# chengl7-lab/scape

Measured on AMD Instinct MI355X. Metric: UTR regions/sec (infer_pa EM to convergence), 50k UTRs x 2k reads synthetic, higher is better.
Workload: dtype f64; 1 GPU; 50k-UTR synthetic stream x 2000 reads, K=1..10 x 10 restarts; step = one resident batch of 512 UTRs per GPU; reads_per_utr=2000, k_cap=10, n_frag_max=1469, re_run_mode=False, rng_mode=per_utr, parallelism=utr-shard x1

## Files before the change

### include/scape_hip.h

```cpp
#ifndef SCAPE_HIP_H
#define SCAPE_HIP_H

#include <stdint.h>

#ifdef __cplusplus
extern "C" {
#endif

#define SCAPE_HIP_ABI_VERSION 4
#define SCAPE_SENT (-3.4028234663852886e38)
#define SCAPE_MAX_BETA 160
#define SCAPE_MAX_S 64
#define SCAPE_MAX_K 63
#define SCAPE_MAX_JOBS_PER_UTR 1024

typedef struct scape_hip_ctx scape_hip_ctx;

typedef struct scape_hip_params {
    double mu_f;
    double sigma_f;
    double max_unif_ws;
    int32_t n_beta;
    int32_t n_s;
    int32_t nround;
    int32_t reserved;
    double betas[SCAPE_MAX_BETA];
    double s_dis[SCAPE_MAX_S];
    double pmf_s[SCAPE_MAX_S];
} scape_hip_params;

int scape_hip_abi_version(void);
const char *scape_hip_last_error(void);
int scape_hip_device_count(int *count);
int scape_hip_create(int device, scape_hip_ctx **out);
int scape_hip_destroy(scape_hip_ctx *ctx);
int scape_hip_device_name(scape_hip_ctx *ctx, char *buf, int buflen);

int scape_hip_loglik_xlr_t_pa(scape_hip_ctx *ctx, const double *x, const double *l,
                              const double *pa, int32_t n, double theta, double sigma_f,
                              double *out);
int scape_hip_loglik_xlr_t_r_known(scape_hip_ctx *ctx, const double *x, const double *l,
                                   const double *r, int32_t n, const double *s_dis,
                                   const double *pmf_s, int32_t n_s, double theta, double mu_f,
                                   double sigma_f, double *out);
int scape_hip_loglik_xlr_t_r_unknown(scape_hip_ctx *ctx, const double *x, const double *l,
                                     const double *r, int32_t n, const double *s_dis,
                                     const double *pmf_s, int32_t n_s, double theta, double mu_f,
                                     double sigma_f, double *out);
int scape_hip_get_loglik_marginal_tensor(scape_hip_ctx *ctx, const double *all_theta,
                                         int32_t n_theta, const double *betas, int32_t n_beta,
                                         const double *loglik_xlr_t_arr, int32_t n_frag,
                                         double *out);

int scape_hip_batch_load(scape_hip_ctx *ctx, const scape_hip_params *params, int32_t n_utr,
                         const int64_t *bin_off, const double *x, const double *l,
                         const double *r, const double *pa, const double *cnt,
                         const int64_t *theta_off, const double *all_theta,
                         const double *utr_L, const double *min_theta, const double *unif_ll);
int scape_hip_batch_bytes(scape_hip_ctx *ctx, int64_t *bytes_batch, int64_t *bytes_free,
                          int64_t *bytes_total);
int scape_hip_batch_build(scape_hip_ctx *ctx);
int scape_hip_batch_phase_b_form(scape_hip_ctx *ctx, int32_t *form);
int scape_hip_batch_em(scape_hip_ctx *ctx, int32_t n_jobs, int32_t kmax, const int32_t *job_utr,
                       const int32_t *job_K, const int32_t *job_fixed, const int32_t *alpha_idx,
                       const int32_t *beta_idx, const double *ws, const int8_t *k_arr,
                       int32_t *alpha_idx_out, int32_t *beta_idx_out, double *ws_out,
                       double *bic_out, int32_t *n_lb_out, double *lb_out);
int scape_hip_batch_em_fetch_lb(scape_hip_ctx *ctx, int32_t n_sel, const int32_t *job_idx, double *lb_out);
int scape_hip_batch_labels(scape_hip_ctx *ctx, int32_t n_sel, int32_t kmax, const int32_t *sel_utr,
                           const int32_t *sel_K, const int32_t *alpha_idx, const int32_t *beta_idx,
                           const double *ws, int32_t *labels_out);
int scape_hip_batch_fetch_loglik(scape_hip_ctx *ctx, int32_t utr, double *A_out);
int scape_hip_batch_fetch_tensor(scape_hip_ctx *ctx, int32_t utr, double *M_out);
int scape_hip_batch_free(scape_hip_ctx *ctx);

int scape_hip_timing_reset(scape_hip_ctx *ctx);
int scape_hip_timing_get(scape_hip_ctx *ctx, int32_t which, double *ms_total, int32_t *n_launches);
int scape_hip_em_counters(scape_hip_ctx *ctx, int64_t *rounds, int64_t *slab_elems,
                          int64_t *z_elems);

int scape_hip_em_traffic(scape_hip_ctx *ctx, int64_t *mstep_tensor_bytes, int64_t *mstep_v_bytes_requested,
                         int64_t *mstep_v_bytes_unique, int64_t *mstep_launches);

int scape_hip_report_counts(scape_hip_ctx *ctx, int32_t n_rec, const int64_t *read_off, const int32_t *K,
                            const int64_t *label, const int64_t *cb_id, int64_t id_min, int64_t id_span,
                            const int32_t *id2col, int32_t n_cols, int64_t *row_tot_out, int8_t *complete_out,
                            int64_t *bad_read_out);
int scape_hip_report_render(scape_hip_ctx *ctx, int32_t slot, int32_t n_rows, const int64_t *rows, const int8_t *is_int,
                            const int64_t *pre_off, const char *pre, int64_t *bytes_out);
int scape_hip_report_render_mtx(scape_hip_ctx *ctx, int32_t slot, int32_t n_rows, const int64_t *rows, int64_t row_no0,
                                int64_t *bytes_out, int64_t *nnz_out);
int scape_hip_report_group_sums(scape_hip_ctx *ctx, int32_t n_seg, const int32_t *seg_off, int32_t n_rows,
                                const int64_t *rows, int32_t *sum_out, int32_t *nz_out);
int scape_hip_report_perm_masks(scape_hip_ctx *ctx, int32_t n1, int32_t n2, int64_t p_first, int32_t p_count,
                                uint64_t seed);
int scape_hip_report_perm_masks_strata(scape_hip_ctx *ctx, int32_t n_strata, const int32_t *m1, const int32_t *m2,
                                       int64_t p_first, int32_t p_count, uint64_t seed);
int scape_hip_report_perm_bits_get(scape_hip_ctx *ctx, int32_t p, uint64_t *words_out);
int scape_hip_report_perm_test(scape_hip_ctx *ctx, int32_t n_rec, const int64_t *rec_row_off, const int64_t *rows,
                               int64_t *t_out, int64_t *a0_out, int64_t *site_n_ge_out, double *stat0_out,
                               int64_t *gene_n_ge_out);
int scape_hip_report_perm_len(scape_hip_ctx *ctx, int32_t n_rec, const int64_t *rec_row_off, const int64_t *rows,
                              const double *w, const double *tol, int64_t *t_out, int64_t *a0_out, double *delta0_out,
                              int64_t *n_ge_out);
int scape_hip_report_perm_labels(scape_hip_ctx *ctx, int32_t n_groups, const int32_t *sizes, int64_t p_first,
                                 int32_t p_count, uint64_t seed);
int scape_hip_report_perm_labels_get(scape_hip_ctx *ctx, int32_t p, uint8_t *labels_out);
int scape_hip_report_perm_groups(scape_hip_ctx *ctx, int32_t n_rec, const int64_t *rec_row_off, const int64_t *rows,
                                 int32_t n_groups, const int32_t *seg_off, int64_t *t_out, int64_t *a0_out,
                                 int64_t *site_n_ge_out, double *stat0_out, double *site_stat0_out,
                                 int64_t *gene_n_ge_out);
int scape_hip_report_perm_len_groups(scape_hip_ctx *ctx, int32_t n_rec, const int64_t *rec_row_off, const int64_t *rows,
                                     int32_t n_groups, const int32_t *seg_off, const int32_t *q, const double *tol_stat,
                                     const double *tol_delta, int64_t *t_out, int64_t *a0_out, double *stat0_out,
                                     double *delta0_out, int64_t *n_ge_out, int64_t *group_n_ge_out);
int scape_hip_report_perm_pair_masks(scape_hip_ctx *ctx, int32_t n_groups, const int32_t *sizes, int32_t n_pairs,
                                     const int32_t *pair_g, const int32_t *pair_h, int64_t p_first, int32_t p_count,
                                     uint64_t seed);
int scape_hip_report_perm_pair_bits_get(scape_hip_ctx *ctx, int32_t pair, int32_t p, uint64_t *words_out);
int scape_hip_report_perm_pairs(scape_hip_ctx *ctx, int32_t n_rec, const int64_t *rec_row_off, const int64_t *rows,
                                int32_t n_groups, const int32_t *seg_off, int32_t pair_first, int32_t pair_count,
                                int64_t *t_out, int64_t *a0_out, int64_t *site_n_ge_out, double *stat0_out,
                                int64_t *gene_n_ge_out);
int scape_hip_report_perm_marker_masks(scape_hip_ctx *ctx, int32_t n_markers, const int32_t *sizes, int32_t n_others,
                                       const int32_t *orig_rank, int64_t p_first, int32_t p_count, uint64_t seed);
int scape_hip_report_perm_marker_bits_get(scape_hip_ctx *ctx, int32_t marker, int32_t p, uint64_t *words_out);
int scape_hip_report_perm_markers(scape_hip_ctx *ctx, int32_t n_rec, const int64_t *rec_row_off, const int64_t *rows,
                                  int32_t n_seg, const int32_t *seg_off, int32_t marker_first, int32_t marker_count,
                                  int64_t *t_out, int64_t *a0_out, int64_t *site_n_ge_out, double *stat0_out,
                                  int64_t *gene_n_ge_out);
int scape_hip_report_perm_scores(scape_hip_ctx *ctx, int32_t n, const uint16_t *q, int64_t p_first, int32_t p_count,
                                 uint64_t seed);
int scape_hip_report_perm_scores_get(scape_hip_ctx *ctx, int32_t p, uint16_t *scores_out);
int scape_hip_report_perm_trend(scape_hip_ctx *ctx, int32_t n_rec, const int64_t *rec_row_off, const int64_t *rows,
                                int64_t *t_out, int64_t *s0_out, int64_t *sq0_out, int64_t *site_n_ge_out,
                                double *d0_out, double *stat0_out, int64_t *gene_n_ge_out);
int scape_hip_report_perm_len_trend(scape_hip_ctx *ctx, int32_t n_rec, const int64_t *rec_row_off, const int64_t *rows,
                                    const int32_t *x, int64_t *t_out, int64_t *s0_out, int64_t *sq0_out,
                                    int64_t *c0_out ,
                                    int64_t *n_ge_out );
int scape_hip_report_fetch(scape_hip_ctx *ctx, int32_t slot, void **host_ptr, int64_t *bytes_out);
int scape_hip_report_hist(scape_hip_ctx *ctx, int32_t n_rec, const int64_t *read_off, const int32_t *K,
                          const int64_t *label, const int64_t *cb_id, int64_t id_min, int64_t id_span,
                          const int32_t *id2code, int32_t n_codes, int64_t *n_groups_out, int64_t *bad_read_out);
int scape_hip_report_hist_fetch(scape_hip_ctx *ctx, int64_t n_groups, int32_t *codes_out, int64_t n_hist,
                                int32_t *hist_out);
int scape_hip_report_free(scape_hip_ctx *ctx);

#ifdef __cplusplus
}
#endif
#endif
```

### scape_amd/_lib.py

```python
from __future__ import annotations

import ctypes
import os

import numpy as np

SENT = float(np.finfo("f").min)
MAX_BETA, MAX_S, MAX_K = 160, 64, 63
_HERE = os.path.dirname(os.path.abspath(__file__))
LIB_PATH = os.environ.get("SCAPE_HIP_LIB") or os.path.join(_HERE, "libscape_hip.so")

c_d, c_i, c_i32, c_i64 = ctypes.c_double, ctypes.c_int, ctypes.c_int32, ctypes.c_int64
P_d = ctypes.POINTER(c_d)
P_i32 = ctypes.POINTER(c_i32)
P_i64 = ctypes.POINTER(c_i64)
P_i8 = ctypes.POINTER(ctypes.c_int8)
P_u16 = ctypes.POINTER(ctypes.c_uint16)
P_void = ctypes.c_void_p


class ScapeHipError(RuntimeError):
    pass


class Params(ctypes.Structure):
    _fields_ = [("mu_f", c_d), ("sigma_f", c_d), ("max_unif_ws", c_d),
                ("n_beta", c_i32), ("n_s", c_i32), ("nround", c_i32), ("reserved", c_i32),
                ("betas", c_d * MAX_BETA), ("s_dis", c_d * MAX_S), ("pmf_s", c_d * MAX_S)]


SIGNATURES = {
    "scape_hip_abi_version": (c_i, []),
    "scape_hip_last_error": (ctypes.c_char_p, []),
    "scape_hip_device_count": (c_i, [ctypes.POINTER(c_i)]),
    "scape_hip_create": (c_i, [c_i, ctypes.POINTER(P_void)]),
    "scape_hip_destroy": (c_i, [P_void]),
    "scape_hip_device_name": (c_i, [P_void, ctypes.c_char_p, c_i]),
    "scape_hip_loglik_xlr_t_pa": (c_i, [P_void, P_d, P_d, P_d, c_i32, c_d, c_d, P_d]),
    "scape_hip_loglik_xlr_t_r_known": (c_i, [P_void, P_d, P_d, P_d, c_i32, P_d, P_d, c_i32, c_d, c_d, c_d, P_d]),
    "scape_hip_loglik_xlr_t_r_unknown": (c_i, [P_void, P_d, P_d, P_d, c_i32, P_d, P_d, c_i32, c_d, c_d, c_d, P_d]),
    "scape_hip_get_loglik_marginal_tensor": (c_i, [P_void, P_d, c_i32, P_d, c_i32, P_d, c_i32, P_d]),
    "scape_hip_batch_load": (c_i, [P_void, ctypes.POINTER(Params), c_i32, P_i64, P_d, P_d, P_d, P_d, P_d,
                                   P_i64, P_d, P_d, P_d, P_d]),
    "scape_hip_batch_bytes": (c_i, [P_void, P_i64, P_i64, P_i64]),
    "scape_hip_batch_phase_b_form": (c_i, [P_void, P_i32]),
    "scape_hip_batch_build": (c_i, [P_void]),
    "scape_hip_batch_em": (c_i, [P_void, c_i32, c_i32, P_i32, P_i32, P_i32, P_i32, P_i32, P_d, P_i8,
                                 P_i32, P_i32, P_d, P_d, P_i32, P_d]),
    "scape_hip_batch_em_fetch_lb": (c_i, [P_void, c_i32, P_i32, P_d]),
    "scape_hip_batch_labels": (c_i, [P_void, c_i32, c_i32, P_i32, P_i32, P_i32, P_i32, P_d, P_i32]),
    "scape_hip_batch_fetch_loglik": (c_i, [P_void, c_i32, P_d]),
    "scape_hip_batch_fetch_tensor": (c_i, [P_void, c_i32, P_d]),
    "scape_hip_batch_free": (c_i, [P_void]),
    "scape_hip_timing_reset": (c_i, [P_void]),
    "scape_hip_timing_get": (c_i, [P_void, c_i32, P_d, P_i32]),
    "scape_hip_em_counters": (c_i, [P_void, P_i64, P_i64, P_i64]),
    "scape_hip_em_traffic": (c_i, [P_void, P_i64, P_i64, P_i64, P_i64]),
    "scape_hip_report_counts": (c_i, [P_void, c_i32, P_i64, P_i32, P_i64, P_i64, c_i64, c_i64, P_i32, c_i32,
                                      P_i64, P_i8, P_i64]),
    "scape_hip_report_render": (c_i, [P_void, c_i32, c_i32, P_i64, P_i8, P_i64, ctypes.c_char_p, P_i64]),
    "scape_hip_report_render_mtx": (c_i, [P_void, c_i32, c_i32, P_i64, c_i64, P_i64, P_i64]),
    "scape_hip_report_group_sums": (c_i, [P_void, c_i32, P_i32, c_i32, P_i64, P_i32, P_i32]),
    "scape_hip_report_perm_masks": (c_i, [P_void, c_i32, c_i32, c_i64, c_i32, ctypes.c_uint64]),
    "scape_hip_report_perm_masks_strata": (c_i, [P_void, c_i32, P_i32, P_i32, c_i64, c_i32, ctypes.c_uint64]),
    "scape_hip_report_perm_bits_get": (c_i, [P_void, c_i32, ctypes.POINTER(ctypes.c_uint64)]),
    "scape_hip_report_perm_test": (c_i, [P_void, c_i32, P_i64, P_i64, P_i64, P_i64, P_i64, P_d, P_i64]),
    "scape_hip_report_perm_len": (c_i, [P_void, c_i32, P_i64, P_i64, P_d, P_d, P_i64, P_i64, P_d, P_i64]),
    "scape_hip_report_perm_labels": (c_i, [P_void, c_i32, P_i32, c_i64, c_i32, ctypes.c_uint64]),
    "scape_hip_report_perm_labels_get": (c_i, [P_void, c_i32, ctypes.POINTER(ctypes.c_uint8)]),
    "scape_hip_report_perm_groups": (c_i, [P_void, c_i32, P_i64, P_i64, c_i32, P_i32, P_i64, P_i64, P_i64, P_d, P_d,
                                           P_i64]),
    "scape_hip_report_perm_len_groups": (c_i, [P_void, c_i32, P_i64, P_i64, c_i32, P_i32, P_i32, P_d, P_d, P_i64, P_i64,
                                               P_d, P_d, P_i64, P_i64]),
    "scape_hip_report_perm_pair_masks": (c_i, [P_void, c_i32, P_i32, c_i32, P_i32, P_i32, c_i64, c_i32, ctypes.c_uint64]),
    "scape_hip_report_perm_pair_bits_get": (c_i, [P_void, c_i32, c_i32, ctypes.POINTER(ctypes.c_uint64)]),
    "scape_hip_report_perm_pairs": (c_i, [P_void, c_i32, P_i64, P_i64, c_i32, P_i32, c_i32, c_i32, P_i64, P_i64, P_i64,
                                          P_d, P_i64]),
    "scape_hip_report_perm_marker_masks": (c_i, [P_void, c_i32, P_i32, c_i32, P_i32, c_i64, c_i32, ctypes.c_uint64]),
    "scape_hip_report_perm_marker_bits_get": (c_i, [P_void, c_i32, c_i32, ctypes.POINTER(ctypes.c_uint64)]),
    "scape_hip_report_perm_markers": (c_i, [P_void, c_i32, P_i64, P_i64, c_i32, P_i32, c_i32, c_i32, P_i64, P_i64, P_i64,
                                            P_d, P_i64]),
    "scape_hip_report_perm_scores": (c_i, [P_void, c_i32, P_u16, c_i64, c_i32, ctypes.c_uint64]),
    "scape_hip_report_perm_scores_get": (c_i, [P_void, c_i32, P_u16]),
    "scape_hip_report_perm_trend": (c_i, [P_void, c_i32, P_i64, P_i64, P_i64, P_i64, P_i64, P_i64, P_d, P_d, P_i64]),
    "scape_hip_report_perm_len_trend": (c_i, [P_void, c_i32, P_i64, P_i64, P_i32, P_i64, P_i64, P_i64, P_i64, P_i64]),
    "scape_hip_report_fetch": (c_i, [P_void, c_i32, ctypes.POINTER(P_void), P_i64]),
    "scape_hip_report_hist": (c_i, [P_void, c_i32, P_i64, P_i32, P_i64, P_i64, c_i64, c_i64, P_i32, c_i32,
                                    P_i64, P_i64]),
    "scape_hip_report_hist_fetch": (c_i, [P_void, c_i64, P_i32, c_i64, P_i32]),
    "scape_hip_report_free": (c_i, [P_void]),
}

_lib = None


def load_library():
    global _lib
    if _lib is None:
        if not os.path.exists(LIB_PATH):
            raise ScapeHipError(
                f"{LIB_PATH} is missing: build it with `python -c 'import __graft_entry__ as g; g.build()'` "
                "(hipcc --offload-arch=gfx950); scape_amd has no CPU fallback")
        lib = ctypes.CDLL(LIB_PATH)
        for name, (res, args) in SIGNATURES.items():
            fn = getattr(lib, name)
            fn.restype, fn.argtypes = res, args
        if lib.scape_hip_abi_version() != 4:
            raise ScapeHipError("libscape_hip.so ABI version mismatch")
        _lib = lib
    return _lib


def last_error():
    return load_library().scape_hip_last_error().decode("utf-8", "replace")


def check(rc, what):
    if rc != 0:
        raise ScapeHipError(f"{what}: {last_error()}")


def ptr(a, t=P_d):
    return a.ctypes.data_as(t)


def f64(a):
    return np.ascontiguousarray(a, dtype=np.float64)


def i32(a):
    return np.ascontiguousarray(a, dtype=np.int32)


def device_count():
    n = c_i(0)
    check(load_library().scape_hip_device_count(ctypes.byref(n)), "device_count")
    return n.value


class Context:

    def __init__(self, device=0):
        self.lib = load_library()
        self.h = P_void()
        check(self.lib.scape_hip_create(int(device), ctypes.byref(self.h)), f"create(device={device})")
        self.device = device

    def close(self):
        if self.h:
            self.lib.scape_hip_destroy(self.h)
            self.h = P_void()

    def __del__(self):
        try:
            self.close()
        except Exception:
            pass

    def __enter__(self):
        return self

    def __exit__(self, *exc):
        self.close()

    def name(self):
        buf = ctypes.create_string_buffer(256)
        check(self.lib.scape_hip_device_name(self.h, buf, 256), "device_name")
        return buf.value.decode()


_default_ctx = {}


def default_context(device=None):
    if device is None:
        device = int(os.environ.get("SCAPE_HIP_DEVICE", os.environ.get("LOCAL_RANK", "0")))
    if device not in _default_ctx:
        _default_ctx[device] = Context(device)
    return _default_ctx[device]
```

### scape_amd/csrc/em_lockstep.inc

```

#define MT_RB 1
#define MT_ROWS (64 * MT_RB)
#define MT_NC 32
#define MT_PITCH (MT_NC + 2)
#define MT_VPITCH (MT_NC + 2)
#define MT_MAXJ 64
#ifndef EM_DEPTH
#define EM_DEPTH 3
#endif
static_assert(EM_DEPTH >= 1 && EM_DEPTH <= 8, "column slots per job");
#ifndef MT_DV1
#define MT_DV1 1
#endif

#ifndef MT_DEEP
#define MT_DEEP 2
#endif
#define CNT_SLAB 4
#define CNT_EXEC (4 + 64)
#define CNT_MSTEP_TENSOR (4 + 2 * 64)
#define CNT_MSTEP_VREQ (4 + 3 * 64)
#define CNT_MSTEP_VUNI (4 + 4 * 64)
static_assert(MT_ROWS == TILE_ROWS, "tile height must match k_tile_extent / the host tables");
static_assert(MT_MAXJ <= 64, "the per-pass job setup gives one job to each lane of one wavefront");

struct EmState {
    int32_t *ia, *ib, *sia, *sib;
    double *ws, *slw;
    double *lb, *ell;
    int32_t *nlb, *status;
    unsigned long long *pend;
    int32_t *rd_k, *rd_lo, *rd_hi, *rd_m;
    int32_t *rd_n0, *rd_n1;
    double *rd_lw, *rd_sv;
    double *V;
    double *Vsuf;
    const int64_t *voff;
    double *pt_score;
    int32_t *pt_row;
    const int64_t *ptoff;
};

__device__ __forceinline__ double d_wave_allsum(double v) {
#pragma unroll
    for (int off = 32; off > 0; off >>= 1) v += __shfl_xor(v, off, 64);
    return v;
}

#ifndef ESTEP_EXP_GROUP
#define ESTEP_EXP_GROUP 1
#endif
struct EstepNext {
    int status;
    int nlb;
    int pub_k;
    int k_next;
};

template <int CA, int CX, int NW = 1>
__device__ __forceinline__ EstepNext estep_body(
    const UtrDesc *__restrict__ descs, const DevParams &P, const double *__restrict__ cnt,
    const double *__restrict__ M, int kmax, const int32_t *__restrict__ job_utr,
    const int32_t *__restrict__ job_K, const int32_t *__restrict__ job_fixed,
    const int32_t *__restrict__ a_in, const int32_t *__restrict__ b_in,
    const double *__restrict__ ws_in, const int8_t *__restrict__ k_arr, const EmState &S,
    int32_t *__restrict__ a_out, int32_t *__restrict__ b_out, double *__restrict__ ws_out,
    double *__restrict__ bic_out, int32_t *__restrict__ nlb_out, double *__restrict__ lb_out,
    unsigned long long *__restrict__ counters, int launch, int slot, int depth, int job, int lane, int status,
    unsigned long long *s_roff, double *s_lwc, double *s_wsum ,
    const double2 *s_exptab , int wave = 0, double *s_xz = nullptr ,
    double *s_tot = nullptr ) {
    constexpr int CMAX = CA;
#ifdef ESTEP_STAMPS
    const unsigned long long st0 = __builtin_amdgcn_s_memtime();
#define ESTEP_STAMP(v) const unsigned long long v = __builtin_amdgcn_s_memtime()
#else
#define ESTEP_STAMP(v)
#endif
    const bool lead = (NW == 1) || wave == 0;
    const int nround = P.nround, B = P.B;
    const int u_job = job_utr[job];
    const int K = (CX > 0) ? CX - 1 : job_K[job], C = K + 1;
    const bool fixed = job_fixed[job] != 0;
    int32_t *ia = S.ia + (size_t)job * kmax, *ib = S.ib + (size_t)job * kmax;
    int32_t *sia = S.sia + (size_t)job * kmax, *sib = S.sib + (size_t)job * kmax;
    double *ws = S.ws + (size_t)job * (kmax + 1), *slw = S.slw + (size_t)job * (kmax + 1);
    const bool r0 = launch == 0 && slot == 0;
    const bool resolve = slot == 0 && launch > 0;
    const size_t col0 = (size_t)job * depth, col = col0 + slot;
    int pre_m[EM_DEPTH], pre_lo[EM_DEPTH], pre_hi[EM_DEPTH], pre_k[EM_DEPTH];
    int64_t pre_ptoff[EM_DEPTH];
    bool rdm = false;
#pragma unroll
    for (int q = 0; q < EM_DEPTH; ++q) {
        const bool on = resolve && q < depth;
        pre_m[q] = on ? S.rd_m[col0 + q] : 0;
        pre_lo[q] = on ? S.rd_lo[col0 + q] : 0;
        pre_hi[q] = on ? S.rd_hi[col0 + q] : 0;
        pre_k[q] = on ? S.rd_k[col0 + q] : 0;
        pre_ptoff[q] = on ? S.ptoff[col0 + q] : 0;
        rdm = rdm || pre_m[q] != 0;
    }
    const int64_t pre_voff = S.voff[col];
    const int k_lane = (lane < nround) ? (int)k_arr[(size_t)job * nround + lane] : 0;
    const double lb_prev = r0 ? SENT : S.lb[job];
    const int nlb_prev = r0 ? 0 : S.nlb[job];
    auto k_of_round = [&](int i) {
        const int ii = min(i, nround - 1);
        return (nround <= 64) ? __shfl(k_lane, ii, 64) : (int)k_arr[(size_t)job * nround + ii];
    };
    const int k_now = k_of_round(nlb_prev);
    const int k_next = __builtin_amdgcn_readfirstlane(k_of_round(nlb_prev + 1));
    double my_ws = 0.0, my_slw = 0.0;
    int my_ia = 0, my_ib = 0, my_sia = 0, my_sib = 0;
    if (lane < C) {
        my_ws = r0 ? ws_in[(size_t)job * (kmax + 1) + lane] : ws[lane];
        if (!r0) my_slw = slw[lane];
        if (lane < K) {
            my_ia = r0 ? a_in[(size_t)job * kmax + lane] : ia[lane];
            my_ib = r0 ? b_in[(size_t)job * kmax + lane] : ib[lane];
            my_sia = r0 ? my_ia : sia[lane];
            my_sib = r0 ? my_ib : sib[lane];
        }
    }
    const UtrDesc d = descs[u_job];
    double pt_best[EM_DEPTH];
    int pt_best_r[EM_DEPTH];
#pragma unroll
    for (int q = 0; q < EM_DEPTH; ++q) {
        pt_best[q] = -INFINITY;
        pt_best_r[q] = pre_lo[q];
        if (pre_m[q]) {
            const int t0 = pre_lo[q] / MT_ROWS, t1 = (pre_hi[q] - 1) / MT_ROWS;
            for (int t = t0 + lane; t <= t1; t += 64) {
                const double sc = S.pt_score[pre_ptoff[q] + t];
                const int rr = S.pt_row[pre_ptoff[q] + t];
                if (sc > pt_best[q]) {
                    pt_best[q] = sc;
                    pt_best_r[q] = rr;
                }
            }
        }
    }
    const int N = d.N, Np = d.Np;
    const double *Mu = M + (size_t)d.m_off;
    const double *cu = cnt + d.bin_off;
    if (r0) my_slw = d_logw(my_ws);

    if (lead && r0) {
        if (lane < C) {
            ws[lane] = my_ws;
            slw[lane] = my_slw;
            if (lane < K) {
                ia[lane] = sia[lane] = my_ia;
                ib[lane] = sib[lane] = my_ib;
            }
        }
        if (lane == 0) {
            S.lb[job] = SENT;
            S.nlb[job] = 0;
            S.ell[job] = 0.0;
        }
    }
    int upd_k[EM_DEPTH], upd_a[EM_DEPTH], upd_b[EM_DEPTH];
#pragma unroll
    for (int q = 0; q < EM_DEPTH; ++q) {
        upd_k[q] = -1;
        upd_a[q] = upd_b[q] = 0;
        if (pre_m[q]) {
            double best = pt_best[q];
            int best_r = pt_best_r[q];
#pragma unroll
            for (int off = 32; off > 0; off >>= 1) {
                const double ob = __shfl_xor(best, off, 64);
                const int orr = __shfl_xor(best_r, off, 64);
                if (ob > best || (ob == best && orr < best_r)) {
                    best = ob;
                    best_r = orr;
                }
            }
            upd_k[q] = pre_k[q];
            upd_a[q] = best_r / B;
            upd_b[q] = best_r - upd_a[q] * B;
            if (lead && lane == 0) {
                ia[upd_k[q]] = upd_a[q];
                ib[upd_k[q]] = upd_b[q];
            }
            if (lane == upd_k[q]) {
                my_ia = upd_a[q];
                my_ib = upd_b[q];
            }
        }
    }
    if (slot == 0 && lead && lane == 0 && (r0 || rdm))
        for (int q = 0; q < depth; ++q) S.rd_m[col0 + q] = 0;
    auto cur_ia = [&](int i) {
        int v = ia[i];
#pragma unroll
        for (int q = 0; q < EM_DEPTH; ++q) v = (i == upd_k[q]) ? upd_a[q] : v;
        return v;
    };
    auto cur_ib = [&](int i) {
        int v = ib[i];
#pragma unroll
        for (int q = 0; q < EM_DEPTH; ++q) v = (i == upd_k[q]) ? upd_b[q] : v;
        return v;
    };

    if (status == 1 || nlb_prev >= nround) {
        if (lead && lane == 0) {
            const int n_lb = S.nlb[job];
            bic_out[job] = d_bic(S.ell[job], K, N);
            nlb_out[job] = n_lb;
            int idx[CMAX];
            for (int i = 0; i < K; ++i) idx[i] = i;
            for (int i = 1; i < K; ++i) {
                const int v = idx[i];
                int j = i - 1;
                while (j >= 0 && cur_ia(idx[j]) > cur_ia(v)) {
                    idx[j + 1] = idx[j];
                    --j;
                }
                idx[j + 1] = v;
            }
            for (int i = 0; i < K; ++i) {
                a_out[(size_t)job * kmax + i] = cur_ia(idx[i]);
                b_out[(size_t)job * kmax + i] = cur_ib(idx[i]);
                ws_out[(size_t)job * (kmax + 1) + i] = ws[idx[i]];
            }
            ws_out[(size_t)job * (kmax + 1) + K] = ws[K];
            for (int i = K; i < kmax; ++i) {
                a_out[(size_t)job * kmax + i] = -1;
                b_out[(size_t)job * kmax + i] = -1;
                ws_out[(size_t)job * (kmax + 1) + i + 1] = 0.0;
            }
            S.status[job] = 2;
            atomicAdd(&counters[0], (unsigned long long)n_lb);
            atomicAdd(&counters[2], (unsigned long long)n_lb * (unsigned long long)N * (unsigned long long)C);
        }
        return EstepNext{2, nlb_prev, -1, 0};
    }

    if (lead && lane == 0) atomicAdd(&counters[CNT_EXEC + (job & 63)], 1ull);
    const int k = k_now;
    const double wk_old = __shfl(my_ws, k, 64);
    const double slw_k = d_logw(wk_old);
    const int sia_k = (k < K) ? __shfl(my_ia, k, 64) : 0;
    const int sib_k = (k < K) ? __shfl(my_ib, k, 64) : 0;
    const int ia_km1 = __shfl(my_ia, max(k - 1, 0), 64), ia_kp1 = __shfl(my_ia, min(k + 1, 63), 64);
    if (lead && lane == 0) {
        slw[k] = slw_k;
        if (k < K) {
            sia[k] = sia_k;
            sib[k] = sib_k;
        }
    }
    if (lead && lane < CMAX) {
        const int c = lane;
        int sa = 0, sb = 0;
        double lw_c = 0.0;
        if (c < C) {
            if (c == k) {
                lw_c = slw_k;
                sa = sia_k;
                sb = sib_k;
            } else {
                lw_c = my_slw;
                sa = my_sia;
                sb = my_sib;
            }
        }
        s_roff[c] = (c < K) ? ((unsigned long long)sa * B + sb) * Np : 0ull;
        s_lwc[c] = (c < K) ? lw_c : lw_c + d.unif_ll;
    }
    __syncthreads();
    double *Vj = S.V + pre_voff;

    ESTEP_STAMP(st1);
    double tot_w[CMAX], t_sumk = 0.0, t_ell = 0.0, t_ent = 0.0;
    int nz_lo = 0x7fffffff, nz_hi = -1;
    bool mod = false;
    if constexpr (NW == 1) {
        for (int pass = 0; pass < 2; ++pass) {
    #pragma unroll
            for (int c = 0; c < CMAX; ++c) s_wsum[c * 64 + lane] = 0.0;
            double sumk = 0.0, ell = 0.0, ent = 0.0;
            nz_lo = 0x7fffffff;
            nz_hi = -1;
            double mcur[CMAX], ccur = 0.0;
            auto fetch = [&](int n, double (&m)[CMAX], double &cn) {
                const bool ok = n < N;
                cn = ok ? cu[n] : 0.0;
    #pragma unroll
                for (int c = 0; c < CMAX; ++c) m[c] = (ok && c < K) ? Mu[s_roff[c] + n] : 0.0;
            };
            fetch(lane, mcur, ccur);
    #pragma unroll
            for (int c = 0; c < CMAX; ++c) asm volatile("" : "+v"(mcur[c]));
            asm volatile("" : "+v"(ccur));
            for (int n = lane; n < Np; n += 64) {
                double mnext[CMAX], cnext;
                fetch(n + 64, mnext, cnext);
                double vkn = 0.0;
                if (n < N) {
                    const double cn = ccur;
                    auto lzv = [&](int c) { return (c < K) ? s_lwc[c] + mcur[c] : s_lwc[c]; };
                    double mx = 0.0;
    #pragma unroll
                    for (int c = 0; c < CMAX; ++c) {
                        if (c < C) {
                            const double v = lzv(c);
                            mx = (c == 0 || v > mx) ? v : mx;
                        }
                    }
                    double z[CMAX];
                    unsigned long long live = 0ull;
#if ESTEP_EXP_GROUP >= 2
    #pragma unroll
                    for (int c = 0; c < CMAX; c += ESTEP_EXP_GROUP) {
    #pragma unroll
                        for (int i = 0; i < ESTEP_EXP_GROUP; ++i)
                            if (c + i < CMAX) z[c + i] = 0.0;
                        if (c < C) {
                            double arg[ESTEP_EXP_GROUP];
                            bool any_live = false;
    #pragma unroll
                            for (int i = 0; i < ESTEP_EXP_GROUP; ++i) {
                                const bool in = (c + i < CMAX) && (c + i < C);
                                arg[i] = in ? (lzv((c + i < CMAX) ? c + i : c) - mx) * cn : -1000.0;
                                any_live |= arg[i] >= -746.0;
                            }
                            if (__ballot(any_live)) {
    #pragma unroll
                                for (int i = 0; i < ESTEP_EXP_GROUP; ++i)
                                    if (c + i < CMAX)
                                        if (c + i < C) {
                                            live |= 1ull << (c + i);
                                            z[c + i] = d_exp_nonpos(arg[i], s_exptab);
                                        }
                            }
                            __builtin_amdgcn_sched_barrier(0);
                        }
                    }
#else
    #pragma unroll
                    for (int c = 0; c < CMAX; ++c) {
                        z[c] = 0.0;
                        if (c < C) {
                            const double arg = (lzv(c) - mx) * cn;
                            if (__ballot(arg >= -746.0)) {
                                live |= 1ull << c;
                                z[c] = d_exp_nonpos(arg, s_exptab);
                            }
                            __builtin_amdgcn_sched_barrier(0);
                        }
                    }
#endif
                    const double s = d_np_sum<CMAX>(z, C);
                    const double rs = d_rcp_mid(s);
                    double zk = 0.0;
    #pragma unroll
                    for (int c = 0; c < CMAX; ++c) {
                        if (live & (1ull << c)) z[c] = z[c] * rs;
                        if (c == k) {
                            sumk += z[c];
                            if (mod) z[c] += 1e-8;
                            zk = z[c];
                        }
                    }
                    const double s2 = d_np_sum<CMAX>(z, C);
                    const double x2 = s2 - 1.0;
                    const double ls = d_log_pos(s), rs2 = d_rcp_mid(s2);
                    double ls2 = x2 - 0.5 * x2 * x2;
                    if (__ballot(fabs(x2) >= 1e-5)) ls2 = (fabs(x2) < 1e-5) ? ls2 : log(s2);
                    double lzk_mod = 0.0;
                    if (mod) lzk_mod = log(zk);
                    double en = 0.0;
    #pragma unroll
                    for (int c = 0; c < CMAX; ++c) {
                        if (c < C && ((live & (1ull << c)) || (mod && c == k))) {
                            const double lzc_full = lzv(c);
                            s_wsum[c * 64 + lane] += cn * z[c];
                            if (z[c] != 0.0) ell += (z[c] * cn) * lzc_full;
                            const double pk = z[c] * rs2;
                            const double lzc = (mod && c == k) ? lzk_mod : (lzc_full - mx) * cn - ls;
                            en += (pk > 0.0) ? -pk * (lzc - ls2) : 0.0;
                        }
                    }
                    ent += cn * en;
                    vkn = zk * cn;
                }
                Vj[n] = vkn;
                if (vkn != 0.0) {
                    nz_lo = min(nz_lo, n);
                    nz_hi = n;
                }
    #pragma unroll
                for (int c = 0; c < CMAX; ++c) mcur[c] = mnext[c];
                ccur = cnext;
            }
    #pragma unroll
            for (int c = 0; c < CMAX; ++c) tot_w[c] = d_wave_allsum(s_wsum[c * 64 + lane]);
            t_sumk = d_wave_allsum(sumk);
            t_ell = d_wave_allsum(ell);
            t_ent = d_wave_allsum(ent);
            if (pass == 0 && t_sumk < 1e-8) {
                mod = true;
                continue;
            }
            break;
        }
    } else {
        for (int pass = 0; pass < 2; ++pass) {
#pragma unroll
            for (int c = 0; c < CMAX; ++c)
                if ((c % NW) == wave) s_wsum[c * 64 + lane] = 0.0;
            double sumk = 0.0, ell = 0.0, ent = 0.0;
            nz_lo = 0x7fffffff;
            nz_hi = -1;
            double mcur[CMAX], ccur = 0.0;
            auto fetch = [&](int n, double (&m)[CMAX], double &cn) {
                const bool ok = n < N;
                cn = ok ? cu[n] : 0.0;
#pragma unroll
                for (int c = 0; c < CMAX; ++c) m[c] = (ok && c < K) ? Mu[s_roff[c] + n] : 0.0;
            };
            fetch(lane, mcur, ccur);
#pragma unroll
            for (int c = 0; c < CMAX; ++c) asm volatile("" : "+v"(mcur[c]));
            asm volatile("" : "+v"(ccur));
            int buf = 0;
            for (int n0 = 0; n0 < Np; n0 += 64, buf ^= 1) {
                const int n = n0 + lane;
                double mnext[CMAX], cnext;
                fetch(n + 64, mnext, cnext);
                double *xz = s_xz + (size_t)buf * (CMAX * 64);
                const double cn = ccur;
                auto lzv = [&](int c) { return (c < K) ? s_lwc[c] + mcur[c] : s_lwc[c]; };
                double mx = 0.0;
                if (n < N) {
#pragma unroll
                    for (int c = 0; c < CMAX; ++c) {
                        if (c < C) {
                            const double v = lzv(c);
                            mx = (c == 0 || v > mx) ? v : mx;
                        }
                    }
#pragma unroll
                    for (int c = 0; c < CMAX; ++c) {
                        if (c < C && (c % NW) == wave) {
                            const double arg = (lzv(c) - mx) * cn;
                            double zr = 0.0;
                            if (__ballot(arg >= -746.0)) zr = d_exp_nonpos(arg, s_exptab);
                            xz[c * 64 + lane] = zr;
                            __builtin_amdgcn_sched_barrier(0);
                        }
                    }
                }
                __syncthreads();
                double vkn = 0.0;
                if (n < N) {
                    double z[CMAX];
#pragma unroll
                    for (int c = 0; c < CMAX; ++c) z[c] = (c < C) ? xz[c * 64 + lane] : 0.0;
                    const double s = d_np_sum<CMAX>(z, C);
                    const double rs = d_rcp_mid(s);
                    double zk = 0.0;
#pragma unroll
                    for (int c = 0; c < CMAX; ++c) {
                        z[c] = z[c] * rs;
                        if (c == k) {
                            sumk += z[c];
                            if (mod) z[c] += 1e-8;
                            zk = z[c];
                        }
                    }
                    const double s2 = d_np_sum<CMAX>(z, C);
                    const double x2 = s2 - 1.0;
                    const double ls = d_log_pos(s), rs2 = d_rcp_mid(s2);
                    double ls2 = x2 - 0.5 * x2 * x2;
                    if (__ballot(fabs(x2) >= 1e-5)) ls2 = (fabs(x2) < 1e-5) ? ls2 : log(s2);
                    double lzk_mod = 0.0;
                    if (mod) lzk_mod = log(zk);
#pragma unroll
                    for (int c = 0; c < CMAX; ++c)
                        if (c < C && (c % NW) == wave) s_wsum[c * 64 + lane] += cn * z[c];
                    if (lead) {
                        double en = 0.0;
#pragma unroll
                        for (int c = 0; c < CMAX; ++c) {
                            if (c < C) {
                                const double lzc_full = lzv(c);
                                if (z[c] != 0.0) ell += (z[c] * cn) * lzc_full;
                                const double pk = z[c] * rs2;
                                const double lzc = (mod && c == k) ? lzk_mod : (lzc_full - mx) * cn - ls;
                                en += (pk > 0.0) ? -pk * (lzc - ls2) : 0.0;
                            }
                        }
                        ent += cn * en;
                        vkn = zk * cn;
                    }
                }
                if (lead && n < Np) {
                    Vj[n] = vkn;
                    if (vkn != 0.0) {
                        nz_lo = min(nz_lo, n);
                        nz_hi = n;
                    }
                }
#pragma unroll
                for (int c = 0; c < CMAX; ++c) mcur[c] = mnext[c];
                ccur = cnext;
            }
#pragma unroll
            for (int c = 0; c < CMAX; ++c) {
                if ((c % NW) == wave) {
                    const double t = d_wave_allsum(s_wsum[c * 64 + lane]);
                    if (lane == 0) s_tot[c] = t;
                }
            }
            if (lead) {
                t_sumk = d_wave_allsum(sumk);
                t_ell = d_wave_allsum(ell);
                t_ent = d_wave_allsum(ent);
                if (lane == 0) s_tot[CMAX] = (pass == 0 && t_sumk < 1e-8) ? 1.0 : 0.0;
            }
            __syncthreads();
#pragma unroll
            for (int c = 0; c < CMAX; ++c) tot_w[c] = s_tot[c];
            const bool redo = s_tot[CMAX] != 0.0;
            __syncthreads();
            if (redo) {
                mod = true;
                continue;
            }
            break;
        }
        if (!lead) return EstepNext{0, 0, -1, 0};
    }

    ESTEP_STAMP(st2);
    double sv = 0.0;
#pragma unroll
    for (int c = 0; c < CMAX; ++c)
        if (c == k) sv = tot_w[c];
    double wn[CMAX];
#pragma unroll
    for (int c = 0; c < CMAX; ++c) wn[c] = (c < C) ? tot_w[c] : 0.0;
    {
        const double s = d_np_sum<CMAX>(wn, C);
#pragma unroll
        for (int c = 0; c < CMAX; ++c) wn[c] = wn[c] / s;
        double wK = 0.0;
#pragma unroll
        for (int c = 0; c < CMAX; ++c)
            if (c == K) wK = wn[c];
        if (wK > P.max_unif_ws) {
            const double sk = d_np_sum<CMAX>(wn, K);
#pragma unroll
            for (int c = 0; c < CMAX; ++c) {
                if (c < K) wn[c] = (1 - P.max_unif_ws) * wn[c] / sk;
                if (c == K) wn[c] = P.max_unif_ws;
            }
        }
    }
    double wk_new = 0.0;
#pragma unroll
    for (int c = 0; c < CMAX; ++c) {
        if (c == k) wk_new = wn[c];
        if (c == lane && c < C) ws[c] = wn[c];
    }

#pragma unroll
    for (int off = 32; off > 0; off >>= 1) {
        nz_lo = min(nz_lo, __shfl_xor(nz_lo, off, 64));
        nz_hi = max(nz_hi, __shfl_xor(nz_hi, off, 64));
    }
    ESTEP_STAMP(st3);
    if (!fixed && k < K) {
        double *Sj = S.Vsuf + (pre_voff >> 4) + col;
        double carry = 0.0;
        for (int nb = ((Np - 1) >> 6) << 6; nb >= 0; nb -= 8 * 64) {
            double vv[8];
#pragma unroll
            for (int q = 0; q < 8; ++q) {
                const int n = nb - 64 * q + lane;
                vv[q] = (n >= 0 && n < Np) ? Vj[n] : 0.0;
            }
#pragma unroll
            for (int off = 1; off < 64; off <<= 1) {
#pragma unroll
                for (int q = 0; q < 8; ++q) {
                    const double t = __shfl_down(vv[q], off, 64);
                    if (lane + off < 64) vv[q] += t;
                }
            }
#pragma unroll
            for (int q = 0; q < 8; ++q) {
                const int n0 = nb - 64 * q;
                if (n0 >= 0) {
                    const int n = n0 + lane;
                    if ((lane & 15) == 0 && n < Np) Sj[n >> 4] = carry + vv[q];
                    carry += __shfl(vv[q], 0, 64);
                }
            }
        }
        if (lane == 0) Sj[Np >> 4] = 0.0;
    }
    ESTEP_STAMP(st4);
    const double lb_new = t_ell + t_ent;
    const int status_new = (fabs(lb_new - lb_prev) < fabs(1e-6 * lb_prev)) ? 1 : 0;
    const bool has_m = (!fixed && k < K);
    if (lane == 0) {
        const int n_lb = nlb_prev;
        lb_out[(size_t)job * nround + n_lb] = lb_new;
        S.nlb[job] = n_lb + 1;
        S.ell[job] = t_ell;
        S.lb[job] = lb_new;
        S.status[job] = status_new;
        S.rd_m[col] = has_m ? 1 : 0;
        if (has_m) {
            const int lo = (k == 0) ? 0 : ia_km1;
            const int hi = (k == K - 1) ? d.T - 1 : ia_kp1;
            S.rd_k[col] = k;
            S.rd_lo[col] = lo * B;
            S.rd_hi[col] = (hi + 1) * B;
            S.rd_lw[col] = d_logw(wk_new);
            S.rd_sv[col] = sv;
            S.rd_n0[col] = (nz_hi >= 0) ? nz_lo : 0;
            S.rd_n1[col] = (nz_hi >= 0) ? nz_hi + 1 : 0;
            atomicAdd(&counters[CNT_SLAB + (job & 63)], (unsigned long long)(hi + 1 - lo) * B * (unsigned long long)N);
        }
    }
#ifdef ESTEP_STAMPS
    if (NW == 1 && lane == 0) {
        const unsigned long long st5 = __builtin_amdgcn_s_memtime();
        unsigned long long *sp = counters + 4 + 5 * 64;
        atomicAdd(&sp[0], st1 - st0);
        atomicAdd(&sp[1], st2 - st1);
        atomicAdd(&sp[2], st3 - st2);
        atomicAdd(&sp[3], st4 - st3);
        atomicAdd(&sp[4], st5 - st4);
        atomicAdd(&sp[7], 1ull);
    }
#endif
#undef ESTEP_STAMP
    return EstepNext{status_new, nlb_prev + 1, has_m ? k : -1, k_next};
}

#define ESTEP_ARGS(ROUND, STATUS) descs, P, cnt, M, kmax, job_utr, job_K, job_fixed, a_in, b_in, ws_in, k_arr, S, a_out, \
                   b_out, ws_out, bic_out, nlb_out, lb_out, counters, ROUND, slot, depth, job, lane, STATUS, s_roff, s_lwc, s_wsum, s_exptab
#define ESTEP_CASE(C, ROUND, STATUS) \
    case C: nx = estep_body<C, C, ESTEP_NW>(ESTEP_ARGS(ROUND, STATUS) ESTEP_EXTRA); break;
#define ESTEP_DISPATCH(CM, ROUND, STATUS)                                                         \
    do {                                                                                          \
        if constexpr (CM <= 16) {                                                                 \
            const int c_exact = job_K[job] + 1;                                                   \
            if constexpr (CM >= 16) {                                                             \
                if (c_exact > 12) {                                                               \
                    switch (c_exact) {                                                            \
                        ESTEP_CASE(13, ROUND, STATUS) ESTEP_CASE(14, ROUND, STATUS)               \
                        ESTEP_CASE(15, ROUND, STATUS)                                             \
                        default: nx = estep_body<16, 16, ESTEP_NW>(ESTEP_ARGS(ROUND, STATUS) ESTEP_EXTRA); break;            \
                    }                                                                             \
                    break;                                                                        \
                }                                                                                 \
            }                                                                                     \
            if constexpr (CM >= 12) {                                                             \
                if (c_exact > 8) {                                                                \
                    switch (c_exact) {                                                            \
                        ESTEP_CASE(9, ROUND, STATUS) ESTEP_CASE(10, ROUND, STATUS)                \
                        ESTEP_CASE(11, ROUND, STATUS)                                             \
                        default: nx = estep_body<12, 12, ESTEP_NW>(ESTEP_ARGS(ROUND, STATUS) ESTEP_EXTRA); break;            \
                    }                                                                             \
                    break;                                                                        \
                }                                                                                 \
            }                                                                                     \
            if constexpr (CM >= 8) {                                                              \
                if (c_exact > 4) {                                                                \
                    switch (c_exact) {                                                            \
                        ESTEP_CASE(5, ROUND, STATUS) ESTEP_CASE(6, ROUND, STATUS)                 \
                        ESTEP_CASE(7, ROUND, STATUS)                                              \
                        default: nx = estep_body<8, 8, ESTEP_NW>(ESTEP_ARGS(ROUND, STATUS) ESTEP_EXTRA); break;              \
                    }                                                                             \
                    break;                                                                        \
                }                                                                                 \
            }                                                                                     \
            switch (c_exact) {                                                                    \
                ESTEP_CASE(1, ROUND, STATUS) ESTEP_CASE(2, ROUND, STATUS) ESTEP_CASE(3, ROUND, STATUS) \
                default: nx = estep_body<4, 4, ESTEP_NW>(ESTEP_ARGS(ROUND, STATUS) ESTEP_EXTRA); break;                      \
            }                                                                                     \
        } else {                                                                                  \
            nx = estep_body<CM, 0, ESTEP_NW>(ESTEP_ARGS(ROUND, STATUS) ESTEP_EXTRA);                                       \
        }                                                                                         \
    } while (0)

__host__ __device__ inline bool em_run_ahead_stops(int status, int nlb, int nround, int k_next, unsigned long long pend) {
    return status != 0 || nlb >= nround || (pend & (7ull << k_next)) != 0ull;
}
#define ESTEP_NW 1
#ifndef ESTEP_WPS
#define ESTEP_WPS 3
#endif
#define ESTEP_EXTRA
template <int CMAX>
__global__ __launch_bounds__(64, (CMAX > 12 ? 2 : ESTEP_WPS)) void k2_estep(
    const UtrDesc *__restrict__ descs, DevParams P, const double *__restrict__ cnt,
    const double *__restrict__ M, int kmax, const int32_t *__restrict__ job_utr,
    const int32_t *__restrict__ job_K, const int32_t *__restrict__ job_fixed,
    const int32_t *__restrict__ a_in, const int32_t *__restrict__ b_in,
    const double *__restrict__ ws_in, const int8_t *__restrict__ k_arr, EmState S,
    int32_t *__restrict__ a_out, int32_t *__restrict__ b_out, double *__restrict__ ws_out,
    double *__restrict__ bic_out, int32_t *__restrict__ nlb_out, double *__restrict__ lb_out,
    unsigned long long *__restrict__ counters, int launch, int slot, int depth, const int32_t *__restrict__ job_list,
    int n_jobs) {
    const int chunk = (n_jobs + 7) >> 3;
    const int jidx = (int)(blockIdx.x & 7) * chunk + (int)(blockIdx.x >> 3);
    if (jidx >= n_jobs) return;
    const int job = job_list[jidx];
    const int lane = threadIdx.x;
    const int status = (launch == 0 && slot == 0) ? 0 : S.status[job];
    if (status == 2) return;
    unsigned long long pend = 0ull;
    if (slot > 0) {
        pend = S.pend[job];
        if (!(pend & 1ull)) return;
        pend &= ~1ull;
    }
    __shared__ unsigned long long s_roff[CMAX];
    __shared__ double s_lwc[CMAX];
    __shared__ double s_wsum[CMAX * 64];
    __shared__ double2 s_exptab[128];
    d_load_exptab(s_exptab, lane, 64);
    EstepNext nx;
    ESTEP_DISPATCH(CMAX, launch, status);
    if (depth > 1 && lane == 0) {
        if (nx.pub_k >= 0) pend |= 2ull << nx.pub_k;
        const bool stop = em_run_ahead_stops(nx.status, nx.nlb, P.nround, nx.k_next, pend) || job_fixed[job] != 0;
        S.pend[job] = pend | (stop ? 0ull : 1ull);
    }
}

template <int CMAX>
__global__ __launch_bounds__(64, (CMAX > 12 ? 2 : 3)) void k2_estep_all_rounds(
    const UtrDesc *__restrict__ descs, DevParams P, const double *__restrict__ cnt,
    const double *__restrict__ M, int kmax, const int32_t *__restrict__ job_utr,
    const int32_t *__restrict__ job_K, const int32_t *__restrict__ job_fixed,
    const int32_t *__restrict__ a_in, const int32_t *__restrict__ b_in,
    const double *__restrict__ ws_in, const int8_t *__restrict__ k_arr, EmState S,
    int32_t *__restrict__ a_out, int32_t *__restrict__ b_out, double *__restrict__ ws_out,
    double *__restrict__ bic_out, int32_t *__restrict__ nlb_out, double *__restrict__ lb_out,
    unsigned long long *__restrict__ counters, const int32_t *__restrict__ job_list, int n_jobs) {
    const int chunk = (n_jobs + 7) >> 3;
    const int jidx = (int)(blockIdx.x & 7) * chunk + (int)(blockIdx.x >> 3);
    if (jidx >= n_jobs) return;
    const int job = job_list[jidx];
    const int lane = threadIdx.x;
    __shared__ unsigned long long s_roff[CMAX];
    __shared__ double s_lwc[CMAX];
    __shared__ double s_wsum[CMAX * 64];
    __shared__ double2 s_exptab[128];
    d_load_exptab(s_exptab, lane, 64);
    for (int round = 0; round <= P.nround; ++round) {
        const int status = (round == 0) ? 0 : S.status[job];
        if (status == 2) return;
        constexpr int slot = 0, depth = 1;
        EstepNext nx;
        ESTEP_DISPATCH(CMAX, round, status);
        (void)nx;
        __threadfence();
        __syncthreads();
    }
}
#undef ESTEP_NW
#undef ESTEP_EXTRA
#define ESTEP_NW 4
#define ESTEP_EXTRA , wave, s_xz, s_tot
template <int CMAX>
__global__ __launch_bounds__(256, 1) void k2_estep_cs(
    const UtrDesc *__restrict__ descs, DevParams P, const double *__restrict__ cnt,
    const double *__restrict__ M, int kmax, const int32_t *__restrict__ job_utr,
    const int32_t *__restrict__ job_K, const int32_t *__restrict__ job_fixed,
    const int32_t *__restrict__ a_in, const int32_t *__restrict__ b_in,
    const double *__restrict__ ws_in, const int8_t *__restrict__ k_arr, EmState S,
    int32_t *__restrict__ a_out, int32_t *__restrict__ b_out, double *__restrict__ ws_out,
    double *__restrict__ bic_out, int32_t *__restrict__ nlb_out, double *__restrict__ lb_out,
    unsigned long long *__restrict__ counters, int round, const int32_t *__restrict__ job_list, int n_jobs) {
    const int chunk = (n_jobs + 7) >> 3;
    const int jidx = (int)(blockIdx.x & 7) * chunk + (int)(blockIdx.x >> 3);
    if (jidx >= n_jobs) return;
    const int job = job_list[jidx];
    const int lane = threadIdx.x & 63, wave = threadIdx.x >> 6;
    const int status = (round == 0) ? 0 : S.status[job];
    if (status == 2) return;
    __shared__ unsigned long long s_roff[CMAX];
    __shared__ double s_lwc[CMAX];
    __shared__ double s_wsum[CMAX * 64];
    __shared__ double s_xz[2 * CMAX * 64];
    __shared__ double s_tot[CMAX + 4];
    __shared__ double2 s_exptab[128];
    d_load_exptab(s_exptab, threadIdx.x, 256);
    constexpr int slot = 0, depth = 1;
    EstepNext nx;
    ESTEP_DISPATCH(CMAX, round, status);
    (void)nx;
}
#undef ESTEP_NW
#undef ESTEP_EXTRA
#undef ESTEP_DISPATCH
#undef ESTEP_CASE


typedef double v4f64 __attribute__((ext_vector_type(4)));

template <int G, int D>
__device__ __forceinline__ void mstep_pass(const double *__restrict__ Mu, const double *__restrict__ V,
                                           const int64_t *__restrict__ voff, const int *s_jobs, double *mt,
                                           double *vt, int cnt, int Np, int n_lo, int n_hi, int nrows, int row0, int wave, int lane,
                                           int need, v4f64 (&acc)[MT_RB][MT_MAXJ / 16]) {
    const int quarter = lane >> 4, ns = 2 * (lane & 15);
    const int kq = lane >> 4, rc = lane & 15;
    constexpr int DV = MT_DV1 ? 1 : D;
    double2 rm_st[D][4 * MT_RB], rv_st[DV][G];
    const double *vsrc[G];
#pragma unroll
    for (int it = 0; it < G; ++it) {
        const int js = 4 * wave + quarter + 16 * it;
        vsrc[it] = (js < cnt) ? V + voff[s_jobs[js]] : nullptr;
    }
    auto fetchV = [&](int n0, double2 (&rv)[G]) {
        const int nc = (n_hi - n0 < MT_NC) ? n_hi - n0 : MT_NC;
#pragma unroll
        for (int it = 0; it < G; ++it)
            rv[it] = (ns < nc && vsrc[it]) ? *reinterpret_cast<const double2 *>(vsrc[it] + n0 + ns) : make_double2(0.0, 0.0);
    };
    auto fetchM = [&](int n0, double2 (&rm)[4 * MT_RB]) {
        const int nc = (n_hi - n0 < MT_NC) ? n_hi - n0 : MT_NC;
#pragma unroll
        for (int it = 0; it < 4 * MT_RB; ++it) {
            const int row = row0 + 4 * wave + quarter + 16 * it;
            rm[it] = (ns < nc && row < nrows && ((need >> (it / MT_RB)) & 1)) ? *reinterpret_cast<const double2 *>(Mu + (size_t)row * Np + n0 + ns)
                                               : make_double2(0.0, 0.0);
        }
    };
    auto chunk = [&](int n0, double2 (&rm)[4 * MT_RB], double2 (&rv)[G]) {
        const int nc = (n_hi - n0 < MT_NC) ? n_hi - n0 : MT_NC;
        __syncthreads();
#pragma unroll
        for (int it = 0; it < 4 * MT_RB; ++it) {
            const int rr = 4 * wave + quarter + 16 * it;
            *reinterpret_cast<double2 *>(&mt[rr * MT_PITCH + ns]) = rm[it];
        }
#pragma unroll
        for (int it = 0; it < G; ++it) {
            const int js = 4 * wave + quarter + 16 * it;
            *reinterpret_cast<double2 *>(&vt[js * MT_VPITCH + ns]) = rv[it];
        }
        __syncthreads();
        fetchM(n0 + D * MT_NC, rm);
        fetchV(n0 + DV * MT_NC, rv);
#pragma unroll 4
        for (int n4 = 0; n4 < nc; n4 += 4) {
            double a[MT_RB], b[G];
#pragma unroll
            for (int rb = 0; rb < MT_RB; ++rb) a[rb] = mt[(16 * (MT_RB * wave + rb) + rc) * MT_PITCH + n4 + kq];
#pragma unroll
            for (int g = 0; g < G; ++g) b[g] = vt[(16 * g + rc) * MT_VPITCH + n4 + kq];
#pragma unroll
            for (int rb = 0; rb < MT_RB; ++rb)
#pragma unroll
                for (int g = 0; g < G; ++g)
                    acc[rb][g] = __builtin_amdgcn_mfma_f64_16x16x4f64(a[rb], b[g], acc[rb][g], 0, 0, 0);
        }
    };
#pragma unroll
    for (int dd = 0; dd < D; ++dd) fetchM(n_lo + dd * MT_NC, rm_st[dd]);
#pragma unroll
    for (int dd = 0; dd < DV; ++dd) fetchV(n_lo + dd * MT_NC, rv_st[dd]);
    for (int n0 = n_lo; n0 < n_hi; n0 += D * MT_NC) {
#pragma unroll
        for (int dd = 0; dd < D; ++dd)
            if (n0 + dd * MT_NC < n_hi) chunk(n0 + dd * MT_NC, rm_st[dd], rv_st[dd % DV]);
    }
}

__global__ __launch_bounds__(256, 3) void k2_mstep(const UtrDesc *__restrict__ descs, DevParams P,
                                                   const double *__restrict__ M, const int32_t *__restrict__ active, int n_utr, int tiles_max,
                                                   const int64_t *__restrict__ ujob_off,
                                                   const int32_t *__restrict__ ujob_list,
                                                   const double *__restrict__ V,
                                                   const double *__restrict__ Vsuf,
                                                   const int64_t *__restrict__ voff,
                                                   const int32_t *__restrict__ rd_m,
                                                   const int32_t *__restrict__ rd_lo,
                                                   const int32_t *__restrict__ rd_hi,
                                                   const double *__restrict__ rd_lw,
                                                   const double *__restrict__ rd_sv,
                                                   const int32_t *__restrict__ rd_n0,
                                                   const int32_t *__restrict__ rd_n1,
                                                   const int64_t *__restrict__ ptoff,
                                                   double *__restrict__ pt_score,
                                                   int32_t *__restrict__ pt_row,
                                                   const int32_t *__restrict__ tile_nend,
                                                   unsigned long long *__restrict__ counters, int jobs_per_pass,
                                                   unsigned long long *__restrict__ dbg) {
    __shared__ __attribute__((aligned(16))) double mt[MT_ROWS * MT_PITCH];
    __shared__ __attribute__((aligned(16))) double vt[MT_MAXJ * MT_VPITCH];
    __shared__ int s_jobs[MT_MAXJ];
    __shared__ int s_all[1024];
    __shared__ int s_cnt, s_nlo, s_nhi, s_need, s_first;
    __shared__ double s_ps[4][MT_MAXJ];
    __shared__ int s_pr[4][MT_MAXJ];
    __shared__ double s_tail[MT_MAXJ];
    const int id = blockIdx.x;
    int ul, t;
    if (n_utr >= 8) {
        const int slot = id >> 3;
        ul = (slot / tiles_max) * 8 + (id & 7);
        t = slot % tiles_max;
    } else {
        ul = id % n_utr;
        t = id / n_utr;
    }
    if (ul >= n_utr || t >= tiles_max) return;
    const int u = active[ul];
    const UtrDesc d = descs[u];
    const int B = P.B, Np = d.Np;
    const int nrows = d.T * B, row0 = t * MT_ROWS;
    if (row0 >= nrows) return;
    const int tid = threadIdx.x, lane = tid & 63, wave = tid >> 6;
    const double *Mu = M + (size_t)d.m_off;
    const int64_t jlo = ujob_off[u], jhi = ujob_off[u + 1];
    __shared__ int s_wcnt[4];
    int found = 0;
    for (int64_t j0 = jlo; j0 < jhi; j0 += 256) {
        const int64_t jj = j0 + tid;
        int j = -1;
        bool hit = false;
        if (jj < jhi) {
            j = ujob_list[jj];
            hit = rd_m[j] && rd_lo[j] < row0 + MT_ROWS && rd_hi[j] > row0;
        }
        const unsigned long long mask = __ballot(hit);
        if (lane == 0) s_wcnt[wave] = __popcll(mask);
        __syncthreads();
        int off = found;
        for (int w = 0; w < wave; ++w) off += s_wcnt[w];
        off += __popcll(mask & ((1ull << lane) - 1ull));
        if (hit && off < 1024) s_all[off] = j;
        found += s_wcnt[0] + s_wcnt[1] + s_wcnt[2] + s_wcnt[3];
        __syncthreads();
    }
    if (tid == 0) s_cnt = found;
    __syncthreads();
    const int total = min(s_cnt, 1024);
    if (dbg && tid == 0) {
        atomicAdd(&dbg[0], 1ull);
        atomicAdd(&dbg[1], (unsigned long long)(total > 0));
        atomicAdd(&dbg[2], (unsigned long long)total);
        atomicAdd(&dbg[3], (unsigned long long)((total + MT_MAXJ - 1) / MT_MAXJ));
        atomicAdd(&dbg[4 + min((total + 15) / 16, 11)], 1ull);
    }
    if (total == 0) return;
    __shared__ unsigned long long s_by[3];
    if (tid == 0) s_by[0] = s_by[1] = s_by[2] = 0ull;

    for (int base = (int)blockIdx.y * jobs_per_pass; base < total; base += jobs_per_pass * (int)gridDim.y) {
        const int cnt = min(jobs_per_pass, total - base);
        const int G = (cnt + 15) >> 4;
        __syncthreads();
        if (wave == 0) {
            int mk = 0, nlo = 0x7fffffff, nhi = 0;
            bool fst = false;
            if (lane < cnt) {
                const int j = s_all[base + lane];
                s_jobs[lane] = j;
                fst = rd_lo[j] / MT_ROWS == t;
                const int lo = rd_lo[j] - row0, hi = rd_hi[j] - row0;
#pragma unroll
                for (int g4 = 0; g4 < 4; ++g4) mk |= (lo < 16 * (g4 + 1) && hi > 16 * g4) ? (1 << g4) : 0;
                if (rd_n1[j] > rd_n0[j]) {
                    nlo = rd_n0[j];
                    nhi = rd_n1[j];
                }
            }
#pragma unroll
            for (int off = 32; off > 0; off >>= 1) {
                mk |= __shfl_xor(mk, off, 64);
                nlo = min(nlo, __shfl_xor(nlo, off, 64));
                nhi = max(nhi, __shfl_xor(nhi, off, 64));
            }
            const unsigned long long fmask = __ballot(fst);
            if (lane == 0) {
                s_need = mk;
                s_nlo = nlo;
                s_nhi = nhi;
                s_first = __popcll(fmask);
            }
        }
        __syncthreads();
        const int n_lo = (s_nhi > 0) ? (s_nlo & ~15) : 0;
        const int n_sup = (s_nhi > 0) ? min(Np, (s_nhi + 15) & ~15) : 0;
        const int n_ext = tile_nend[d.tile_off + t];
        const int n_hi = min(n_sup, n_ext);
        const int need = s_need;
        if (tid == 0 && n_hi > n_lo) {
            int rows = 0;
#pragma unroll
            for (int g4 = 0; g4 < 4; ++g4)
                if ((need >> g4) & 1) rows += max(0, min(16, nrows - row0 - 16 * g4));
            const unsigned long long span = (unsigned long long)(n_hi - n_lo) * 8ull;
            s_by[0] += span * (unsigned long long)rows;
            s_by[1] += span * (unsigned long long)cnt;
            s_by[2] += span * (unsigned long long)s_first;
        }
        for (int sj = tid; sj < cnt; sj += 256) {
            const int j = s_jobs[sj];
            s_tail[sj] = Vsuf[(voff[j] >> 4) + j + (n_ext >> 4)];
        }
        __syncthreads();
        v4f64 acc[MT_RB][MT_MAXJ / 16];
#pragma unroll
        for (int rb = 0; rb < MT_RB; ++rb)
#pragma unroll
            for (int g = 0; g < MT_MAXJ / 16; ++g) acc[rb][g] = (v4f64){0.0, 0.0, 0.0, 0.0};
        switch (G) {
            case 1: mstep_pass<1, MT_DEEP>(Mu, V, voff, s_jobs, mt, vt, cnt, Np, n_lo, n_hi, nrows, row0, wave, lane, need, acc); break;
            case 2: mstep_pass<2, MT_DEEP>(Mu, V, voff, s_jobs, mt, vt, cnt, Np, n_lo, n_hi, nrows, row0, wave, lane, need, acc); break;
            case 3: mstep_pass<3, 2>(Mu, V, voff, s_jobs, mt, vt, cnt, Np, n_lo, n_hi, nrows, row0, wave, lane, need, acc); break;
            default: mstep_pass<4, 2>(Mu, V, voff, s_jobs, mt, vt, cnt, Np, n_lo, n_hi, nrows, row0, wave, lane, need, acc); break;
        }
        {
            const int kq = lane >> 4, rc = lane & 15;
#pragma unroll
            for (int g = 0; g < MT_MAXJ / 16; ++g) {
                if (g < G) {
                    const int slot_j = 16 * g + rc;
                    double best = -INFINITY;
                    int best_r = 0x7fffffff;
                    if (slot_j < cnt) {
                        const int j = s_jobs[slot_j];
                        const int lo = rd_lo[j], hi = rd_hi[j];
                        const double tl = s_tail[slot_j];
                        const double c0 = rd_lw[j] * rd_sv[j] + ((tl != 0.0) ? SENT * tl : 0.0);
#pragma unroll
                        for (int rb = 0; rb < MT_RB; ++rb) {
#pragma unroll
                            for (int i = 0; i < 4; ++i) {
                                const int row = row0 + 16 * (MT_RB * wave + rb) + kq + 4 * i;
                                const double sc = c0 + acc[rb][g][i];
                                if (row >= lo && row < hi && row < nrows && sc > best) {
                                    best = sc;
                                    best_r = row;
                                }
                            }
                        }
                    }
#pragma unroll
                    for (int off = 16; off <= 32; off <<= 1) {
                        const double ob = __shfl_xor(best, off, 64);
                        const int orr = __shfl_xor(best_r, off, 64);
                        if (ob > best || (ob == best && orr < best_r)) {
                            best = ob;
                            best_r = orr;
                        }
                    }
                    if (kq == 0 && slot_j < cnt) {
                        s_ps[wave][slot_j] = best;
                        s_pr[wave][slot_j] = best_r;
                    }
                }
            }
        }
        __syncthreads();
        for (int sj = tid; sj < cnt; sj += 256) {
            double best = s_ps[0][sj];
            int best_r = s_pr[0][sj];
            for (int w = 1; w < 4; ++w)
                if (s_ps[w][sj] > best) {
                    best = s_ps[w][sj];
                    best_r = s_pr[w][sj];
                }
            const int j = s_jobs[sj];
            pt_score[ptoff[j] + t] = best;
            pt_row[ptoff[j] + t] = (best_r == 0x7fffffff) ? max(rd_lo[j], row0) : best_r;
        }
    }
    if (tid == 0 && s_by[0]) {
        const int sh = (int)(blockIdx.x & 63);
        atomicAdd(&counters[CNT_MSTEP_TENSOR + sh], s_by[0]);
        atomicAdd(&counters[CNT_MSTEP_VREQ + sh], s_by[1]);
        atomicAdd(&counters[CNT_MSTEP_VUNI + sh], s_by[2]);
    }
}
```

### scape_amd/csrc/mstep_multi.inc

```

#ifndef M4_TPW
#define M4_TPW 2
#endif
static_assert(M4_TPW >= 1 && M4_TPW <= 4, "one wavefront per tile table");
#define M4_NW 4
#define M4_WPC M3_WPC
static_assert(M4_TPW * M4_NW <= 16, "per-wavefront hit counts of the set-up");
__device__ __forceinline__ bool m4_is_tile_issuer(int wave) { return wave < 2; }
__device__ __forceinline__ bool m4_is_vec_issuer(int wave) { return wave >= 2; }
__device__ __forceinline__ int m4_role_index(int wave) { return wave & 1; }
#define M4_REC_BYTES (64 * 24)
#define M4_TAIL_BYTES (4 * 64 * 12 + M4_TPW * (M4_REC_BYTES + 12 * 4) + 16 * 4 + 4 * 8)
#define M4_AREA_BYTES (((M4_WPC >= 3 ? 53760 : 81920) - M4_TAIL_BYTES) / 1024 * 1024)
#define M4_LDS_BYTES (M4_AREA_BYTES + M4_TAIL_BYTES)
static_assert((M4_LDS_BYTES + 1279) / 1280 * M4_WPC <= 128, "LDS granules: the rings do not fit at this occupancy");
__host__ __device__ constexpr int m4_rv(int G) { return M4_AREA_BYTES / (G * 2048 + 8192) < 2 ? 2 : M4_AREA_BYTES / (G * 2048 + 8192); }
__host__ __device__ constexpr int m4_rt(int G) {
    return (M4_AREA_BYTES - m4_rv(G) * G * 2048) / 8192 > 10 ? 10 : (M4_AREA_BYTES - m4_rv(G) * G * 2048) / 8192;
}
static_assert(m4_rt(4) >= 2 && m4_rt(3) >= 2 && m4_rt(2) >= 2 && m4_rt(1) >= 2, "a ring needs the slot being multiplied and one in flight");

struct M4Tile {
    const double *tb0, *vb0;
    int nh, G, np_w;
    int he1, he2, he3;
    unsigned pieces;
    bool needed;
    unsigned offs[4];
#ifdef M4_STAMPS
    unsigned long long *stamps;
#endif
};

template <int G>
__device__ __forceinline__ int m4_gact(const M4Tile &T, int h) {
    int g = 1;
    if (G > 1 && h < T.he1) g = 2;
    if (G > 2 && h < T.he2) g = 3;
    if (G > 3 && h < T.he3) g = 4;
    return g;
}
template <int G>
__device__ __forceinline__ void m4_issue(const M4Tile &T, unsigned lds_area, int wave, int h) {
    constexpr int RT = m4_rt(G), RV = m4_rv(G), VSLOT = G * 16 * M3_CH;
    if (m4_is_vec_issuer(wave)) {
        const double *b = T.vb0 + (size_t)h * M3_CH;
        const unsigned dst = lds_area + (unsigned)(h % RV) * (VSLOT * 8) + (unsigned)m4_role_index(wave) * 1024u;
        const int np = m4_gact<G>(T, h);
#pragma unroll
        for (int q = 0; q < G; ++q)
            if (q < np) m3_dma<false>(T.offs[q], b, dst + (unsigned)q * 2048u);
    } else if (m4_is_tile_issuer(wave)) {
        const double *b = T.tb0 + (size_t)h * M3_CH;
        const unsigned dst = lds_area + RV * VSLOT * 8 + (unsigned)(h % RT) * (M3_TSLOT * 8);
#pragma unroll
        for (int i = 0; i < 4; ++i)
            if (i < T.np_w) m3_dma<M3_TILE_NT>(T.offs[i], b, dst + ((T.pieces >> (4 * i)) & 15u) * 1024u);
    }
}
template <int G>
__device__ __forceinline__ void m4_prologue(const M4Tile &T, unsigned lds_area, int wave) {
    const int ahead = m4_is_vec_issuer(wave) ? m4_rv(G) - 1 : m4_rt(G) - 1;
    for (int j = 0; j < ahead; ++j)
        if (j < T.nh) m4_issue<G>(T, lds_area, wave, j);
}
template <int G, int GA>
__device__ __forceinline__ void m4_seg(const M4Tile &T, unsigned lds_area, const double *area, int wave, int lane, int h0, int h1,
                                       v4f64 (&acc)[MT_MAXJ / 16]) {
    constexpr int RT = m4_rt(G), RV = m4_rv(G), VSLOT = G * 16 * M3_CH;
    const double *ringV = area, *ringT = area + RV * VSLOT;
    const int kq = lane >> 4, rc = lane & 15, f = (rc >> 1) & 7;
    int offd[4];
#pragma unroll
    for (int s = 0; s < 4; ++s) offd[s] = ((((2 * s + (kq >> 1)) ^ f) << 1) | (kq & 1));
    const bool vwave = m4_is_vec_issuer(wave);
    const int ahead = vwave ? RV - 1 : RT - 1;
    const int nh = T.nh;
#ifdef M4_STAMPS
    unsigned long long st_wait = 0, st_bar = 0, st_issue = 0, st_mfma = 0;
#define M4_T(v) const unsigned long long v = __builtin_amdgcn_s_memtime()
#else
#define M4_T(v)
#endif
    for (int h = h0; h < h1; ++h) {
        M4_T(t0);
        const int keep = min(ahead - 1, nh - 1 - h);
        int younger = T.np_w * keep;
        if (vwave) {
            younger = 0;
            for (int y = 1; y <= keep; ++y) younger += m4_gact<G>(T, h + y);
        }
        m3_wait_vm(younger);
        asm volatile("s_waitcnt lgkmcnt(0)" ::: "memory");
        M4_T(t1);
        __builtin_amdgcn_s_barrier();
        asm volatile("" ::: "memory");
        M4_T(t2);
        if (h + ahead < nh) m4_issue<G>(T, lds_area, wave, h + ahead);
        M4_T(t3);
        if (T.needed) {
            const double *ts = ringT + (h % RT) * M3_TSLOT + (16 * wave + rc) * M3_CH;
            const double *vs = ringV + (h % RV) * VSLOT + rc * M3_CH;
#pragma unroll
            for (int s = 0; s < 4; ++s) {
                const double a = ts[offd[s]];
                double b[GA];
#pragma unroll
                for (int g = 0; g < GA; ++g) b[g] = vs[g * 16 * M3_CH + offd[s]];
#pragma unroll
                for (int g = 0; g < GA; ++g) acc[g] = __builtin_amdgcn_mfma_f64_16x16x4f64(a, b[g], acc[g], 0, 0, 0);
            }
        }
#ifdef M4_STAMPS
        asm volatile("" : "+v"(acc[0]));
        M4_T(t4);
        st_wait += t1 - t0;
        st_bar += t2 - t1;
        st_issue += t3 - t2;
        st_mfma += t4 - t3;
#endif
    }
#ifdef M4_STAMPS
    if (lane == 0 && h1 > h0) {
        unsigned long long *sp = T.stamps + 4 * ((GA - 1) * 2 + (vwave ? 1 : 0));
        atomicAdd(&sp[0], st_wait);
        atomicAdd(&sp[1], st_bar);
        atomicAdd(&sp[2], st_issue);
        atomicAdd(&sp[3], st_mfma);
        atomicAdd(T.stamps + 32 + (GA - 1) * 2 + (vwave ? 1 : 0), (unsigned long long)(h1 - h0));
    }
#endif
#undef M4_T
}
template <int G>
__device__ __forceinline__ void m4_loop(const M4Tile &T, unsigned lds_area, const double *area, int wave, int lane,
                                        v4f64 (&acc)[MT_MAXJ / 16]) {
    const int nh = T.nh;
    int h = 0;
    if constexpr (G >= 4) {
        m4_seg<G, 4>(T, lds_area, area, wave, lane, h, min(T.he3, nh), acc);
        h = max(h, min(T.he3, nh));
    }
    if constexpr (G >= 3) {
        m4_seg<G, 3>(T, lds_area, area, wave, lane, h, min(T.he2, nh), acc);
        h = max(h, min(T.he2, nh));
    }
    if constexpr (G >= 2) {
        m4_seg<G, 2>(T, lds_area, area, wave, lane, h, min(T.he1, nh), acc);
        h = max(h, min(T.he1, nh));
    }
    m4_seg<G, 1>(T, lds_area, area, wave, lane, h, nh, acc);
}

__global__ __launch_bounds__(64 * M4_NW, (M4_NW * M4_WPC + 3) / 4) void k4_mstep(const UtrDesc *__restrict__ descs, DevParams P,
                                                        const double *__restrict__ M, const int32_t *__restrict__ active, int n_utr, int groups_max,
                                                        const int64_t *__restrict__ ujob_off,
                                                        const int32_t *__restrict__ ujob_list,
                                                        const double *__restrict__ V,
                                                        const double *__restrict__ Vsuf,
                                                        const int64_t *__restrict__ voff,
                                                        const int32_t *__restrict__ rd_m,
                                                        const int32_t *__restrict__ rd_lo,
                                                        const int32_t *__restrict__ rd_hi,
                                                        const double *__restrict__ rd_lw,
                                                        const double *__restrict__ rd_sv,
                                                        const int32_t *__restrict__ rd_n0,
                                                        const int32_t *__restrict__ rd_n1,
                                                        const int64_t *__restrict__ ptoff,
                                                        double *__restrict__ pt_score,
                                                        int32_t *__restrict__ pt_row,
                                                        const int32_t *__restrict__ tile_nend,
                                                        unsigned long long *__restrict__ counters) {
    extern __shared__ __attribute__((aligned(16))) double m4_lds[];
    double *area = m4_lds;
    double *x_ps = m4_lds + M4_AREA_BYTES / 8;
    int *x_pr = reinterpret_cast<int *>(x_ps + 4 * 64);
    int *rec_i = x_pr + 4 * 64;
    int *t_sc = rec_i + M4_TPW * 64 * 6;
    int *t_he = t_sc + M4_TPW * 8;
    int *s_misc = t_he + M4_TPW * 4;
    unsigned long long *s_by = reinterpret_cast<unsigned long long *>(s_misc + 16);
    const unsigned lds_area = (unsigned)(size_t)(__attribute__((address_space(3))) double *)area;

    const int id = blockIdx.x;
    int ul, tg;
    if (n_utr >= 8) {
        const int slot = id >> 3;
        ul = (slot / groups_max) * 8 + (id & 7);
        tg = slot % groups_max;
    } else {
        ul = id % n_utr;
        tg = id / n_utr;
    }
    if (ul >= n_utr || tg >= groups_max) return;
    const int u = active[ul];
    const UtrDesc d = descs[u];
    const int B = P.B, Np = d.Np;
    const int nrows = d.T * B;
    const int t_first = tg * M4_TPW;
    if (t_first * MT_ROWS >= nrows) return;
    const int n_tiles = min(M4_TPW, (nrows - t_first * MT_ROWS + MT_ROWS - 1) / MT_ROWS);
    const int tid = threadIdx.x, lane = tid & 63, wave = __builtin_amdgcn_readfirstlane(tid >> 6);
    const double *Mu = M + (size_t)d.m_off;
    const int64_t jlo = ujob_off[u], jhi = ujob_off[u + 1];

    int found[M4_TPW];
    auto collect = [&](int i_lo, int i_hi, int base) {
#pragma unroll
        for (int i = 0; i < M4_TPW; ++i) found[i] = 0;
        for (int64_t j0 = jlo; j0 < jhi; j0 += 64 * M4_NW) {
            const int64_t jj = j0 + tid;
            int j = -1, lo = 0, hi = 0;
            if (jj < jhi) {
                j = ujob_list[jj];
                if (rd_m[j]) {
                    lo = rd_lo[j];
                    hi = rd_hi[j];
                }
            }
#pragma unroll
            for (int i = 0; i < M4_TPW; ++i) {
                const int row0 = (t_first + i) * MT_ROWS;
                const bool hit = i >= i_lo && i < i_hi && lo < row0 + MT_ROWS && hi > row0;
                const unsigned long long mask = __ballot(hit);
                if (lane == 0) s_misc[M4_NW * i + wave] = __popcll(mask);
            }
            __syncthreads();
#pragma unroll
            for (int i = 0; i < M4_TPW; ++i) {
                const int row0 = (t_first + i) * MT_ROWS;
                const bool hit = i >= i_lo && i < i_hi && lo < row0 + MT_ROWS && hi > row0;
                const unsigned long long mask = __ballot(hit);
                int off = found[i];
                for (int w = 0; w < wave; ++w) off += s_misc[M4_NW * i + w];
                off += __popcll(mask & ((1ull << lane) - 1ull));
                if (hit && off >= base && off < base + 64) rec_i[(i * 64 + off - base) * 6 + 2] = j;
#pragma unroll
                for (int w = 0; w < M4_NW; ++w) found[i] += s_misc[M4_NW * i + w];
            }
            __syncthreads();
        }
    };
    auto finish_table = [&](int i, int total, int base) {
        const int t = t_first + i, row0 = t * MT_ROWS;
        const int cnt = max(0, min(total - base, 64));
        const int n_ext = tile_nend[d.tile_off + t];
        int mk = 0, nlo = 0x7fffffff, nhi = 0;
        bool fst = false;
        int j = 0, lo = 0, hi = 0, n0 = 0, n1 = 0, po32 = 0, vo16 = 0;
        double c0 = 0.0;
        if (lane < cnt) {
            j = rec_i[(i * 64 + lane) * 6 + 2];
            lo = rd_lo[j];
            hi = rd_hi[j];
            n0 = rd_n0[j];
            n1 = rd_n1[j];
            const int64_t vo = voff[j];
            const double lw = rd_lw[j], sv = rd_sv[j];
            const int64_t po = ptoff[j];
            const double tl = Vsuf[(vo >> 4) + j + (n_ext >> 4)];
            c0 = lw * sv + ((tl != 0.0) ? SENT * tl : 0.0);
            fst = lo / MT_ROWS == t;
#pragma unroll
            for (int g4 = 0; g4 < 4; ++g4) mk |= (lo - row0 < 16 * (g4 + 1) && hi - row0 > 16 * g4) ? (1 << g4) : 0;
            if (n1 > n0) {
                nlo = n0;
                nhi = n1;
            }
            po32 = (int)(po + t);
            vo16 = (int)(vo >> 4);
        }
#pragma unroll
        for (int off = 32; off > 0; off >>= 1) {
            mk |= __shfl_xor(mk, off, 64);
            nlo = min(nlo, __shfl_xor(nlo, off, 64));
            nhi = max(nhi, __shfl_xor(nhi, off, 64));
        }
        const unsigned long long fmask = __ballot(fst);
        const int n_lo = (nhi > 0) ? (nlo & ~15) : 0;
        const int n_sup = (nhi > 0) ? min(Np, (nhi + 15) & ~15) : 0;
        const int n_hi = min(n_sup, n_ext);
        const int nh = (n_hi > n_lo) ? (n_hi - n_lo) >> 4 : 0;
        if (lane < 4) t_he[i * 4 + lane] = 0;
        int hc = 0;
        if (lane < cnt && n1 > n0) hc = max(0, min((min(n1, n_hi) - n_lo + 15) >> 4, nh));
        int rank = 0;
        for (int o = 0; o < 64; ++o) {
            const int other = __shfl(hc, o, 64);
            rank += (o < cnt) && (other > hc || (other == hc && o < lane));
        }
        if (lane < cnt) {
            int *rc_ = rec_i + (i * 64 + rank) * 6;
            rc_[0] = lo;
            rc_[1] = hi;
            rc_[2] = po32;
            rc_[3] = vo16;
            *reinterpret_cast<double *>(rc_ + 4) = c0;
            if ((rank & 15) == 0) t_he[i * 4 + (rank >> 4)] = hc;
        }
        if (lane == 0) {
            int *sc = t_sc + i * 8;
            sc[0] = cnt;
            sc[1] = n_lo;
            sc[2] = nh;
            sc[3] = mk;
            sc[4] = __popcll(fmask);
            sc[5] = n_ext;
            sc[6] = total;
        }
    };
    collect(0, n_tiles, 0);
    if (wave < n_tiles) {
        int total = 0;
#pragma unroll
        for (int i = 0; i < M4_TPW; ++i)
            if (i == wave) total = found[i];
        finish_table(wave, total, 0);
    }
    if (tid == 0) s_by[0] = s_by[1] = s_by[2] = 0ull;
    __syncthreads();

    const int l8 = lane >> 3, u8 = lane & 7;
    auto make_tile = [&](int i, M4Tile &T) {
        const int t = t_first + i, row0 = t * MT_ROWS;
        const int *sc = t_sc + i * 8;
        const int cnt = __builtin_amdgcn_readfirstlane(sc[0]), n_lo = __builtin_amdgcn_readfirstlane(sc[1]);
        const int need = __builtin_amdgcn_readfirstlane(sc[3]);
        T.nh = __builtin_amdgcn_readfirstlane(sc[2]);
        T.G = (cnt + 15) >> 4;
        T.he1 = __builtin_amdgcn_readfirstlane(t_he[i * 4 + 1]);
        T.he2 = __builtin_amdgcn_readfirstlane(t_he[i * 4 + 2]);
        T.he3 = __builtin_amdgcn_readfirstlane(t_he[i * 4 + 3]);
        T.needed = (need >> wave) & 1;
        T.np_w = 0;
        T.pieces = 0;
        if (cnt == 0) T.nh = 0;
        if (m4_is_tile_issuer(wave)) {
#pragma unroll
            for (int q = 0; q < 4; ++q) {
                const int pc = 4 * m4_role_index(wave) + q;
                if ((need >> (pc >> 1)) & 1) {
                    const int r = 8 * pc + l8;
                    const int rr = min(row0 + r, nrows - 1) - row0;
                    const unsigned o = (unsigned)(((size_t)rr * Np + 2 * (u8 ^ ((r >> 1) & 7))) * 8);
                    if (T.np_w == 0) T.offs[0] = o; else if (T.np_w == 1) T.offs[1] = o; else if (T.np_w == 2) T.offs[2] = o; else T.offs[3] = o;
                    T.pieces |= (unsigned)pc << (4 * T.np_w);
                    ++T.np_w;
                }
            }
        } else if (m4_is_vec_issuer(wave)) {
#pragma unroll
            for (int q = 0; q < 4; ++q) {
                const int js = 8 * (2 * q + m4_role_index(wave)) + l8;
                const unsigned vo16 = (unsigned)rec_i[(i * 64 + min(js, max(cnt, 1) - 1)) * 6 + 3];
                T.offs[q] = (unsigned)((((size_t)vo16 << 4) + 2 * (u8 ^ ((js >> 1) & 7))) * 8);
            }
        }
#ifdef M4_STAMPS
        T.stamps = counters + (4 + 5 * 64 + 16);
#endif
        T.tb0 = m3_uniform_ptr(Mu + (size_t)row0 * Np + n_lo);
        T.vb0 = m3_uniform_ptr(V + n_lo);
        if (tid == 0 && T.nh > 0) {
            int rows = 0;
#pragma unroll
            for (int g4 = 0; g4 < 4; ++g4)
                if ((need >> g4) & 1) rows += max(0, min(16, nrows - row0 - 16 * g4));
            const unsigned long long span = (unsigned long long)T.nh * 128ull;
            s_by[0] += span * (unsigned long long)rows;
            s_by[1] += span * (unsigned long long)cnt;
            s_by[2] += span * (unsigned long long)sc[4];
        }
    };
#define M4_BY_G(G_, CALL)                 \
    switch (G_) {                          \
        case 0: break;                     \
        case 1: { constexpr int GG = 1; CALL; } break; \
        case 2: { constexpr int GG = 2; CALL; } break; \
        case 3: { constexpr int GG = 3; CALL; } break; \
        default: { constexpr int GG = 4; CALL; } break; \
    }
    auto process = [&](int i, M4Tile &cur, bool have_next, int i_next, M4Tile &nxt) {
        const int t = t_first + i, row0 = t * MT_ROWS;
        v4f64 acc[MT_MAXJ / 16];
#pragma unroll
        for (int g = 0; g < MT_MAXJ / 16; ++g) acc[g] = (v4f64){0.0, 0.0, 0.0, 0.0};
        M4_BY_G(cur.G, m4_loop<GG>(cur, lds_area, area, wave, lane, acc));
        asm volatile("s_waitcnt lgkmcnt(0)" ::: "memory");
        __builtin_amdgcn_s_barrier();
        asm volatile("" ::: "memory");
        if (have_next) {
            make_tile(i_next, nxt);
            M4_BY_G(nxt.G, m4_prologue<GG>(nxt, lds_area, wave));
        }
        const int cnt = __builtin_amdgcn_readfirstlane(t_sc[i * 8]);
        const int G = (cnt + 15) >> 4;
        {
            const int kq = lane >> 4, rc = lane & 15;
#pragma unroll
            for (int g = 0; g < MT_MAXJ / 16; ++g) {
                if (g < G) {
                    const int slot_j = 16 * g + rc;
                    double best = -INFINITY;
                    int best_r = 0x7fffffff;
                    if (slot_j < cnt) {
                        const int *rc_ = rec_i + (i * 64 + slot_j) * 6;
                        const int lo = rc_[0], hi = rc_[1];
                        const double c0 = *reinterpret_cast<const double *>(rc_ + 4);
#pragma unroll
                        for (int q = 0; q < 4; ++q) {
                            const int row = row0 + 16 * wave + kq + 4 * q;
                            const double sc = c0 + acc[g][q];
                            if (row >= lo && row < hi && row < nrows && sc > best) {
                                best = sc;
                                best_r = row;
                            }
                        }
                    }
#pragma unroll
                    for (int off = 16; off <= 32; off <<= 1) {
                        const double ob = __shfl_xor(best, off, 64);
                        const int orr = __shfl_xor(best_r, off, 64);
                        if (ob > best || (ob == best && orr < best_r)) {
                            best = ob;
                            best_r = orr;
                        }
                    }
                    if (kq == 0 && slot_j < cnt) {
                        x_ps[wave * 64 + slot_j] = best;
                        x_pr[wave * 64 + slot_j] = best_r;
                    }
                }
            }
        }
        asm volatile("s_waitcnt lgkmcnt(0)" ::: "memory");
        __builtin_amdgcn_s_barrier();
        asm volatile("" ::: "memory");
        if (tid < cnt) {
            double best = x_ps[tid];
            int best_r = x_pr[tid];
            for (int w = 1; w < 4; ++w)
                if (x_ps[w * 64 + tid] > best) {
                    best = x_ps[w * 64 + tid];
                    best_r = x_pr[w * 64 + tid];
                }
            const int *rc_ = rec_i + (i * 64 + tid) * 6;
            pt_score[(unsigned)rc_[2]] = best;
            pt_row[(unsigned)rc_[2]] = (best_r == 0x7fffffff) ? max(rc_[0], row0) : best_r;
        }
    };
    M4Tile cur, nxt;
    make_tile(0, cur);
    M4_BY_G(cur.G, m4_prologue<GG>(cur, lds_area, wave));
    bool overflow = false;
    for (int i = 0; i < n_tiles; ++i) {
        process(i, cur, i + 1 < n_tiles, i + 1, nxt);
        overflow |= t_sc[i * 8 + 6] > 64;
        cur = nxt;
    }
    if (overflow) {
        asm volatile("s_waitcnt vmcnt(0) lgkmcnt(0)" ::: "memory");
        __syncthreads();
        for (int i = 0; i < n_tiles; ++i) {
            const int total = __builtin_amdgcn_readfirstlane(t_sc[i * 8 + 6]);
            for (int base = 64; base < total; base += 64) {
                collect(i, i + 1, base);
                if (wave == 0) finish_table(i, total, base);
                __syncthreads();
                make_tile(i, cur);
                M4_BY_G(cur.G, m4_prologue<GG>(cur, lds_area, wave));
                process(i, cur, false, 0, nxt);
                asm volatile("s_waitcnt vmcnt(0) lgkmcnt(0)" ::: "memory");
                __syncthreads();
                if (tid == 0) t_sc[i * 8 + 6] = total;
                __syncthreads();
            }
        }
    }
#undef M4_BY_G
    if (tid == 0 && s_by[0]) {
        const int sh = (int)(blockIdx.x & 63);
        atomicAdd(&counters[CNT_MSTEP_TENSOR + sh], s_by[0]);
        atomicAdd(&counters[CNT_MSTEP_VREQ + sh], s_by[1]);
        atomicAdd(&counters[CNT_MSTEP_VUNI + sh], s_by[2]);
    }
}
```

### scape_amd/csrc/scape_hip.hip

```cpp
#include <hip/hip_runtime.h>

#include <algorithm>
#include <atomic>
#include <cmath>
#include <cstdint>
#include <cstdio>
#include <cstdlib>
#include <cstring>
#include <string>
#include <type_traits>
#include <chrono>
#include <utility>
#include <vector>

#include "scape_hip.h"

#define SENT SCAPE_SENT
#define PI_REF 3.141592653589793
#define PITCH 16
#define TILE_ROWS 64

static thread_local std::string g_err;
static int fail(const std::string &msg) {
    g_err = msg;
// ... 325 lines not shown
    }
    const int Wall = hi_all - lo_all + 1;
    for (int e = tid; e < B * Wmax; e += blockDim.x) {
        const int j = e / Wmax, w = e - j * Wmax;
        const int tw = lo_all + w;
        double val = 0.0;
        if (w < Wall && tw >= lo[j] && tw <= hi[j]) val = exp(g[(size_t)j * Wmax + (tw - lo[j])] - G[j]);
        p[e] = val;
    }
    __syncthreads();
    if (Wall > Wmax) {
        if (tid == 0) atomicExch(err_flag, 2);
        return;
    }

    double *Mi = M + (size_t)d.m_off + (size_t)i * B * d.Np;
    const int tile0 = (i * B) / TILE_ROWS, j_split = (tile0 + 1) * TILE_ROWS - i * B;
    int fin0 = 0, fin1 = 0;
    auto note = [&](int j, int n, double val) {
        if (val != SENT) {
            if (j < j_split) fin0 = max(fin0, n + 1);
            else fin1 = max(fin1, n + 1);
        }
    };
    if (probe & 2) {
    } else if (!all_log && BMAX == 16) {
        typedef double v4d __attribute__((ext_vector_type(4)));
        const int WP = ((Wmax + 3) & ~3) + 1;
        double *pm = reinterpret_cast<double *>(hi + B + (B & 1));
        for (int e = tid; e < 16 * WP; e += blockDim.x) {
            const int j = e / WP, w = e - j * WP;
            pm[e] = (j < B && w < Wmax) ? p[(size_t)j * Wmax + w] : 0.0;
        }
        __syncthreads();
        const double *Vu = V + (size_t)d.at_off;
        const int lane = tid & 63, wave = tid >> 6, kq = lane >> 4, rc = lane & 15;
        const int nblocks = d.Np >> 4;
        const int steps = (Wall + 3) >> 2;
        const int full = max(0, min(steps, (d.T - lo_all) >> 2));
        const size_t rstep = (size_t)4 * d.Np;
        const double *pw = pm + rc * WP + kq;
        const double *vbase = Vu + (size_t)(lo_all + kq) * d.Np + rc;
        auto finish = [&](int n, const v4d &acc) {
            const bool pad = n >= d.N;
            const int nn = pad ? d.N - 1 : n;
            const bool lin = !pad && isnan(pa[d.bin_off + nn]) && isnan(r[d.bin_off + nn]);
            const bool wr = pad || lin;
            bool f0 = false, f1 = false;
#pragma unroll
            for (int q = 0; q < 4; ++q) {
                const int j = kq + 4 * q;
                const double a = acc[q];
                const bool pos = a > 0.0;
                const double lg = d_log_pos(pos ? a : 1.0);
                const double val = pad ? 0.0 : (pos ? lg : SENT);
                if (wr && j < B) Mi[(size_t)j * d.Np + n] = val;
                const bool fin = lin && pos && j < B;
                f0 |= fin && j < j_split;
                f1 |= fin && j >= j_split;
            }
            fin0 = max(fin0, f0 ? n + 1 : 0);
            fin1 = max(fin1, f1 ? n + 1 : 0);
        };
        int nb = wave;
        for (; nb + 4 < nblocks; nb += 8) {
            const double *v0 = vbase + nb * 16, *v1 = v0 + 64;
            v4d acc0 = {0.0, 0.0, 0.0, 0.0}, acc1 = {0.0, 0.0, 0.0, 0.0};
            int st = 0;
            auto batch = [&](auto nbc) {
                constexpr int NB = decltype(nbc)::value;
                double b0[NB], b1[NB], av[NB];
#pragma unroll
                for (int k = 0; k < NB; ++k) {
                    b0[k] = v0[k * rstep];
                    b1[k] = v1[k * rstep];
                }
#pragma unroll
                for (int k = 0; k < NB; ++k) av[k] = pw[4 * (st + k)];
#pragma unroll
                for (int k = 0; k < NB; ++k) {
                    acc0 = __builtin_amdgcn_mfma_f64_16x16x4f64(av[k], b0[k], acc0, 0, 0, 0);
                    acc1 = __builtin_amdgcn_mfma_f64_16x16x4f64(av[k], b1[k], acc1, 0, 0, 0);
                }
                v0 += NB * rstep;
                v1 += NB * rstep;
                st += NB;
            };
            while (st + 4 <= full) batch(std::integral_constant<int, 4>());
            switch (full - st) {
                case 3: batch(std::integral_constant<int, 3>()); break;
                case 2: batch(std::integral_constant<int, 2>()); break;
                case 1: batch(std::integral_constant<int, 1>()); break;
                default: break;
            }
            for (; st < steps; ++st) {
                const int wr = min(lo_all + 4 * st + kq, d.T - 1);
                const double av = pw[4 * st];
                const double *vr = Vu + (size_t)wr * d.Np + nb * 16 + rc;
                acc0 = __builtin_amdgcn_mfma_f64_16x16x4f64(av, vr[0], acc0, 0, 0, 0);
                acc1 = __builtin_amdgcn_mfma_f64_16x16x4f64(av, vr[64], acc1, 0, 0, 0);
            }
            finish(nb * 16 + rc, acc0);
            finish(nb * 16 + 64 + rc, acc1);
        }
        for (; nb < nblocks; nb += 4) {
            const double *v0 = vbase + nb * 16;
            v4d acc0 = {0.0, 0.0, 0.0, 0.0};
            int st = 0;
#pragma unroll 4
            for (; st < full; ++st) {
                acc0 = __builtin_amdgcn_mfma_f64_16x16x4f64(pw[4 * st], *v0, acc0, 0, 0, 0);
                v0 += rstep;
            }
            for (; st < steps; ++st) {
                const int wr = min(lo_all + 4 * st + kq, d.T - 1);
                acc0 = __builtin_amdgcn_mfma_f64_16x16x4f64(pw[4 * st], Vu[(size_t)wr * d.Np + nb * 16 + rc], acc0, 0, 0, 0);
            }
            finish(nb * 16 + rc, acc0);
        }
    } else if (!all_log) {
        const double *Vu = V + (size_t)d.at_off;
        for (int n = tid; n < d.Np; n += blockDim.x) {
            if (n >= d.N) {
                for (int j = 0; j < B; ++j) Mi[(size_t)j * d.Np + n] = 0.0;
                continue;
            }
            if (!isnan(pa[d.bin_off + n]) || !isnan(r[d.bin_off + n])) continue;
            if (B <= BMAX) {
                double acc[BMAX];
#pragma unroll
                for (int j = 0; j < BMAX; ++j) acc[j] = 0.0;
                for (int w = 0; w < Wall; ++w) {
                    const double v = Vu[(size_t)(lo_all + w) * d.Np + n];
#pragma unroll
                    for (int j = 0; j < BMAX; ++j)
                        if (j < B) acc[j] += v * p[(size_t)j * Wmax + w];
                }
#pragma unroll
                for (int j = 0; j < BMAX; ++j)
                    if (j < B) {
                        const double val = (acc[j] > 0.0) ? d_log_pos(acc[j]) : SENT;
                        Mi[(size_t)j * d.Np + n] = val;
                        note(j, n, val);
                    }
            } else {
                for (int j = 0; j < B; ++j) {
                    double acc = 0.0;
                    for (int w = 0; w < Wall; ++w)
                        acc += Vu[(size_t)(lo_all + w) * d.Np + n] * p[(size_t)j * Wmax + w];
                    const double val = (acc > 0.0) ? d_log_pos(acc) : SENT;
                    Mi[(size_t)j * d.Np + n] = val;
                    note(j, n, val);
                }
            }
        }
    } else if (all_log) {
        for (int n = d.N + tid; n < d.Np; n += blockDim.x)
            for (int j = 0; j < B; ++j) Mi[(size_t)j * d.Np + n] = 0.0;
    }
    const int n_log = (probe & 1) ? 0 : (all_log ? d.N : d.n_log);
    const double *Au = AT + (size_t)d.at_off;
    for (int item = tid; item < n_log * B; item += blockDim.x) {
        const int j = item / n_log, q = item - j * n_log;
        const int n = all_log ? q : loglist[d.log_off + q];
        const int a = lo[j], W = hi[j] - lo[j] + 1;
        const double Gj = G[j];
        const double *gj = g + (size_t)j * Wmax;
        double mx = Au[(size_t)a * d.Np + n] + gj[0] - Gj;
        for (int w = 1; w < W; ++w) {
            const double t = Au[(size_t)(a + w) * d.Np + n] + gj[w] - Gj;
            if (t > mx) mx = t;
        }
        double sum = 0.0;
        for (int w = 0; w < W; ++w) sum += d_exp_nonpos(Au[(size_t)(a + w) * d.Np + n] + gj[w] - Gj - mx, s_exptab);
        const double val = d_log_pos(sum) + mx;
        Mi[(size_t)j * d.Np + n] = val;
        note(j, n, val);
    }
    if (tile_nend) {
        __shared__ int s_fin[2];
        if (tid < 2) s_fin[tid] = 0;
        __syncthreads();
#pragma unroll
        for (int off = 32; off > 0; off >>= 1) {
            fin0 = max(fin0, __shfl_xor(fin0, off, 64));
            fin1 = max(fin1, __shfl_xor(fin1, off, 64));
        }
        if ((tid & 63) == 0) {
            atomicMax(&s_fin[0], fin0);
            atomicMax(&s_fin[1], fin1);
        }
        __syncthreads();
        if (tid < 2 && s_fin[tid] > 0)
            atomicMax(&tile_nend[d.tile_off + tile0 + tid], min(d.Np, (s_fin[tid] + 15) & ~15));
    }
}

#include "phase_b_split.inc"
#include "em_lockstep.inc"
#include "mstep_ring.inc"
#include "mstep_multi.inc"

template <int CMAX>
__global__ __launch_bounds__(256) void k_labels(const UtrDesc *__restrict__ descs, DevParams P,
                                                const double *__restrict__ cnt,
                                                const double *__restrict__ M, int kmax,
                                                const int32_t *__restrict__ sel_utr,
                                                const int32_t *__restrict__ sel_K,
                                                const int32_t *__restrict__ a_in,
                                                const int32_t *__restrict__ b_in,
                                                const double *__restrict__ ws_in,
                                                int32_t *__restrict__ labels) {
    __shared__ double2 s_exptab[128];
    d_load_exptab(s_exptab, threadIdx.x, blockDim.x);
    __syncthreads();
    const int sel = blockIdx.x;
    const UtrDesc d = descs[sel_utr[sel]];
    const int K = sel_K[sel], C = K + 1, B = P.B;
    const double *Mu = M + (size_t)d.m_off;
    size_t roff[CMAX];
    double slw[CMAX];
#pragma unroll
    for (int c = 0; c < CMAX; ++c) {
        roff[c] = (c < K) ? ((size_t)a_in[(size_t)sel * kmax + c] * B + b_in[(size_t)sel * kmax + c]) * d.Np : 0;
        slw[c] = (c < C) ? d_logw(ws_in[(size_t)sel * (kmax + 1) + c]) : 0.0;
    }
    for (int n = threadIdx.x; n < d.N; n += blockDim.x) {
        const double cn = cnt[d.bin_off + n];
        double lz[CMAX], z[CMAX], mx = 0.0;
#pragma unroll
        for (int c = 0; c < CMAX; ++c) {
            if (c < C) {
                lz[c] = (c < K) ? slw[c] + Mu[roff[c] + n] : slw[c] + d.unif_ll;
                mx = (c == 0 || lz[c] > mx) ? lz[c] : mx;
            } else {
                lz[c] = 0.0;
            }
        }
#pragma unroll
        for (int c = 0; c < CMAX; ++c) z[c] = (c < C) ? d_exp_nonpos((lz[c] - mx) * cn, s_exptab) : 0.0;
        const double s = d_np_sum<CMAX>(z, C);
        int best = 0;
        double bz = 0.0;
#pragma unroll
        for (int c = 0; c < CMAX; ++c) {
            const double zc = z[c] / s;
            if (c < C && (c == 0 || zc > bz)) {
                bz = zc;
                best = c;
            }
        }
        labels[d.bin_off + n] = best;
    }
}

struct DevBuf {
    void *p = nullptr;
    size_t cap = 0;
    DevBuf() = default;
    DevBuf(const DevBuf &) = delete;
    DevBuf &operator=(const DevBuf &) = delete;
    ~DevBuf() { release(); }
    int ensure(size_t bytes) {
        if (bytes <= cap && p) return 0;
        const bool regrow = p != nullptr || (bytes > ((size_t)1 << 30) && bytes <= ((size_t)48 << 30));
        if (p) {
            (void)hipFree(p);
            p = nullptr;
            cap = 0;
        }
        if (bytes == 0) bytes = 16;
        size_t want = regrow ? bytes + bytes / 8 : bytes;
        if (hipMalloc(&p, want) != hipSuccess) {
            (void)hipGetLastError();
            p = nullptr;
            want = bytes;
            HIPCHK(hipMalloc(&p, want));
        }
        cap = want;
        return 0;
    }
    void release() {
        if (p) (void)hipFree(p);
        p = nullptr;
        cap = 0;
    }
    template <typename T>
    T *as() const {
        return reinterpret_cast<T *>(p);
    }
};
static_assert(!std::is_copy_constructible<DevBuf>::value && !std::is_copy_assignable<DevBuf>::value,
              "a copy of a DevBuf would free its memory twice");

struct EventPair {
    hipEvent_t a, b;
};

struct ReportState;

struct EmBufs {
    DevBuf ia, ib, sia, sib, ws, slw, lb, ell, nlb, status, pend, rd_k, rd_lo, rd_hi, rd_m, rd_n0, rd_n1, rd_lw, rd_sv, V, Vsuf,
        voff, pt_score, pt_row, ptoff;
    DevBuf ujoff, ujlist, active, elist, dbg;
    int ensure(size_t nj, size_t nc, size_t kmax, size_t n_utr, size_t vtot, size_t pttot) {
        return ia.ensure(nj * kmax * 4) || ib.ensure(nj * kmax * 4) || sia.ensure(nj * kmax * 4) || sib.ensure(nj * kmax * 4) ||
               ws.ensure(nj * (kmax + 1) * 8) || slw.ensure(nj * (kmax + 1) * 8) || lb.ensure(nj * 8) || ell.ensure(nj * 8) ||
               nlb.ensure(nj * 4) || status.ensure(nj * 4) || pend.ensure(nj * 8) || rd_k.ensure(nc * 4) || rd_lo.ensure(nc * 4) ||
               rd_hi.ensure(nc * 4) || rd_m.ensure(nc * 4) || rd_n0.ensure(nc * 4) || rd_n1.ensure(nc * 4) ||
               rd_lw.ensure(nc * 8) || rd_sv.ensure(nc * 8) || V.ensure(vtot * 8) || Vsuf.ensure((vtot / 16 + nc + 1) * 8) ||
               voff.ensure(nc * 8) || pt_score.ensure(pttot * 8) || pt_row.ensure(pttot * 4) || ptoff.ensure(nc * 8) ||
               ujoff.ensure((n_utr + 1) * 8) || ujlist.ensure(nc * 4) || active.ensure(n_utr * 4) || elist.ensure(nj * 4);
    }
    EmState state() const {
        return EmState{ia.as<int32_t>(), ib.as<int32_t>(), sia.as<int32_t>(), sib.as<int32_t>(), ws.as<double>(), slw.as<double>(),
                       lb.as<double>(), ell.as<double>(), nlb.as<int32_t>(), status.as<int32_t>(), pend.as<unsigned long long>(),
                       rd_k.as<int32_t>(),
                       rd_lo.as<int32_t>(), rd_hi.as<int32_t>(), rd_m.as<int32_t>(), rd_n0.as<int32_t>(), rd_n1.as<int32_t>(),
                       rd_lw.as<double>(), rd_sv.as<double>(), V.as<double>(), Vsuf.as<double>(), voff.as<int64_t>(),
                       pt_score.as<double>(), pt_row.as<int32_t>(), ptoff.as<int64_t>()};
    }
    void release() {
        for (DevBuf *b : {&ia, &ib, &sia, &sib, &ws, &slw, &lb, &ell, &nlb, &status, &pend, &rd_k, &rd_lo, &rd_hi, &rd_m, &rd_n0, &rd_n1, &rd_lw,
                          &rd_sv, &V, &Vsuf, &voff, &pt_score, &pt_row, &ptoff, &ujoff, &ujlist, &active, &elist, &dbg})
            b->release();
    }
};

#define N_COUNTERS (4 + 5 * 64 + 16 + 48)
struct scape_hip_ctx {
    int device = 0;
    std::atomic<bool> busy{false};
    hipStream_t stream = nullptr;
    char name[256] = {0};
    DevParams prm;
    bool loaded = false, built = false;
    bool build_unchecked = false;
    int n_utr = 0, T_max = 0, Np_max = 0, W_max = 1;
    int64_t n_bins = 0;
    std::vector<UtrDesc> h_desc;
    size_t at_total = 0, m_total = 0;
    DevBuf d_x, d_l, d_r, d_pa, d_cnt, d_theta, d_desc, d_loglist, d_AT, d_V, d_M, d_err, d_counters, d_tile_nend;
    DevBuf d_tbi, d_tbG, d_tbpm, d_mlog, d_logbin;
    size_t n_theta_total = 0, mlog_total = 0, n_logbins = 0;
    int pb_form = 0;
    bool pb_slide = false;
    int tiles_max_all = 1;
    size_t tiles_total = 0;
    DevBuf j_utr, j_K, j_fixed, j_a, j_b, j_ws, j_karr, j_ao, j_bo, j_wso, j_bic, j_nlb, j_lb, j_sel, j_lbsel;
    int last_em_jobs = 0;
    DevBuf l_utr, l_K, l_a, l_b, l_ws, l_labels;
    EmBufs em;
    std::vector<EventPair> ev[6];
    double ms_acc[6] = {0, 0, 0, 0, 0, 0};
    int n_acc[6] = {0, 0, 0, 0, 0, 0};
    unsigned long long h_counters[3] = {0, 0, 0};
    unsigned long long h_traffic[4] = {0, 0, 0, 0};
    ReportState *rep = nullptr;
};

static int ev_begin(scape_hip_ctx *c, int which) {
    EventPair e;
    HIPCHK(hipEventCreate(&e.a));
    HIPCHK(hipEventCreate(&e.b));
    HIPCHK(hipEventRecord(e.a, c->stream));
    c->ev[which].push_back(e);
    return 0;
}
static int ev_end(scape_hip_ctx *c, int which) {
    HIPCHK(hipEventRecord(c->ev[which].back().b, c->stream));
    return 0;
}
static int ev_collect(scape_hip_ctx *c) {
    HIPCHK(hipStreamSynchronize(c->stream));
    const bool trace = getenv("SCAPE_HIP_ROUND_TRACE") != nullptr;
    for (int w = 0; w < 6; ++w) {
        int i = 0;
        for (auto &e : c->ev[w]) {
            float ms = 0;
            HIPCHK(hipEventElapsedTime(&ms, e.a, e.b));
            if (trace && w >= 4) fprintf(stderr, "[trace] kind %d launch %d %.4f ms\n", w, i, ms);
            ++i;
            c->ms_acc[w] += ms;
            c->n_acc[w] += 1;
            (void)hipEventDestroy(e.a);
            (void)hipEventDestroy(e.b);
        }
        c->ev[w].clear();
    }
    return 0;
}

static int round_up(int v, int g) { return (v + g - 1) / g * g; }

static int set_device(scape_hip_ctx *c) {
    HIPCHK(hipSetDevice(c->device));
    return 0;
}

struct BusyGuard {
    scape_hip_ctx *c;
    bool ok;
    explicit BusyGuard(scape_hip_ctx *ctx) : c(ctx), ok(ctx && !ctx->busy.exchange(true)) {}
    ~BusyGuard() { if (ok) c->busy.store(false); }
};
#define CTX_GUARD(c)                                                                                      \
    if (!(c)) return fail("ctx is NULL");                                                                 \
    BusyGuard busy_guard_(c);                                                                             \
    if (!busy_guard_.ok) return fail("handle is in use by another host thread (calls on a handle are not re-entrant)")
#define CTX_ENTER(c)                                                                                      \
    CTX_GUARD(c);                                                                                         \
    if (set_device(c)) return 1

static void fill_params(DevParams &d, double mu_f, double sigma_f, double max_unif_ws, int B,
                        const double *betas, int S, const double *s, const double *pmf, int nround) {
    memset(&d, 0, sizeof(d));
    d.mu_f = mu_f;
    d.sigma_f = sigma_f;
    d.max_unif_ws = max_unif_ws;
    d.B = B;
    d.S = S;
    d.nround = nround;
    for (int i = 0; i < B; ++i) d.betas[i] = betas[i];
    for (int i = 0; i < S; ++i) {
        d.s_dis[i] = s[i];
        d.pmf_s[i] = pmf[i];
        d.inv_s[i] = 1 / s[i];
    }
}

static int max_window(const double *th, int T, double beta) {
    int best = 1, a = 0, b = 0;
    for (int i = 0; i < T; ++i) {
        const double lo = th[i] - 3 * beta, hi = th[i] + 3 * beta;
        while (a < i && th[a] < lo) ++a;
        if (b < i) b = i;
        while (b + 1 < T && th[b + 1] <= hi) ++b;
        best = std::max(best, b - a + 1);
    }
    return best;
}

static int launch_phase_b(scape_hip_ctx *c, const DevParams &prm, int n_utr, int T_max, int Wmax,
                          const UtrDesc *d_desc, const double *d_r, const double *d_pa,
                          const double *d_theta, const int32_t *d_loglist, const double *d_AT,
                          const double *d_V, double *d_M, int all_log, int32_t *d_tile_nend) {
    if (c->d_err.ensure(sizeof(int))) return 1;
    HIPCHK(hipMemsetAsync(c->d_err.p, 0, sizeof(int), c->stream));
    const size_t lds = ((size_t)2 * prm.B * Wmax + prm.B) * sizeof(double) + (size_t)2 * (prm.B + 1) * sizeof(int) +
                       (size_t)16 * (((Wmax + 3) & ~3) + 1) * sizeof(double);
    if (lds > 150 * 1024) return fail("Phase B: window table does not fit LDS (n_beta x window too large)");
    dim3 grid((unsigned)(((n_utr + 7) / 8) * 8 * T_max));
#ifdef SCAPE_HIP_TOOLS
    const char *pe = getenv("SCAPE_HIP_PB_PROBE");
    const int probe = pe ? atoi(pe) : 0;
#else
    const int probe = 0;
#endif
    if (prm.B <= 16)
        hipLaunchKernelGGL(k_phase_b<16>, grid, dim3(256), lds, c->stream, d_desc, prm, d_r, d_pa, d_theta,
                           d_loglist, d_AT, d_V, d_M, Wmax, all_log, c->d_err.as<int>(), n_utr, T_max, d_tile_nend, probe);
    else
        hipLaunchKernelGGL(k_phase_b<1>, grid, dim3(256), lds, c->stream, d_desc, prm, d_r, d_pa, d_theta,
                           d_loglist, d_AT, d_V, d_M, Wmax, all_log, c->d_err.as<int>(), n_utr, T_max, d_tile_nend, probe);
    HIPCHK(hipGetLastError());
    return 0;
}

static int check_err_flag(scape_hip_ctx *c, const char *what);
static int finish_build(scape_hip_ctx *c) {
    if (!c->build_unchecked) return 0;
    c->build_unchecked = false;
    if (check_err_flag(c, "batch_build")) {
        c->built = false;
        return 1;
    }
    return 0;
}

static int check_err_flag(scape_hip_ctx *c, const char *what) {
    int flag = 0;
    HIPCHK(hipMemcpyAsync(&flag, c->d_err.p, sizeof(int), hipMemcpyDeviceToHost, c->stream));
    HIPCHK(hipStreamSynchronize(c->stream));
    if (flag) return fail(std::string(what) + ": device-side consistency check failed (flag " + std::to_string(flag) + ")");
    return 0;
}

using EstepClasses = std::integer_sequence<int, 4, 8, 12, 16, 24, 32, 64>;
using WideClasses = std::integer_sequence<int, 4, 8, 12, 16>;
using LabelClasses = std::integer_sequence<int, 8, 16, 32, 64>;

template <int... Cs>
constexpr int last_class(std::integer_sequence<int, Cs...>) {
    int last = 0;
    ((last = Cs), ...);
    return last;
}
static_assert(last_class(EstepClasses{}) == SCAPE_MAX_K + 1 && last_class(LabelClasses{}) == SCAPE_MAX_K + 1,
              "the largest class holds the largest kmax a call may have");
constexpr int WIDE_MAX_COLUMNS = last_class(WideClasses{});

template <int... Cs, typename F>
static bool with_column_class(std::integer_sequence<int, Cs...>, int columns, F &&f) {
    return ((columns <= Cs && (f(std::integral_constant<int, Cs>()), true)) || ...);
}

struct EmPlan {
    std::vector<int64_t> ujoff, voff, ptoff;
    std::vector<int32_t> ujlist, active, elist;
    size_t vtot = 0, pttot = 0;
    int depth = 1;
    int tiles_max = 1, max_cols_utr = 1;
    bool any_m = false;
};

static EmPlan em_plan(const std::vector<UtrDesc> &h_desc, int B, size_t nj, const int32_t *job_utr, const int32_t *job_fixed,
                      bool size_order, int depth) {
    EmPlan p;
    const int n_utr = (int)h_desc.size();
    p.depth = depth;
    p.ujoff.assign(n_utr + 1, 0);
    p.ujlist.resize(nj * depth);
    for (size_t j = 0; j < nj; ++j) p.ujoff[job_utr[j] + 1] += depth;
    for (int u = 0; u < n_utr; ++u) p.ujoff[u + 1] += p.ujoff[u];
    {
        std::vector<int64_t> fill(p.ujoff.begin(), p.ujoff.end() - 1);
        for (size_t j = 0; j < nj; ++j)
            for (int q = 0; q < depth; ++q) p.ujlist[fill[job_utr[j]]++] = (int32_t)(j * depth + q);
    }
    for (int u = 0; u < n_utr; ++u)
        if (p.ujoff[u + 1] > p.ujoff[u]) p.active.push_back(u);
    if (size_order)
        std::stable_sort(p.active.begin(), p.active.end(), [&](int32_t a, int32_t b) {
            const UtrDesc &da = h_desc[a], &db = h_desc[b];
            return (int64_t)da.T * da.Np > (int64_t)db.T * db.Np;
        });
    const int n_active = (int)p.active.size();
    for (int u : p.active) {
        p.max_cols_utr = std::max<int>(p.max_cols_utr, (int)(p.ujoff[u + 1] - p.ujoff[u]));
        p.tiles_max = std::max(p.tiles_max, (h_desc[u].T * B + MT_ROWS - 1) / MT_ROWS);
    }
    p.voff.resize(nj * depth);
    p.ptoff.resize(nj * depth);
    for (size_t j = 0; j < nj; ++j) {
        const UtrDesc &d = h_desc[job_utr[j]];
        for (int q = 0; q < depth; ++q) {
            p.voff[j * depth + q] = (int64_t)p.vtot;
            p.ptoff[j * depth + q] = (int64_t)p.pttot;
            p.vtot += (size_t)d.Np;
            p.pttot += (size_t)((d.T * B + MT_ROWS - 1) / MT_ROWS);
        }
        p.any_m = p.any_m || job_fixed[j] == 0;
    }
    p.elist.reserve(nj);
    auto jobs_of = [&](int u) {
        for (int64_t q = p.ujoff[u]; q < p.ujoff[u + 1]; q += depth) p.elist.push_back(p.ujlist[q] / depth);
    };
    if (size_order && n_active >= 8) {
        for (int x = 0; x < 8; ++x)
            for (int k = x; k < n_active; k += 8) jobs_of(p.active[k]);
    } else {
        for (int u = 0; u < n_utr; ++u) jobs_of(u);
    }
    return p;
}

struct EmSwitches {
    bool size_order, debug, fine, mstep_v2, mstep_v3;
    int split_maxtiles, wide_maxjobs;
    int depth;
};
static EmSwitches em_switches() {
    const char *env_m = getenv("SCAPE_HIP_MSTEP"), *env_r = getenv("SCAPE_HIP_SPLIT_MAXTILES"), *env_w = getenv("SCAPE_HIP_WIDE_MAXJOBS");
    EmSwitches s;
    s.size_order = !getenv("SCAPE_HIP_NO_SIZE_ORDER");
    s.debug = getenv("SCAPE_HIP_DEBUG") != nullptr;
    s.fine = getenv("SCAPE_HIP_ROUND_TIMING") != nullptr;
    s.mstep_v2 = env_m && strcmp(env_m, "v2") == 0;
    s.mstep_v3 = env_m && strcmp(env_m, "v3") == 0;
    s.split_maxtiles = env_r ? atoi(env_r) : 1024;
    s.wide_maxjobs = env_w ? atoi(env_w) : 1024;
    const char *env_d = getenv("SCAPE_HIP_EM_DEPTH");
    s.depth = std::min(EM_DEPTH, std::max(1, env_d ? atoi(env_d) : EM_DEPTH));
    return s;
}

struct EmKernels {
    bool wide;
    bool job_split;
    bool ring_mstep;
    bool multi_mstep;
};
static bool em_wide(const EmSwitches &sw, int n_jobs, int kmax) {
    const bool wide = n_jobs <= sw.wide_maxjobs && kmax + 1 <= WIDE_MAX_COLUMNS;
    return wide;
}

static int em_depth(const std::vector<UtrDesc> &h_desc, int B, const EmSwitches &sw, int n_jobs, int kmax, const int32_t *job_utr,
                    const int32_t *job_fixed) {
    bool any_m = false;
    size_t v1 = 0, pt1 = 0;
    std::vector<int> per_utr(h_desc.size(), 0);
    int max_jobs_utr = 1;
    for (int j = 0; j < n_jobs; ++j) {
        const UtrDesc &d = h_desc[job_utr[j]];
        any_m = any_m || job_fixed[j] == 0;
        v1 += (size_t)d.Np;
        pt1 += (size_t)((d.T * B + MT_ROWS - 1) / MT_ROWS);
        max_jobs_utr = std::max(max_jobs_utr, ++per_utr[job_utr[j]]);
    }
    if (!any_m || em_wide(sw, n_jobs, kmax)) return 1;
    int depth = sw.depth;
    while (depth > 1 && ((size_t)max_jobs_utr * depth > 1024 || v1 * depth * 8 >= ((size_t)1 << 31) || pt1 * depth >= ((size_t)1 << 31)))
        --depth;
    return depth;
}

static int em_choose(const EmPlan &p, const EmSwitches &sw, int n_jobs, int kmax, EmKernels &k) {
    k.wide = em_wide(sw, n_jobs, kmax);
    k.job_split = (long long)p.active.size() * p.tiles_max <= sw.split_maxtiles;
    k.ring_mstep = !sw.mstep_v2 && p.vtot * 8 < ((size_t)1 << 31);
    k.multi_mstep = k.ring_mstep && !k.job_split && !sw.debug && p.pttot < ((size_t)1 << 31) && !sw.mstep_v3;
    if (k.multi_mstep && M4_LDS_BYTES > 64 * 1024)
        HIPCHK(hipFuncSetAttribute(reinterpret_cast<const void *>(k4_mstep), hipFuncAttributeMaxDynamicSharedMemorySize, M4_LDS_BYTES));
    if (k.ring_mstep && M3_LDS_BYTES > 64 * 1024)
        HIPCHK(hipFuncSetAttribute(reinterpret_cast<const void *>(k3_mstep), hipFuncAttributeMaxDynamicSharedMemorySize, M3_LDS_BYTES));
    return 0;
}

static int em_upload(scape_hip_ctx *c, const EmPlan &p, size_t nj, int kmax) {
    EmBufs &e = c->em;
    const size_t nc = nj * p.depth;
    if (e.ensure(nj, nc, kmax, c->n_utr, p.vtot, p.pttot)) return 1;
    HIPCHK(hipMemcpyAsync(e.elist.p, p.elist.data(), nj * 4, hipMemcpyHostToDevice, c->stream));
    if (!p.active.empty())
        HIPCHK(hipMemcpyAsync(e.active.p, p.active.data(), p.active.size() * 4, hipMemcpyHostToDevice, c->stream));
    HIPCHK(hipMemcpyAsync(e.voff.p, p.voff.data(), nc * 8, hipMemcpyHostToDevice, c->stream));
    HIPCHK(hipMemcpyAsync(e.ptoff.p, p.ptoff.data(), nc * 8, hipMemcpyHostToDevice, c->stream));
    HIPCHK(hipMemcpyAsync(e.ujoff.p, p.ujoff.data(), p.ujoff.size() * 8, hipMemcpyHostToDevice, c->stream));
    HIPCHK(hipMemcpyAsync(e.ujlist.p, p.ujlist.data(), nc * 4, hipMemcpyHostToDevice, c->stream));
    HIPCHK(hipStreamSynchronize(c->stream));
    return 0;
}

template <typename Kernel, typename... Round>
static void launch_estep(scape_hip_ctx *c, Kernel kernel, unsigned threads, const EmState &S, int kmax, const int32_t *job_list,
                         int n_jobs, Round... round) {
    hipLaunchKernelGGL(kernel, dim3((unsigned)(((n_jobs + 7) / 8) * 8)), dim3(threads), 0, c->stream, c->d_desc.as<UtrDesc>(),
                       c->prm, c->d_cnt.as<double>(), c->d_M.as<double>(), kmax, c->j_utr.as<int32_t>(), c->j_K.as<int32_t>(),
                       c->j_fixed.as<int32_t>(), c->j_a.as<int32_t>(), c->j_b.as<int32_t>(), c->j_ws.as<double>(),
                       c->j_karr.as<int8_t>(), S, c->j_ao.as<int32_t>(), c->j_bo.as<int32_t>(), c->j_wso.as<double>(),
                       c->j_bic.as<double>(), c->j_nlb.as<int32_t>(), c->j_lb.as<double>(),
                       c->d_counters.as<unsigned long long>(), round..., job_list, n_jobs);
}

template <typename Kernel>
static void launch_estep_slots(scape_hip_ctx *c, Kernel kernel, const EmState &S, int kmax, const int32_t *job_list, int n_jobs,
                               int r, int slots, int depth) {
    for (int slot = 0; slot < slots; ++slot) launch_estep(c, kernel, 64, S, kmax, job_list, n_jobs, r, slot, depth);
}

template <typename Kernel, typename... Tail>
static void launch_mstep(scape_hip_ctx *c, Kernel kernel, unsigned grid_y, unsigned threads, size_t lds, const EmState &S,
                         int n_active, int extent, Tail... tail) {
    hipLaunchKernelGGL(kernel, dim3((unsigned)(((n_active + 7) / 8) * 8 * extent), grid_y), dim3(threads), lds, c->stream,
                       c->d_desc.as<UtrDesc>(), c->prm, c->d_M.as<double>(), c->em.active.as<int32_t>(), n_active, extent,
                       c->em.ujoff.as<int64_t>(), c->em.ujlist.as<int32_t>(), S.V, S.Vsuf, S.voff, S.rd_m, S.rd_lo, S.rd_hi,
                       S.rd_lw, S.rd_sv, S.rd_n0, S.rd_n1, S.ptoff, S.pt_score, S.pt_row, c->d_tile_nend.as<int32_t>(),
                       c->d_counters.as<unsigned long long>(), tail...);
}

static int em_debug_round(scape_hip_ctx *c, int r, int nround) {
    unsigned long long *dbg = c->em.dbg.as<unsigned long long>();
    if (r < nround) {
        unsigned long long shard[64], tb = 0;
        HIPCHK(hipMemcpy(shard, c->d_counters.as<unsigned long long>() + CNT_MSTEP_TENSOR, sizeof(shard), hipMemcpyDeviceToHost));
        for (int i = 0; i < 64; ++i) tb += shard[i];
        fprintf(stderr, "[em bytes %d] %llu\n", r, tb);
    }
    if (r == 0 || r == 10 || r == 25 || r == nround - 1) {
        unsigned long long h[24];
        HIPCHK(hipMemcpy(h, dbg, sizeof(h), hipMemcpyDeviceToHost));
        fprintf(stderr, "[em round %d] job-halfchunks own-support %llu, union %llu, padded to groups %llu; sorted-by-n1 groups %llu\n", r, h[16], h[17], h[18], h[19]);
        fprintf(stderr, "[em round %d] tiles %llu active %llu sum_cnt %llu passes %llu | G-hist:", r, h[0], h[1], h[2], h[3]);
        for (int i = 4; i < 16; ++i) fprintf(stderr, " %llu", h[i]);
        fprintf(stderr, "\n");
        HIPCHK(hipMemsetAsync(dbg, 0, 24 * sizeof(unsigned long long), c->stream));
    }
    return 0;
}

static int em_rounds(scape_hip_ctx *c, const EmPlan &p, const EmSwitches &sw, const EmKernels &k, int n_jobs, int kmax) {
    const EmState S = c->em.state();
    const int nround = c->prm.nround, n_active = (int)p.active.size();
    const int32_t *jl = c->em.elist.as<int32_t>();
    unsigned long long *dbg = nullptr;
    if (sw.debug) {
        if (c->em.dbg.ensure(24 * sizeof(unsigned long long))) return 1;
        dbg = c->em.dbg.as<unsigned long long>();
        HIPCHK(hipMemsetAsync(dbg, 0, 24 * sizeof(unsigned long long), c->stream));
    }
    if (!p.any_m) {
        if (sw.fine && ev_begin(c, 4)) return 1;
        if (!with_column_class(EstepClasses{}, kmax + 1, [&](auto cm) {
                launch_estep(c, k2_estep_all_rounds<decltype(cm)::value>, 64, S, kmax, c->em.ujlist.as<int32_t>(), n_jobs);
            }))
            return fail("no E-step kernel for kmax " + std::to_string(kmax));
        HIPCHK(hipGetLastError());
        if (sw.fine && ev_end(c, 4)) return 1;
        return 0;
    }
    const int jobs_per_pass = k.job_split ? 16 : MT_MAXJ;
    const unsigned psplit = k.job_split ? (unsigned)std::min(64, (p.max_cols_utr + 15) / 16) : 1u;
    unsigned long long executed_prev = 0;
    const int probe_mask = (n_jobs >= 8192 && p.depth == 1) ? 7 : 3;
    for (int r = 0; r <= nround; ++r) {
        if (sw.fine && ev_begin(c, 4)) return 1;
        const bool launched =
            k.wide ? with_column_class(WideClasses{}, kmax + 1, [&](auto cm) {
                         launch_estep(c, k2_estep_cs<decltype(cm)::value>, 256, S, kmax, jl, n_jobs, r);
                     })
                   : with_column_class(EstepClasses{}, kmax + 1, [&](auto cm) {
                         launch_estep_slots(c, k2_estep<decltype(cm)::value>, S, kmax, jl, n_jobs, r, r < nround ? p.depth : 1, p.depth);
                     });
        if (!launched) return fail("no E-step kernel for kmax " + std::to_string(kmax));
        HIPCHK(hipGetLastError());
        if (sw.fine && ev_end(c, 4)) return 1;
        if (r < nround) {
            if (sw.fine && ev_begin(c, 5)) return 1;
            if (k.multi_mstep)
                launch_mstep(c, k4_mstep, 1u, 64 * M4_NW, M4_LDS_BYTES, S, n_active, (p.tiles_max + M4_TPW - 1) / M4_TPW);
            else if (k.ring_mstep)
                launch_mstep(c, k3_mstep, psplit, 256, M3_LDS_BYTES, S, n_active, p.tiles_max, jobs_per_pass, dbg);
            else
                launch_mstep(c, k2_mstep, psplit, 256, 0, S, n_active, p.tiles_max, jobs_per_pass, dbg);
            c->h_traffic[3] += 1;
            HIPCHK(hipGetLastError());
            if (sw.fine && ev_end(c, 5)) return 1;
        }
        if (r < nround && (r & probe_mask) == probe_mask) {
            unsigned long long executed = 0, shard[64];
            HIPCHK(hipMemcpyAsync(shard, c->d_counters.as<unsigned long long>() + CNT_EXEC, sizeof(shard),
                                  hipMemcpyDeviceToHost, c->stream));
            HIPCHK(hipStreamSynchronize(c->stream));
            for (int i = 0; i < 64; ++i) executed += shard[i];
            if (executed == executed_prev) break;
            executed_prev = executed;
        }
        if (sw.debug && em_debug_round(c, r, nround)) return 1;
    }
    return 0;
}

static int em_lockstep(scape_hip_ctx *c, int n_jobs, int kmax, const int32_t *job_utr, const int32_t *job_fixed) {
    const EmSwitches sw = em_switches();
    const int depth = em_depth(c->h_desc, c->prm.B, sw, n_jobs, kmax, job_utr, job_fixed);
    const EmPlan plan = em_plan(c->h_desc, c->prm.B, (size_t)n_jobs, job_utr, job_fixed, sw.size_order, depth);
    EmKernels kernels;
    if (em_choose(plan, sw, n_jobs, kmax, kernels) || em_upload(c, plan, (size_t)n_jobs, kmax)) return 1;
    return em_rounds(c, plan, sw, kernels, n_jobs, kmax);
}

static void report_release(scape_hip_ctx *c);

extern "C" {

int scape_hip_abi_version(void) { return SCAPE_HIP_ABI_VERSION; }
const char *scape_hip_last_error(void) { return g_err.c_str(); }

int scape_hip_device_count(int *count) {
    if (!count) return fail("count is NULL");
    HIPCHK(hipGetDeviceCount(count));
    return 0;
}

int scape_hip_create(int device, scape_hip_ctx **out) {
    if (!out) return fail("out is NULL");
    int n = 0;
    HIPCHK(hipGetDeviceCount(&n));
    if (device < 0 || device >= n) return fail("no such HIP device: " + std::to_string(device));
    HIPCHK(hipSetDevice(device));
    scape_hip_ctx *c = new scape_hip_ctx();
    c->device = device;
    hipDeviceProp_t prop;
    HIPCHK(hipGetDeviceProperties(&prop, device));
    snprintf(c->name, sizeof(c->name), "%s (%s, %d CUs)", prop.name, prop.gcnArchName, prop.multiProcessorCount);
    HIPCHK(hipStreamCreate(&c->stream));
    if (c->d_counters.ensure(N_COUNTERS * sizeof(unsigned long long))) return 1;
    *out = c;
    return 0;
}

int scape_hip_device_name(scape_hip_ctx *c, char *buf, int buflen) {
    if (!c || !buf || buflen <= 0) return fail("bad argument");
    snprintf(buf, buflen, "%s", c->name);
    return 0;
}

int scape_hip_batch_free(scape_hip_ctx *c) {
    if (!c) return fail("ctx is NULL");
    CTX_ENTER(c);
    DevBuf *all[] = {&c->d_tbi, &c->d_tbG, &c->d_tbpm, &c->d_mlog, &c->d_logbin, &c->d_tile_nend, &c->d_x, &c->d_l, &c->d_r, &c->d_pa, &c->d_cnt, &c->d_theta, &c->d_desc, &c->d_loglist,
                     &c->d_AT, &c->d_V, &c->d_M, &c->j_utr, &c->j_K, &c->j_fixed, &c->j_a, &c->j_b, &c->j_ws,
                     &c->j_karr, &c->j_ao, &c->j_bo, &c->j_wso, &c->j_bic, &c->j_nlb, &c->j_lb, &c->l_utr,
                     &c->l_K, &c->l_a, &c->l_b, &c->l_ws, &c->l_labels, &c->j_sel, &c->j_lbsel};
    for (DevBuf *b : all) b->release();
    c->em.release();
    c->last_em_jobs = 0;
    c->loaded = c->built = c->build_unchecked = false;
    c->n_utr = 0;
    return 0;
}

int scape_hip_destroy(scape_hip_ctx *c) {
    if (!c) return 0;
    (void)hipSetDevice(c->device);
    (void)hipStreamSynchronize(c->stream);
    scape_hip_batch_free(c);
    report_release(c);
    c->d_err.release();
    c->d_counters.release();
    for (int w = 0; w < 6; ++w)
        for (auto &e : c->ev[w]) {
            (void)hipEventDestroy(e.a);
            (void)hipEventDestroy(e.b);
        }
    (void)hipStreamDestroy(c->stream);
    delete c;
    return 0;
}

static int op_common(scape_hip_ctx *c, int n, const double *const *in, int n_in, double **dev, double **dout) {
    if (!c) return fail("ctx is NULL");
    if (n < 0) return fail("negative length");
    if (set_device(c)) return 1;
    for (int i = 0; i < n_in; ++i) {
        if (!in[i] && n > 0) return fail("NULL input array");
        HIPCHK(hipMalloc((void **)&dev[i], std::max<size_t>(16, (size_t)n * sizeof(double))));
        if (n) HIPCHK(hipMemcpyAsync(dev[i], in[i], (size_t)n * sizeof(double), hipMemcpyHostToDevice, c->stream));
    }
    HIPCHK(hipMalloc((void **)dout, std::max<size_t>(16, (size_t)n * sizeof(double))));
    return 0;
}
static int op_finish(scape_hip_ctx *c, int n, double **dev, int n_in, double *dout, double *out) {
    int rc = 0;
    hipError_t e = hipGetLastError();
    if (e != hipSuccess) rc = fail(std::string("kernel launch: ") + hipGetErrorString(e));
    if (!rc && n) {
        e = hipMemcpyAsync(out, dout, (size_t)n * sizeof(double), hipMemcpyDeviceToHost, c->stream);
        if (e != hipSuccess) rc = fail(std::string("copy back: ") + hipGetErrorString(e));
    }
    e = hipStreamSynchronize(c->stream);
    if (!rc && e != hipSuccess) rc = fail(std::string("sync: ") + hipGetErrorString(e));
    for (int i = 0; i < n_in; ++i) (void)hipFree(dev[i]);
    (void)hipFree(dout);
    return rc;
}

int scape_hip_loglik_xlr_t_pa(scape_hip_ctx *c, const double *x, const double *l, const double *pa,
                              int32_t n, double theta, double sigma_f, double *out) {
    CTX_GUARD(c);
    const double *in[3] = {x, l, pa};
    double *dev[3] = {nullptr, nullptr, nullptr}, *dout = nullptr;
    if (op_common(c, n, in, 3, dev, &dout)) return 1;
    if (n) hipLaunchKernelGGL(k_op_pa, dim3((n + 255) / 256), dim3(256), 0, c->stream, dev[0], dev[1], dev[2], n, theta, sigma_f, dout);
    return op_finish(c, n, dev, 3, dout, out);
}

int scape_hip_loglik_xlr_t_r_known(scape_hip_ctx *c, const double *x, const double *l, const double *r,
                                   int32_t n, const double *s_dis, const double *pmf_s, int32_t n_s,
                                   double theta, double mu_f, double sigma_f, double *out) {
    CTX_GUARD(c);
    if (n_s < 1 || n_s > SCAPE_MAX_S) return fail("n_s out of range");
    DevParams P;
    fill_params(P, mu_f, sigma_f, 0, 0, nullptr, n_s, s_dis, pmf_s, 0);
    const double *in[3] = {x, l, r};
    double *dev[3] = {nullptr, nullptr, nullptr}, *dout = nullptr;
    if (op_common(c, n, in, 3, dev, &dout)) return 1;
    if (n) hipLaunchKernelGGL(k_op_r_known, dim3((n + 255) / 256), dim3(256), 0, c->stream, dev[0], dev[1], dev[2], n, P, theta, dout);
    return op_finish(c, n, dev, 3, dout, out);
}

int scape_hip_loglik_xlr_t_r_unknown(scape_hip_ctx *c, const double *x, const double *l, const double *r,
                                     int32_t n, const double *s_dis, const double *pmf_s, int32_t n_s,
                                     double theta, double mu_f, double sigma_f, double *out) {
    CTX_GUARD(c);
    (void)r;
    if (n_s < 1 || n_s > SCAPE_MAX_S) return fail("n_s out of range");
    DevParams P;
    fill_params(P, mu_f, sigma_f, 0, 0, nullptr, n_s, s_dis, pmf_s, 0);
    const double *in[2] = {x, l};
    double *dev[2] = {nullptr, nullptr}, *dout = nullptr;
    if (op_common(c, n, in, 2, dev, &dout)) return 1;
    if (n) hipLaunchKernelGGL(k_op_r_unknown, dim3((n + 255) / 256), dim3(256), 0, c->stream, dev[0], dev[1], n, P, theta, dout);
    return op_finish(c, n, dev, 2, dout, out);
}

int scape_hip_get_loglik_marginal_tensor(scape_hip_ctx *c, const double *all_theta, int32_t T,
                                         const double *betas, int32_t B, const double *A, int32_t N,
                                         double *out) {
    if (!c) return fail("ctx is NULL");
    if (T < 1 || N < 1) return fail("empty theta grid or no fragments");
    if (B < 1 || B > SCAPE_MAX_BETA) return fail("n_beta out of range");
    if (!all_theta || !betas || !A || !out) return fail("NULL argument");
    CTX_ENTER(c);
    if (finish_build(c)) return 1;
    for (int i = 1; i < T; ++i)
        if (!(all_theta[i] >= all_theta[i - 1])) return fail("all_theta must be ascending");
    DevParams P;
    fill_params(P, 0, 1, 0, B, betas, 0, nullptr, nullptr, 0);
    const int Np = round_up(N, PITCH);
    double bmax = betas[0];
    for (int j = 1; j < B; ++j) bmax = std::max(bmax, betas[j]);
    const int Wmax = max_window(all_theta, T, bmax);
    std::vector<double> at((size_t)T * Np, 0.0);
    for (int n = 0; n < N; ++n)
        for (int t = 0; t < T; ++t) at[(size_t)t * Np + n] = A[(size_t)n * T + t];
    UtrDesc d;
    memset(&d, 0, sizeof(d));
    d.N = N;
    d.Np = Np;
    d.T = T;
    DevBuf dAT, dM, dth, ddesc;
    int rc = 0;
    if (dAT.ensure(at.size() * sizeof(double)) || dM.ensure((size_t)T * B * Np * sizeof(double)) ||
        dth.ensure((size_t)T * sizeof(double)) || ddesc.ensure(sizeof(UtrDesc)))
        return 1;
    hipError_t e;
    e = hipMemcpyAsync(dAT.p, at.data(), at.size() * sizeof(double), hipMemcpyHostToDevice, c->stream);
    if (e == hipSuccess) e = hipMemcpyAsync(dth.p, all_theta, (size_t)T * sizeof(double), hipMemcpyHostToDevice, c->stream);
    if (e == hipSuccess) e = hipMemcpyAsync(ddesc.p, &d, sizeof(d), hipMemcpyHostToDevice, c->stream);
    if (e != hipSuccess) return fail(std::string("upload: ") + hipGetErrorString(e));
    rc = launch_phase_b(c, P, 1, T, Wmax, ddesc.as<UtrDesc>(), nullptr, nullptr, dth.as<double>(), nullptr,
                        dAT.as<double>(), nullptr, dM.as<double>(), 1, nullptr);
    if (!rc) rc = check_err_flag(c, "get_loglik_marginal_tensor");
    if (!rc) {
        e = hipMemcpy2DAsync(out, (size_t)N * sizeof(double), dM.p, (size_t)Np * sizeof(double),
                             (size_t)N * sizeof(double), (size_t)T * B, hipMemcpyDeviceToHost, c->stream);
        if (e == hipSuccess) e = hipStreamSynchronize(c->stream);
        if (e != hipSuccess) rc = fail(std::string("copy back: ") + hipGetErrorString(e));
    }
    return rc;
}

int scape_hip_batch_load(scape_hip_ctx *c, const scape_hip_params *p, int32_t n_utr, const int64_t *bin_off,
                         const double *x, const double *l, const double *r, const double *pa,
                         const double *cnt, const int64_t *theta_off, const double *all_theta,
                         const double *utr_L, const double *min_theta, const double *unif_ll) {
    if (!c || !p) return fail("NULL ctx/params");
    if (n_utr < 1 || n_utr > 65535) return fail("n_utr must be in [1, 65535] per batch");
    if (p->n_beta < 1 || p->n_beta > SCAPE_MAX_BETA) return fail("n_beta out of range");
    if (p->n_s < 1 || p->n_s > SCAPE_MAX_S) return fail("n_s out of range");
    if (p->nround < 1 || p->nround > 127) return fail("nround out of range");
    if (!bin_off || !x || !l || !r || !pa || !cnt || !theta_off || !all_theta || !utr_L || !min_theta || !unif_ll)
        return fail("NULL array argument");
    CTX_ENTER(c);
    HIPCHK(hipStreamSynchronize(c->stream));
    c->loaded = c->built = c->build_unchecked = false;
    fill_params(c->prm, p->mu_f, p->sigma_f, p->max_unif_ws, p->n_beta, p->betas, p->n_s, p->s_dis, p->pmf_s, p->nround);
    double bmax = p->betas[0];
    for (int j = 1; j < p->n_beta; ++j) bmax = std::max(bmax, p->betas[j]);

    c->h_desc.assign(n_utr, UtrDesc());
    std::vector<int32_t> loglist;
    size_t at_total = 0, m_total = 0, tiles_total = 0, mlog_total = 0;
    std::vector<int32_t> logbin_utr;
    bool pb_slide = p->n_beta <= 16;
    int T_max = 0, Np_max = 0, W_max = 1, tiles_max_all = 1;
    for (int u = 0; u < n_utr; ++u) {
        UtrDesc &d = c->h_desc[u];
        const int64_t N = bin_off[u + 1] - bin_off[u], T = theta_off[u + 1] - theta_off[u];
        if (N < 1 || T < 1 || N > (1 << 26) || T > 65535) return fail("UTR " + std::to_string(u) + ": bad n_frag / n_theta");
        const double *th = all_theta + theta_off[u];
        for (int64_t i = 1; i < T; ++i)
            if (!(th[i] >= th[i - 1])) return fail("UTR " + std::to_string(u) + ": all_theta must be ascending");
        d.bin_off = bin_off[u];
        d.theta_off = theta_off[u];
        d.N = (int)N;
        d.Np = round_up((int)N, PITCH);
        d.T = (int)T;
        d.at_off = (int64_t)at_total;
        d.m_off = (int64_t)m_total;
        d.log_off = (int64_t)loglist.size();
        d.tile_off = (int64_t)tiles_total;
        {
            const int nt = (int)((T * p->n_beta + TILE_ROWS - 1) / TILE_ROWS);
            tiles_total += (size_t)nt;
            tiles_max_all = std::max(tiles_max_all, nt);
        }
        for (int64_t n = 0; n < N; ++n)
            if (!std::isnan(pa[bin_off[u] + n]) || !std::isnan(r[bin_off[u] + n])) loglist.push_back((int32_t)n);
        d.n_log = (int)(loglist.size() - (size_t)d.log_off);
        d.mlog_off = (int64_t)mlog_total;
        if (d.n_log > 0 && d.n_log <= PB_LOGCAP) mlog_total += (size_t)T * p->n_beta * d.n_log;
        logbin_utr.insert(logbin_utr.end(), (size_t)d.n_log, (int32_t)u);
        {
            d.c_lo = 1;
            d.c_hi = 0;
            const double step0 = (T > 1) ? th[1] - th[0] : 0.0;
            bool uni = step0 > 0.0;
            for (int64_t i = 0; i < T && uni; ++i) uni = std::floor(th[i]) == th[i] && (i == 0 || th[i] - th[i - 1] == step0);
            if (uni) {
                const int rmax = (int)std::floor(3 * bmax / step0) + 1;
                d.c_lo = rmax + 1;
                d.c_hi = (int)T - 2 - rmax;
            }
            if (d.c_lo > d.c_hi) pb_slide = false;
        }
        d.unif_ll = unif_ll[u];
        d.L = utr_L[u];
        d.min_theta = min_theta[u];
        at_total += (size_t)T * d.Np;
        m_total += (size_t)T * p->n_beta * d.Np;
        T_max = std::max(T_max, d.T);
        Np_max = std::max(Np_max, d.Np);
        W_max = std::max(W_max, max_window(th, d.T, bmax));
    }
    const int64_t nb = bin_off[n_utr], nt = theta_off[n_utr];
    c->n_utr = n_utr;
    c->n_bins = nb;
    c->T_max = T_max;
    c->Np_max = Np_max;
    c->W_max = W_max;
    c->at_total = at_total;
    c->m_total = m_total;
    c->tiles_total = tiles_total;
    c->tiles_max_all = tiles_max_all;
    c->n_theta_total = (size_t)nt;
    c->mlog_total = mlog_total;
    c->n_logbins = logbin_utr.size();
    c->pb_slide = pb_slide && W_max <= 4 * PB_STEPS && T_max <= 4096;
    const bool trace_load = getenv("SCAPE_HIP_DEBUG") != nullptr;
    const auto t_alloc0 = std::chrono::steady_clock::now();
    if (c->d_x.ensure(nb * 8) || c->d_l.ensure(nb * 8) || c->d_r.ensure(nb * 8) || c->d_pa.ensure(nb * 8) ||
        c->d_cnt.ensure(nb * 8) || c->d_theta.ensure(nt * 8) || c->d_desc.ensure(n_utr * sizeof(UtrDesc)) ||
        c->d_loglist.ensure(loglist.size() * 4) || c->d_AT.ensure(at_total * 8) || c->d_V.ensure(at_total * 8) ||
        c->d_M.ensure(m_total * 8) || c->d_tile_nend.ensure(tiles_total * 4))
        return 1;
    if (p->n_beta <= 16) {
        const size_t WP = (size_t)(((W_max + 3) & ~3) + 1);
        if (c->d_tbi.ensure((size_t)nt * 40 * 4) || c->d_tbG.ensure((size_t)nt * 16 * 8) || c->d_tbpm.ensure((size_t)nt * 16 * WP * 8) ||
            c->d_mlog.ensure(mlog_total * 8) || c->d_logbin.ensure(logbin_utr.size() * 4))
            return 1;
        if (!logbin_utr.empty())
            HIPCHK(hipMemcpyAsync(c->d_logbin.p, logbin_utr.data(), logbin_utr.size() * 4, hipMemcpyHostToDevice, c->stream));
    }
    const auto t_up0 = std::chrono::steady_clock::now();
    HIPCHK(hipMemcpyAsync(c->d_x.p, x, nb * 8, hipMemcpyHostToDevice, c->stream));
    HIPCHK(hipMemcpyAsync(c->d_l.p, l, nb * 8, hipMemcpyHostToDevice, c->stream));
    HIPCHK(hipMemcpyAsync(c->d_r.p, r, nb * 8, hipMemcpyHostToDevice, c->stream));
    HIPCHK(hipMemcpyAsync(c->d_pa.p, pa, nb * 8, hipMemcpyHostToDevice, c->stream));
    HIPCHK(hipMemcpyAsync(c->d_cnt.p, cnt, nb * 8, hipMemcpyHostToDevice, c->stream));
    HIPCHK(hipMemcpyAsync(c->d_theta.p, all_theta, nt * 8, hipMemcpyHostToDevice, c->stream));
    HIPCHK(hipMemcpyAsync(c->d_desc.p, c->h_desc.data(), n_utr * sizeof(UtrDesc), hipMemcpyHostToDevice, c->stream));
    if (!loglist.empty())
        HIPCHK(hipMemcpyAsync(c->d_loglist.p, loglist.data(), loglist.size() * 4, hipMemcpyHostToDevice, c->stream));
    HIPCHK(hipStreamSynchronize(c->stream));
    if (trace_load) {
        const auto t1 = std::chrono::steady_clock::now();
        fprintf(stderr, "scape_hip_batch_load: %d UTRs, tensors %.2f GB, device buffers (re)allocated in %.1f ms, uploads %.1f ms\n", n_utr,
                (double)(m_total + 2 * at_total) * 8e-9, std::chrono::duration<double, std::milli>(t_up0 - t_alloc0).count(),
                std::chrono::duration<double, std::milli>(t1 - t_up0).count());
    }
    c->loaded = true;
    return 0;
}

int scape_hip_batch_bytes(scape_hip_ctx *c, int64_t *bytes_batch, int64_t *bytes_free, int64_t *bytes_total) {
    if (!c) return fail("ctx is NULL");
    CTX_ENTER(c);
    size_t f = 0, t = 0;
    HIPCHK(hipMemGetInfo(&f, &t));
    if (bytes_batch)
        *bytes_batch = c->loaded ? (int64_t)((2 * c->at_total + c->m_total) * 8 + c->n_bins * 40 + c->em.V.cap + c->em.Vsuf.cap +
                                             c->em.pt_score.cap + c->em.pt_row.cap)
                                 : 0;
    if (bytes_free) *bytes_free = (int64_t)f;
    if (bytes_total) *bytes_total = (int64_t)t;
    return 0;
}

int scape_hip_batch_phase_b_form(scape_hip_ctx *c, int32_t *form) {
    if (!c || !form) return fail("ctx / form is NULL");
    *form = c->pb_form;
    return 0;
}

int scape_hip_batch_build(scape_hip_ctx *c) {
    if (!c) return fail("ctx is NULL");
    if (!c->loaded) return fail("no batch loaded");
    CTX_ENTER(c);
    if (finish_build(c)) return 1;
    dim3 grid((c->Np_max + 255) / 256, (c->T_max + PA_TT - 1) / PA_TT, c->n_utr);
    if (ev_begin(c, 0)) return 1;
    hipLaunchKernelGGL(k_phase_a, grid, dim3(256), 0, c->stream, c->d_desc.as<UtrDesc>(), c->prm, c->d_x.as<double>(),
                       c->d_l.as<double>(), c->d_r.as<double>(), c->d_pa.as<double>(), c->d_theta.as<double>(),
                       c->d_AT.as<double>(), c->d_V.as<double>());
    HIPCHK(hipGetLastError());
    if (ev_end(c, 0)) return 1;
    if (ev_begin(c, 1)) return 1;
    HIPCHK(hipMemsetAsync(c->d_tile_nend.p, 0, c->tiles_total * 4, c->stream));
    const char *pbm = getenv("SCAPE_HIP_PHASE_B");
    const bool pb_v2 = pbm && strcmp(pbm, "v2") == 0, pb_split = pbm && strcmp(pbm, "split") == 0;
    if (c->prm.B <= 16 && !pb_v2 && (pb_split || c->pb_slide)) {
        const bool slide = c->pb_slide && !pb_split;
        c->pb_form = slide ? 2 : 1;
        if (c->d_err.ensure(sizeof(int))) return 1;
        HIPCHK(hipMemsetAsync(c->d_err.p, 0, sizeof(int), c->stream));
        const int Wmax = c->W_max, WP = ((Wmax + 3) & ~3) + 1, B = c->prm.B;
        const size_t lds_t = ((size_t)B * Wmax + 16) * sizeof(double) + 32 * sizeof(int);
        const size_t lds_l = ((size_t)16 * WP + 16 * PB_LOGCAP) * sizeof(double) + PB_LOGCAP * sizeof(int);
        if (lds_t > 60 * 1024 || lds_l > 60 * 1024) return fail("Phase B: window table does not fit LDS (n_beta x window too large)");
        hipLaunchKernelGGL(k_pb_tables<16>, dim3((unsigned)c->T_max, (unsigned)c->n_utr), dim3(PB_TAB_THREADS), lds_t, c->stream,
                           c->d_desc.as<UtrDesc>(), c->prm, c->d_theta.as<double>(), Wmax, WP, c->d_tbi.as<int32_t>(), c->d_tbG.as<double>(),
                           c->d_tbpm.as<double>(), c->d_err.as<int>(), c->T_max, slide ? nullptr : c->d_loglist.as<int32_t>(), c->d_AT.as<double>(),
                           c->d_M.as<double>(), c->d_mlog.as<double>(), c->d_tile_nend.as<int32_t>());
        HIPCHK(hipGetLastError());
        if (slide) {
            if (c->n_logbins) {
                const size_t lds_c = ((size_t)((c->T_max + 1) & ~1) + (size_t)B * Wmax) * sizeof(double) + 16 * sizeof(int);
                hipLaunchKernelGGL(k_pb_logcol, dim3((unsigned)c->n_logbins), dim3(256), lds_c, c->stream, c->d_desc.as<UtrDesc>(), c->prm,
                                   c->d_theta.as<double>(), c->d_loglist.as<int32_t>(), c->d_logbin.as<int32_t>(), c->d_AT.as<double>(),
                                   c->d_tbi.as<int32_t>(), c->d_tbG.as<double>(), c->d_M.as<double>(), c->d_mlog.as<double>(),
                                   c->d_tile_nend.as<int32_t>(), Wmax);
                HIPCHK(hipGetLastError());
            }
            const int blocks_max = (c->Np_max + 63) / 64;
            const size_t lds_s = ((size_t)16 * WP + 4 * PB_RING * 16) * sizeof(double);
            hipLaunchKernelGGL(k_pb_slide, dim3((unsigned)(((c->n_utr + 7) / 8) * 8 * blocks_max)), dim3(256), lds_s, c->stream,
                               c->d_desc.as<UtrDesc>(), c->prm, c->d_r.as<double>(), c->d_pa.as<double>(), c->d_loglist.as<int32_t>(),
                               c->d_V.as<double>(), c->d_M.as<double>(), c->d_mlog.as<double>(), WP, c->d_tbi.as<int32_t>(),
                               c->d_tbpm.as<double>(), c->n_utr, blocks_max, c->d_tile_nend.as<int32_t>());
        } else {
            hipLaunchKernelGGL(k_phase_b_lin, dim3((unsigned)(((c->n_utr + 7) / 8) * 8 * c->T_max)), dim3(256), lds_l, c->stream,
                               c->d_desc.as<UtrDesc>(), c->prm, c->d_r.as<double>(), c->d_pa.as<double>(), c->d_loglist.as<int32_t>(),
                               c->d_V.as<double>(), c->d_M.as<double>(), c->d_mlog.as<double>(), WP, c->d_tbi.as<int32_t>(),
                               c->d_tbpm.as<double>(), c->n_utr, c->T_max, c->d_tile_nend.as<int32_t>());
        }
        HIPCHK(hipGetLastError());
    } else if ((c->pb_form = 0), launch_phase_b(c, c->prm, c->n_utr, c->T_max, c->W_max, c->d_desc.as<UtrDesc>(), c->d_r.as<double>(),
                       c->d_pa.as<double>(), c->d_theta.as<double>(), c->d_loglist.as<int32_t>(),
                       c->d_AT.as<double>(), c->d_V.as<double>(), c->d_M.as<double>(), 0, c->d_tile_nend.as<int32_t>()))
        return 1;
    if (ev_end(c, 1)) return 1;
    c->build_unchecked = true;
    c->built = true;
    if (getenv("SCAPE_HIP_SYNC_BUILD") && finish_build(c)) return 1;
    return 0;
}

int scape_hip_batch_em(scape_hip_ctx *c, int32_t n_jobs, int32_t kmax, const int32_t *job_utr,
                       const int32_t *job_K, const int32_t *job_fixed, const int32_t *alpha_idx,
                       const int32_t *beta_idx, const double *ws, const int8_t *k_arr,
                       int32_t *alpha_idx_out, int32_t *beta_idx_out, double *ws_out, double *bic_out,
                       int32_t *n_lb_out, double *lb_out) {
    if (!c) return fail("ctx is NULL");
    if (!c->built) return fail("batch_build has not run");
    if (n_jobs < 1) return fail("n_jobs < 1");
    if (kmax < 1 || kmax > SCAPE_MAX_K) return fail("kmax out of range");
    if (!job_utr || !job_K || !job_fixed || !alpha_idx || !beta_idx || !ws || !k_arr || !alpha_idx_out ||
        !beta_idx_out || !ws_out || !bic_out || !n_lb_out)
        return fail("NULL array argument");
    CTX_ENTER(c);
    c->last_em_jobs = 0;
    const int nround = c->prm.nround, B = c->prm.B;
    for (int j = 0; j < n_jobs; ++j) {
        const int u = job_utr[j], K = job_K[j];
        if (u < 0 || u >= c->n_utr) return fail("job " + std::to_string(j) + ": bad UTR index");
        if (K < 0 || K > kmax) return fail("job " + std::to_string(j) + ": K out of range");
        const int T = c->h_desc[u].T;
        for (int k = 0; k < K; ++k) {
            const int a = alpha_idx[(size_t)j * kmax + k], b = beta_idx[(size_t)j * kmax + k];
            if (a < 0 || a >= T || b < 0 || b >= B) return fail("job " + std::to_string(j) + ": alpha/beta index out of range");
            if (k > 0 && a < alpha_idx[(size_t)j * kmax + k - 1]) return fail("job " + std::to_string(j) + ": alpha indices must be non-decreasing");
        }
        for (int t = 0; t < nround; ++t) {
            const int k = k_arr[(size_t)j * nround + t];
            if (k < 0 || k > K || (K > 0 && k >= K)) return fail("job " + std::to_string(j) + ": k_arr entry out of range");
        }
    }
    {
        std::vector<int32_t> per_utr(c->n_utr, 0);
        for (int j = 0; j < n_jobs; ++j)
            if (!job_fixed[j] && ++per_utr[job_utr[j]] > SCAPE_MAX_JOBS_PER_UTR)
                return fail("UTR " + std::to_string(job_utr[j]) + ": more than " + std::to_string(SCAPE_MAX_JOBS_PER_UTR) +
                            " non-fixed jobs in one call (split the call)");
    }
    const size_t nj = n_jobs;
    if (c->j_utr.ensure(nj * 4) || c->j_K.ensure(nj * 4) || c->j_fixed.ensure(nj * 4) || c->j_a.ensure(nj * kmax * 4) ||
        c->j_b.ensure(nj * kmax * 4) || c->j_ws.ensure(nj * (kmax + 1) * 8) || c->j_karr.ensure(nj * nround) ||
        c->j_ao.ensure(nj * kmax * 4) || c->j_bo.ensure(nj * kmax * 4) || c->j_wso.ensure(nj * (kmax + 1) * 8) ||
        c->j_bic.ensure(nj * 8) || c->j_nlb.ensure(nj * 4) || c->j_lb.ensure(nj * nround * 8))
        return 1;
    HIPCHK(hipMemcpyAsync(c->j_utr.p, job_utr, nj * 4, hipMemcpyHostToDevice, c->stream));
    HIPCHK(hipMemcpyAsync(c->j_K.p, job_K, nj * 4, hipMemcpyHostToDevice, c->stream));
    HIPCHK(hipMemcpyAsync(c->j_fixed.p, job_fixed, nj * 4, hipMemcpyHostToDevice, c->stream));
    HIPCHK(hipMemcpyAsync(c->j_a.p, alpha_idx, nj * kmax * 4, hipMemcpyHostToDevice, c->stream));
    HIPCHK(hipMemcpyAsync(c->j_b.p, beta_idx, nj * kmax * 4, hipMemcpyHostToDevice, c->stream));
    HIPCHK(hipMemcpyAsync(c->j_ws.p, ws, nj * (kmax + 1) * 8, hipMemcpyHostToDevice, c->stream));
    HIPCHK(hipMemcpyAsync(c->j_karr.p, k_arr, nj * nround, hipMemcpyHostToDevice, c->stream));
    HIPCHK(hipMemsetAsync(c->d_counters.p, 0, N_COUNTERS * sizeof(unsigned long long), c->stream));
    HIPCHK(hipMemsetAsync(c->j_lb.p, 0, nj * nround * 8, c->stream));
    c->h_traffic[3] = 0;
    if (ev_begin(c, 2)) return 1;
    if (em_lockstep(c, n_jobs, kmax, job_utr, job_fixed)) return 1;
    if (ev_end(c, 2)) return 1;
    HIPCHK(hipMemcpyAsync(alpha_idx_out, c->j_ao.p, nj * kmax * 4, hipMemcpyDeviceToHost, c->stream));
    HIPCHK(hipMemcpyAsync(beta_idx_out, c->j_bo.p, nj * kmax * 4, hipMemcpyDeviceToHost, c->stream));
    HIPCHK(hipMemcpyAsync(ws_out, c->j_wso.p, nj * (kmax + 1) * 8, hipMemcpyDeviceToHost, c->stream));
    HIPCHK(hipMemcpyAsync(bic_out, c->j_bic.p, nj * 8, hipMemcpyDeviceToHost, c->stream));
    HIPCHK(hipMemcpyAsync(n_lb_out, c->j_nlb.p, nj * 4, hipMemcpyDeviceToHost, c->stream));
    if (lb_out) HIPCHK(hipMemcpyAsync(lb_out, c->j_lb.p, nj * nround * 8, hipMemcpyDeviceToHost, c->stream));
    unsigned long long hc[N_COUNTERS];
    HIPCHK(hipMemcpyAsync(hc, c->d_counters.p, sizeof(hc), hipMemcpyDeviceToHost, c->stream));
    HIPCHK(hipStreamSynchronize(c->stream));
    if (finish_build(c)) return 1;
    c->last_em_jobs = n_jobs;
#ifdef M4_STAMPS
    {
        const unsigned long long *st = hc + 4 + 5 * 64 + 16;
        for (int ga = 0; ga < 4; ++ga)
            for (int role = 0; role < 2; ++role) {
                const double n = (double)st[32 + ga * 2 + role];
                const unsigned long long *v = st + 4 * (ga * 2 + role);
                if (n > 0)
                    fprintf(stderr, "[mstep stamps] %d running groups, %s wavefronts: %.3g iterations; mean cycles: dma wait %.0f, barrier %.0f, issue %.0f, reads+mfma %.0f (total %.0f)\n",
                            ga + 1, role ? "vector" : "tile", n, v[0] / n, v[1] / n, v[2] / n, v[3] / n, (v[0] + v[1] + v[2] + v[3]) / n);
            }
    }
#endif
#ifdef ESTEP_STAMPS
    {
        const unsigned long long *st = hc + 4 + 5 * 64;
        const double n = (double)st[7];
        if (n > 0)
            fprintf(stderr, "[estep stamps] job-rounds %.0f; mean cycles: set-up %.0f, bin loop %.0f, reductions+weights %.0f, suffix sums %.0f, tail %.0f (total %.0f)\n",
                    n, st[0] / n, st[1] / n, st[2] / n, st[3] / n, st[4] / n, (st[0] + st[1] + st[2] + st[3] + st[4]) / n);
    }
#endif
    for (int i = 0; i < 3; ++i) c->h_counters[i] = hc[i];
    c->h_traffic[0] = c->h_traffic[1] = c->h_traffic[2] = 0;
    for (int i = 0; i < 64; ++i) {
        c->h_counters[1] += hc[CNT_SLAB + i];
        c->h_traffic[0] += hc[CNT_MSTEP_TENSOR + i];
        c->h_traffic[1] += hc[CNT_MSTEP_VREQ + i];
        c->h_traffic[2] += hc[CNT_MSTEP_VUNI + i];
    }
    return 0;
}

__global__ void k_gather_rows(const double *__restrict__ src, const int32_t *__restrict__ idx, double *__restrict__ dst,
                              int rowlen, int n_sel) {
    const int i = blockIdx.x * blockDim.x + threadIdx.x;
    if (i < n_sel * rowlen) dst[i] = src[(size_t)idx[i / rowlen] * rowlen + i % rowlen];
}

int scape_hip_batch_em_fetch_lb(scape_hip_ctx *c, int32_t n_sel, const int32_t *job_idx, double *lb_out) {
    if (!c) return fail("ctx is NULL");
    if (n_sel < 1 || !job_idx || !lb_out) return fail("fetch_lb: bad arguments");
    CTX_ENTER(c);
    if (finish_build(c)) return 1;
    if (c->last_em_jobs < 1) return fail("fetch_lb: no completed scape_hip_batch_em call on this handle");
    for (int i = 0; i < n_sel; ++i)
        if (job_idx[i] < 0 || job_idx[i] >= c->last_em_jobs) return fail("fetch_lb: job index out of range");
    const int nround = c->prm.nround;
    if (c->j_sel.ensure((size_t)n_sel * 4) || c->j_lbsel.ensure((size_t)n_sel * nround * 8)) return 1;
    HIPCHK(hipMemcpyAsync(c->j_sel.p, job_idx, (size_t)n_sel * 4, hipMemcpyHostToDevice, c->stream));
    hipLaunchKernelGGL(k_gather_rows, dim3((unsigned)((n_sel * nround + 255) / 256)), dim3(256), 0, c->stream,
                       c->j_lb.as<double>(), c->j_sel.as<int32_t>(), c->j_lbsel.as<double>(), nround, n_sel);
    HIPCHK(hipGetLastError());
    HIPCHK(hipMemcpyAsync(lb_out, c->j_lbsel.p, (size_t)n_sel * nround * 8, hipMemcpyDeviceToHost, c->stream));
    HIPCHK(hipStreamSynchronize(c->stream));
    return 0;
}

int scape_hip_batch_labels(scape_hip_ctx *c, int32_t n_sel, int32_t kmax, const int32_t *sel_utr,
                           const int32_t *sel_K, const int32_t *alpha_idx, const int32_t *beta_idx,
                           const double *ws, int32_t *labels_out) {
    if (!c) return fail("ctx is NULL");
    if (!c->built) return fail("batch_build has not run");
    if (n_sel < 1) return fail("n_sel < 1");
    if (kmax < 1 || kmax > SCAPE_MAX_K) return fail("kmax out of range");
    if (!sel_utr || !sel_K || !alpha_idx || !beta_idx || !ws || !labels_out) return fail("NULL array argument");
    CTX_ENTER(c);
    const int B = c->prm.B;
    for (int j = 0; j < n_sel; ++j) {
        const int u = sel_utr[j], K = sel_K[j];
        if (u < 0 || u >= c->n_utr) return fail("labels: bad UTR index");
        if (K < 0 || K > kmax) return fail("labels: K out of range");
        for (int k = 0; k < K; ++k) {
            const int a = alpha_idx[(size_t)j * kmax + k], b = beta_idx[(size_t)j * kmax + k];
            if (a < 0 || a >= c->h_desc[u].T || b < 0 || b >= B) return fail("labels: alpha/beta index out of range");
        }
    }
    const size_t ns = n_sel;
    if (c->l_utr.ensure(ns * 4) || c->l_K.ensure(ns * 4) || c->l_a.ensure(ns * kmax * 4) || c->l_b.ensure(ns * kmax * 4) ||
        c->l_ws.ensure(ns * (kmax + 1) * 8) || c->l_labels.ensure((size_t)c->n_bins * 4))
        return 1;
    HIPCHK(hipMemcpyAsync(c->l_utr.p, sel_utr, ns * 4, hipMemcpyHostToDevice, c->stream));
    HIPCHK(hipMemcpyAsync(c->l_K.p, sel_K, ns * 4, hipMemcpyHostToDevice, c->stream));
    HIPCHK(hipMemcpyAsync(c->l_a.p, alpha_idx, ns * kmax * 4, hipMemcpyHostToDevice, c->stream));
    HIPCHK(hipMemcpyAsync(c->l_b.p, beta_idx, ns * kmax * 4, hipMemcpyHostToDevice, c->stream));
    HIPCHK(hipMemcpyAsync(c->l_ws.p, ws, ns * (kmax + 1) * 8, hipMemcpyHostToDevice, c->stream));
    if (ev_begin(c, 3)) return 1;
    if (!with_column_class(LabelClasses{}, kmax + 1, [&](auto cm) {
            hipLaunchKernelGGL(k_labels<decltype(cm)::value>, dim3(n_sel), dim3(256), 0, c->stream, c->d_desc.as<UtrDesc>(), c->prm,
                               c->d_cnt.as<double>(), c->d_M.as<double>(), kmax, c->l_utr.as<int32_t>(), c->l_K.as<int32_t>(),
                               c->l_a.as<int32_t>(), c->l_b.as<int32_t>(), c->l_ws.as<double>(), c->l_labels.as<int32_t>());
        }))
        return fail("no label kernel for kmax " + std::to_string(kmax));
    HIPCHK(hipGetLastError());
    if (ev_end(c, 3)) return 1;
    {
        std::vector<char> sel(c->n_utr, 0);
        for (int j = 0; j < n_sel; ++j) sel[sel_utr[j]] = 1;
        int u = 0;
        while (u < c->n_utr) {
            if (!sel[u]) {
                ++u;
                continue;
            }
            int v = u;
            while (v + 1 < c->n_utr && sel[v + 1]) ++v;
            const int64_t b0 = c->h_desc[u].bin_off, b1 = c->h_desc[v].bin_off + c->h_desc[v].N;
            HIPCHK(hipMemcpyAsync(labels_out + b0, c->l_labels.as<int32_t>() + b0, (size_t)(b1 - b0) * 4,
                                  hipMemcpyDeviceToHost, c->stream));
            u = v + 1;
        }
    }
    HIPCHK(hipStreamSynchronize(c->stream));
    if (finish_build(c)) return 1;
    return 0;
}

int scape_hip_batch_fetch_loglik(scape_hip_ctx *c, int32_t utr, double *A_out) {
    if (!c || !A_out) return fail("NULL argument");
    if (!c->built) return fail("batch_build has not run");
    if (utr < 0 || utr >= c->n_utr) return fail("bad UTR index");
    CTX_ENTER(c);
    if (finish_build(c)) return 1;
    const UtrDesc &d = c->h_desc[utr];
    std::vector<double> at((size_t)d.T * d.Np);
    HIPCHK(hipMemcpy(at.data(), c->d_AT.as<double>() + d.at_off, at.size() * 8, hipMemcpyDeviceToHost));
    for (int n = 0; n < d.N; ++n)
        for (int t = 0; t < d.T; ++t) A_out[(size_t)n * d.T + t] = at[(size_t)t * d.Np + n];
    return 0;
}

int scape_hip_batch_fetch_tensor(scape_hip_ctx *c, int32_t utr, double *M_out) {
    if (!c || !M_out) return fail("NULL argument");
    if (!c->built) return fail("batch_build has not run");
    if (utr < 0 || utr >= c->n_utr) return fail("bad UTR index");
    CTX_ENTER(c);
    if (finish_build(c)) return 1;
    const UtrDesc &d = c->h_desc[utr];
    HIPCHK(hipMemcpy2D(M_out, (size_t)d.N * 8, c->d_M.as<double>() + d.m_off, (size_t)d.Np * 8, (size_t)d.N * 8,
                       (size_t)d.T * c->prm.B, hipMemcpyDeviceToHost));
    return 0;
}

int scape_hip_timing_reset(scape_hip_ctx *c) {
    if (!c) return fail("ctx is NULL");
    CTX_ENTER(c);
    if (ev_collect(c)) return 1;
    for (int w = 0; w < 6; ++w) {
        c->ms_acc[w] = 0;
        c->n_acc[w] = 0;
    }
    return 0;
}

int scape_hip_timing_get(scape_hip_ctx *c, int32_t which, double *ms_total, int32_t *n_launches) {
    if (!c) return fail("ctx is NULL");
    if (which < 0 || which > 5) return fail("which out of range");
    CTX_ENTER(c);
    if (ev_collect(c)) return 1;
    if (ms_total) *ms_total = c->ms_acc[which];
    if (n_launches) *n_launches = c->n_acc[which];
    return 0;
}

int scape_hip_em_counters(scape_hip_ctx *c, int64_t *rounds, int64_t *slab_elems, int64_t *z_elems) {
    if (!c) return fail("ctx is NULL");
    if (rounds) *rounds = (int64_t)c->h_counters[0];
    if (slab_elems) *slab_elems = (int64_t)c->h_counters[1];
    if (z_elems) *z_elems = (int64_t)c->h_counters[2];
    return 0;
}

int scape_hip_em_traffic(scape_hip_ctx *c, int64_t *mstep_tensor_bytes, int64_t *mstep_v_bytes_requested,
                         int64_t *mstep_v_bytes_unique, int64_t *mstep_launches) {
    if (!c) return fail("ctx is NULL");
    if (mstep_tensor_bytes) *mstep_tensor_bytes = (int64_t)c->h_traffic[0];
    if (mstep_v_bytes_requested) *mstep_v_bytes_requested = (int64_t)c->h_traffic[1];
    if (mstep_v_bytes_unique) *mstep_v_bytes_unique = (int64_t)c->h_traffic[2];
    if (mstep_launches) *mstep_launches = (int64_t)c->h_traffic[3];
    return 0;
}

}

#include "report.inc"
#include "perm.inc"
```

### scape_amd/engine.py

```python
from __future__ import annotations

import contextlib
import ctypes
from dataclasses import dataclass, field

import numpy as np

from . import _lib
from ._lib import Params, check, f64, i32, ptr, P_i32, P_i64, P_i8
from . import _hostlib
from .host import MODEL_DEFAULTS, N_ROUND, N_TRIAL, FastSampler, Sampler, UtrPrep


@dataclass
class Fit:
    K: int
    a_idx: np.ndarray
    b_idx: np.ndarray
    ws: np.ndarray
    bic: float
    lb: np.ndarray


@dataclass
class UtrResult:
    prep: UtrPrep
    fit: Fit = None
    labels_bin: np.ndarray = None
    n_jobs: int = 0


@dataclass
class _Job:
    u: int
    K: int
    fixed: bool
    a_idx: np.ndarray
    b_idx: np.ndarray
    ws: np.ndarray
    k_arr: np.ndarray


@dataclass
class PackedJobs:
    ju: np.ndarray
    jk: np.ndarray
    jf: np.ndarray
    a: np.ndarray
    b: np.ndarray
    w: np.ndarray
    ka: np.ndarray

    def __len__(self):
        return len(self.ju)

    @property
    def kmax(self):
        return self.a.shape[1]


def pack_jobs(jobs):
    n = len(jobs)
    kmax = max(1, max(j.K for j in jobs))
    a = np.zeros((n, kmax), dtype=np.int32)
    b = np.zeros((n, kmax), dtype=np.int32)
    w = np.zeros((n, kmax + 1), dtype=np.float64)
    ka = np.zeros((n, N_ROUND), dtype=np.int8)
    for i, j in enumerate(jobs):
        a[i, :j.K], b[i, :j.K], w[i, :j.K + 1], ka[i] = j.a_idx, j.b_idx, j.ws, j.k_arr
    return PackedJobs(i32([j.u for j in jobs]), i32([j.K for j in jobs]), i32([int(j.fixed) for j in jobs]), a, b, w, ka)


def concat_packed(packs):
    if len(packs) == 1:
        return packs[0]
    n, kmax = sum(len(p) for p in packs), max(p.kmax for p in packs)
    a, b = np.zeros((n, kmax), np.int32), np.zeros((n, kmax), np.int32)
    w = np.zeros((n, kmax + 1), np.float64)
    lo = 0
    for p in packs:
        hi, k = lo + len(p), p.kmax
        a[lo:hi, :k], b[lo:hi, :k], w[lo:hi, :k + 1] = p.a, p.b, p.w
        lo = hi
    cat = lambda name: np.concatenate([getattr(p, name) for p in packs])
    return PackedJobs(cat("ju"), cat("jk"), cat("jf"), a, b, w, cat("ka"))


class HipBatch:

    def __init__(self, ctx, preps):
        self.ctx, self.lib, self.preps = ctx, ctx.lib, preps
        p0 = preps[0]
        for q in preps[1:]:
            if not (np.array_equal(q.betas, p0.betas) and np.array_equal(q.s_dis, p0.s_dis)
                    and q.p["mu_f"] == p0.p["mu_f"] and q.p["sigma_f"] == p0.p["sigma_f"]
                    and q.p["max_unif_ws"] == p0.p["max_unif_ws"]):
                raise ValueError("all UTRs of a batch must share the model constants")
        if len(p0.betas) > _lib.MAX_BETA or len(p0.s_dis) > _lib.MAX_S:
            raise ValueError("beta / polyA-length grid too long for the HIP kernels")
        prm = Params()
        prm.mu_f, prm.sigma_f, prm.max_unif_ws = float(p0.p["mu_f"]), float(p0.p["sigma_f"]), float(p0.p["max_unif_ws"])
        prm.n_beta, prm.n_s, prm.nround = len(p0.betas), len(p0.s_dis), N_ROUND
        for i, v in enumerate(p0.betas):
            prm.betas[i] = v
        for i, (s, q) in enumerate(zip(p0.s_dis, p0.pmf_s)):
            prm.s_dis[i], prm.pmf_s[i] = s, q
        self.params = prm
        self.bin_off = np.zeros(len(preps) + 1, dtype=np.int64)
        self.theta_off = np.zeros(len(preps) + 1, dtype=np.int64)
        np.cumsum([q.N for q in preps], out=self.bin_off[1:])
        np.cumsum([q.T for q in preps], out=self.theta_off[1:])
        cat = lambda name: f64(np.concatenate([getattr(q, name) for q in preps]))
        x, l, r, pa, cnt, th = cat("x"), cat("l"), cat("r"), cat("pa"), cat("cnt"), cat("theta")
        Ls = f64([q.L for q in preps])
        mt = f64([q.min_theta for q in preps])
        ul = f64([q.unif_ll for q in preps])
        check(self.lib.scape_hip_batch_load(self.ctx.h, ctypes.byref(prm), len(preps), ptr(self.bin_off, P_i64),
                                            ptr(x), ptr(l), ptr(r), ptr(pa), ptr(cnt), ptr(self.theta_off, P_i64),
                                            ptr(th), ptr(Ls), ptr(mt), ptr(ul)), "batch_load")
        self.n_bins = int(self.bin_off[-1])

    def build(self):
        check(self.lib.scape_hip_batch_build(self.ctx.h), "batch_build")

    def phase_b_form(self):
        form = ctypes.c_int32(-1)
        check(self.lib.scape_hip_batch_phase_b_form(self.ctx.h, ctypes.byref(form)), "batch_phase_b_form")
        return int(form.value)

    def em_packed(self, pj, reuse_buffers=False, want_lb=True):
        n, kmax = len(pj), pj.kmax
        key = (n, kmax, want_lb)
        if reuse_buffers and getattr(self, "_em_buf_key", None) == key:
            ao, bo, wo, bic, nlb, lb = self._em_buf
        else:
            ao, bo = np.empty_like(pj.a), np.empty_like(pj.b)
            wo = np.empty_like(pj.w)
            bic = np.empty(n)
            nlb = np.empty(n, dtype=np.int32)
            lb = np.empty((n, N_ROUND)) if want_lb else None
            if reuse_buffers:
                self._em_buf_key, self._em_buf = key, (ao, bo, wo, bic, nlb, lb)
        check(self.lib.scape_hip_batch_em(self.ctx.h, n, kmax, ptr(pj.ju, P_i32), ptr(pj.jk, P_i32),
                                          ptr(pj.jf, P_i32), ptr(pj.a, P_i32), ptr(pj.b, P_i32), ptr(pj.w),
                                          ptr(pj.ka, P_i8), ptr(ao, P_i32), ptr(bo, P_i32), ptr(wo), ptr(bic),
                                          ptr(nlb, P_i32), ptr(lb) if want_lb else None), "batch_em")
        return ao, bo, wo, bic, nlb, lb

    def em_fetch_lb(self, job_idx):
        idx = i32(job_idx)
        out = np.empty((len(idx), N_ROUND))
        if len(idx):
            check(self.lib.scape_hip_batch_em_fetch_lb(self.ctx.h, len(idx), ptr(idx, P_i32), ptr(out)), "em_fetch_lb")
        return out

    @staticmethod
    def fit_at(pj, out, i, lb_row=None):
        ao, bo, wo, bic, nlb, lb = out
        K = int(pj.jk[i])
        row = lb[i] if lb_row is None else lb_row
        return Fit(K=K, a_idx=ao[i, :K].copy(), b_idx=bo[i, :K].copy(), ws=wo[i, :K + 1].copy(),
                   bic=float(bic[i]), lb=row[:nlb[i]].copy())

    def em(self, jobs):
        if not jobs:
            return []
        pj = pack_jobs(jobs)
        out = self.em_packed(pj)
        return [self.fit_at(pj, out, i) for i in range(len(jobs))]

    def timing(self, which):
        ms, n = ctypes.c_double(), ctypes.c_int32()
        check(self.lib.scape_hip_timing_get(self.ctx.h, which, ctypes.byref(ms), ctypes.byref(n)), "timing_get")
        return ms.value, n.value

    def em_counters(self):
        r, s, z = ctypes.c_int64(), ctypes.c_int64(), ctypes.c_int64()
        check(self.lib.scape_hip_em_counters(self.ctx.h, ctypes.byref(r), ctypes.byref(s), ctypes.byref(z)),
              "em_counters")
        return r.value, s.value, z.value

    def em_traffic(self):
        t, vr, vu, n = ctypes.c_int64(), ctypes.c_int64(), ctypes.c_int64(), ctypes.c_int64()
        check(self.lib.scape_hip_em_traffic(self.ctx.h, ctypes.byref(t), ctypes.byref(vr), ctypes.byref(vu),
                                            ctypes.byref(n)), "em_traffic")
        return dict(tensor_bytes=t.value, v_bytes_requested=vr.value, v_bytes_unique=vu.value, launches=n.value)

    def labels(self, sel):
        if not sel:
            return {}
        n = len(sel)
        kmax = max(1, max(f.K for _, f in sel))
        su = i32([u for u, _ in sel])
        sk = i32([f.K for _, f in sel])
        a = np.zeros((n, kmax), dtype=np.int32)
        b = np.zeros((n, kmax), dtype=np.int32)
        w = np.zeros((n, kmax + 1), dtype=np.float64)
        for i, (_, f) in enumerate(sel):
            a[i, :f.K], b[i, :f.K], w[i, :f.K + 1] = f.a_idx, f.b_idx, f.ws
        out = np.full(self.n_bins, -1, dtype=np.int32)
        check(self.lib.scape_hip_batch_labels(self.ctx.h, n, kmax, ptr(su, P_i32), ptr(sk, P_i32), ptr(a, P_i32),
                                              ptr(b, P_i32), ptr(w), ptr(out, P_i32)), "batch_labels")
        return {u: out[self.bin_off[u]:self.bin_off[u + 1]].copy() for u, _ in sel}

    def labels_packed(self, su, sk, a, b, w):
        su, sk, a, b = i32(su), i32(sk), i32(a), i32(b)
        w = f64(w)
        out = np.full(self.n_bins, -1, dtype=np.int32)
        check(self.lib.scape_hip_batch_labels(self.ctx.h, len(su), a.shape[1], ptr(su, P_i32), ptr(sk, P_i32),
                                              ptr(a, P_i32), ptr(b, P_i32), ptr(w), ptr(out, P_i32)), "batch_labels")
        return out

    def fetch_loglik(self, u):
        q = self.preps[u]
        A = np.zeros((q.N, q.T))
        check(self.lib.scape_hip_batch_fetch_loglik(self.ctx.h, u, ptr(A)), "fetch_loglik")
        return A

    def fetch_tensor(self, u):
        q = self.preps[u]
        M = np.zeros((q.T, len(q.betas), q.N))
        check(self.lib.scape_hip_batch_fetch_tensor(self.ctx.h, u, ptr(M)), "fetch_tensor")
        return M

    def free(self):
        check(self.lib.scape_hip_batch_free(self.ctx.h), "batch_free")


def _no_component_left(q):
    raise IndexError(f"{q.gene_info_str}: every pA component has weight < min_ws={q.p['min_ws']} "
                     "(the reference's rm_component fails here too: arrays used as indices must be of integer "
                     "(or boolean) type, apa_core.py:838-839)")


class _Sweep:

    def __init__(self, u, prep, sampler, re_run_mode, trace=None):
        self.u, self.prep, self.sampler, self.re_run = u, prep, sampler, re_run_mode
        self.n_max, self.n_min = prep.p["n_max_apa"], prep.p["n_min_apa"]
        self.stage = "sweep"
        self.best = None
        self.done = False
        self.n_jobs = 0
        self.trace = trace
        self.pred = None

    def prune_K(self):
        f = self.best
        return int(np.count_nonzero(~(f.ws[:f.K] < self.prep.p["min_ws"])))

    def make_jobs(self, predrawn=None):
        q = self.prep
        jobs = []
        if self.stage == "sweep":
            for K in range(self.n_max, self.n_min - 1, -1):
                for _ in range(N_TRIAL):
                    a, b, w, ka = self.sampler.init_job(q, K)
                    jobs.append(_Job(self.u, K, False, a, b, w, ka))
        elif self.stage == "prune":
            f = self.best
            keep = np.array([i for i in range(f.K) if not f.ws[i] < q.p["min_ws"]], dtype=int)
            Kp = len(keep)
            if Kp == 0:
                _no_component_left(q)
            if predrawn is not None:
                w, ka = predrawn
            else:
                w = self.sampler.init_ws(Kp, q.p["max_unif_ws"])
                ka = self.sampler.k_arr(Kp)
            jobs.append(_Job(self.u, Kp, True, f.a_idx[keep].astype(np.int32), f.b_idx[keep].astype(np.int32), w, ka))
        self.n_jobs += len(jobs)
        return jobs

    def make_packed(self, tables=None, predrawn=None):
        q = self.prep
        if predrawn is not None:
            return pack_jobs(self.make_jobs(predrawn))
        if self.stage == "sweep" and hasattr(self.sampler, "sweep"):
            jk, a, b, w, ka = tables if tables is not None else self.sampler.sweep(q, self.n_max, self.n_min)
            n = len(jk)
            self.n_jobs += n
            return PackedJobs(np.full(n, self.u, np.int32), jk, np.zeros(n, np.int32), a, b, w, ka)
        return pack_jobs(self.make_jobs())

    @staticmethod
    def make_packed_many(sweeps):
        idx = [i for i, sw in enumerate(sweeps) if sw.stage == "sweep" and isinstance(sw.sampler, FastSampler)]
        if len(idx) < 2 or len({id(sweeps[i].sampler) for i in idx}) != len(idx):
            return [sw.make_packed() for sw in sweeps]
        tabs = FastSampler.sweep_many([(sweeps[i].sampler, sweeps[i].prep, sweeps[i].n_max, sweeps[i].n_min) for i in idx])
        by = dict(zip(idx, tabs))
        return [sw.make_packed(by.get(i)) for i, sw in enumerate(sweeps)]

    def absorb_packed(self, pj, out, lo, hi):
        if self.stage == "sweep":
            with np.errstate(over="ignore"):
                grid = out[3][lo:hi].astype(np.float32).reshape(-1, N_TRIAL)
            tb = np.argmin(grid, axis=1)
            kb = int(np.argmin(grid[np.arange(len(tb)), tb]))
            self.best = HipBatch.fit_at(pj, out, lo + kb * N_TRIAL + int(tb[kb]))
            if not self.prep.fixed_run and np.any(self.best.ws[:self.best.K] < self.prep.p["min_ws"]):
                self.stage = "prune"
                return
        elif self.stage == "prune":
            self.best = HipBatch.fit_at(pj, out, lo)
        self._after_fit()

    def absorb(self, fits):
        q = self.prep
        if self.trace is not None:
            self.trace.extend(fits)
        if self.stage == "sweep":
            per_k = []
            for i in range(0, len(fits), N_TRIAL):
                grp = fits[i:i + N_TRIAL]
                per_k.append(grp[int(np.argmin(np.array([f.bic for f in grp], dtype=np.float32)))])
            self.best = per_k[int(np.argmin(np.array([f.bic for f in per_k], dtype=np.float32)))]
            if not q.fixed_run and any(self.best.ws[i] < q.p["min_ws"] for i in range(self.best.K)):
                self.stage = "prune"
                return
        elif self.stage == "prune":
            self.best = fits[0]
        self._after_fit()

    def set_sweep_winner(self, best, n_jobs):
        self.best = best
        self.n_jobs += n_jobs
        if not self.prep.fixed_run and any(best.ws[i] < self.prep.p["min_ws"] for i in range(best.K)):
            self.stage = "prune"
            return
        self._after_fit()

    def _after_fit(self):
        if self.re_run and not self.prep.fixed_run and self.best.K == self.n_max:
            if self.n_max + 2 > _lib.MAX_K:
                import sys
                sys.stderr.write(f"scape_amd: {self.prep.gene_info_str}: K reached n_max_apa={self.n_max} and the "
                                 f"next sweep would exceed the library's K <= {_lib.MAX_K}; keeping K={self.best.K} "
                                 "(the reference would re-run with n_max_apa + 2)\n")
                self.done = True
                return
            self.n_min = self.n_max
            self.n_max = self.n_max + 2
            self.stage = "sweep"
            return
        self.done = True


class Engine:
    defer_prunes = True

    def __init__(self, device=None, mem_fraction=0.7, own_context=False):
        if own_context:
            if device is None:
                device = _lib.default_context(None).device
            self.ctx = _lib.Context(device)
        else:
            self.ctx = _lib.default_context(device)
        self.mem_fraction = mem_fraction
        self.own_context = own_context
        self.sweep_lock = None

    def _budget(self):
        fb, tb, bb = ctypes.c_int64(), ctypes.c_int64(), ctypes.c_int64()
        check(self.ctx.lib.scape_hip_batch_bytes(self.ctx.h, ctypes.byref(bb), ctypes.byref(fb), ctypes.byref(tb)),
              "batch_bytes")
        return int(fb.value * self.mem_fraction)

    EM_DEPTH = 3

    @staticmethod
    def utr_bytes(q):
        npad = (q.N + 15) // 16 * 16
        p = getattr(q, "p", None) or MODEL_DEFAULTS
        jobs = N_TRIAL * max(1, p["n_max_apa"] - p["n_min_apa"] + 1)
        return 8 * npad * q.T * (len(q.betas) + 2) + 48 * q.N + (Engine.EM_DEPTH - 1) * jobs * npad * 17 // 2

    def close(self):
        if self.own_context:
            self.ctx.close()

    def load(self, preps):
        return HipBatch(self.ctx, preps)

    def waves(self, preps):
        budget = self._budget()
        out, cur, used = [], [], 0
        for i, q in enumerate(preps):
            b = self.utr_bytes(q)
            if b > budget:
                raise _lib.ScapeHipError(f"UTR {q.gene_info_str}: marginal tensor ({b >> 20} MiB) exceeds device memory")
            if cur and (used + b > budget or len(cur) >= 65535):
                out.append(cur)
                cur, used = [], 0
            cur.append(i)
            used += b
        if cur:
            out.append(cur)
        return out

    def run(self, preps, rng_mode="reference", seed=1, re_run_mode=True, rs=None, keep_trace=False, seeds=None):
        if rng_mode not in ("reference", "per_utr"):
            raise ValueError("rng_mode must be 'reference' or 'per_utr'")
        results = [UtrResult(prep=q) for q in preps]
        if seeds is None:
            seeds = [(seed + i) % (2 ** 32) for i in range(len(preps))]
        shared = FastSampler(rs if rs is not None else np.random.RandomState(seed)) if rng_mode == "reference" else None
        self.traces = [[] for _ in preps] if keep_trace else None
        for wave in self.waves(preps):
            wp = [preps[i] for i in wave]
            batch = HipBatch(self.ctx, wp)
            if rng_mode == "reference" or keep_trace or any(q.fixed_run for q in wp):
                batch.build()
                sweeps = []
                for u, gi in enumerate(wave):
                    smp = shared if shared is not None else FastSampler(np.random.RandomState(seeds[gi]))
                    sweeps.append(_Sweep(u, preps[gi], smp, re_run_mode, self.traces[gi] if keep_trace else None))
                if rng_mode == "reference":
                    deferred = []
                    if keep_trace:
                        for sw in sweeps:
                            self._drive(batch, [sw], deferred)
                    else:
                        depth = self._stream_depth(1)
                        if depth > 1:
                            self._predict_outcomes(batch, wp, sweeps, re_run_mode)
                        self._drive_streams(batch, [(shared, sweeps)], deferred, depth=depth)
                    self._finish_deferred(batch, deferred)
                else:
                    self._drive(batch, sweeps)
                labs = batch.labels([(sw.u, sw.best) for sw in sweeps])
                out = [(sw.best, labs[sw.u], sw.n_jobs) for sw in sweeps]
            else:
                plan = self.plan(wp, [seeds[gi] for gi in wave])
                out = self.process(batch, wp, plan, re_run_mode)
            for (fit, lab, nj), gi in zip(out, wave):
                results[gi].fit, results[gi].labels_bin, results[gi].n_jobs = fit, lab, nj
        if shared is not None:
            shared.rs
        return results

    def run_streams(self, streams, re_run_mode=True):
        out = [None] * len(streams)
        ready = [(si, preps, seed) for si, (preps, seed) in enumerate(streams)]

        def take(block, room):
            got = ready[:room]
            del ready[:room]
            return got
        self.run_streams_rolling(take, lambda: bool(ready), lambda si, res: out.__setitem__(si, res), re_run_mode,
                                 streams_in_flight=max(1, len(streams)))
        return out

    stream_wave_utrs = 16
    stream_wave_min = 512

    def run_streams_rolling(self, take, more, on_done, re_run_mode=True, streams_in_flight=128):
        full = self._budget()
        budget = min(full, Engine.stream_wave_bytes)
        active = []
        while active or more():
            room = streams_in_flight - len(active)
            if room > 0 and more():
                for tag, preps, seed in take(not active, room):
                    st = [tag, preps, FastSampler(np.random.RandomState(seed)), 0, [UtrResult(prep=q) for q in preps]]
                    if len(preps):
                        active.append(st)
                    else:
                        on_done(tag, [])
            if not active:
                continue
            wave, used, stop = [], 0, False
            per_stream = max(Engine.stream_wave_utrs, -(-Engine.stream_wave_min // len(active)))
            for turn in range(per_stream):
                took = False
                for st in active:
                    i = st[3]
                    if i >= len(st[1]) or len(wave) >= 65535:
                        continue
                    bts = self.utr_bytes(st[1][i])
                    if bts > full:
                        raise _lib.ScapeHipError("a UTR's marginal tensor exceeds device memory")
                    if wave and used + bts > budget:
                        stop = True
                        break
                    wave.append((st, i))
                    st[3] = i + 1
                    used += bts
                    took = True
# ... 452 lines not shown
```

Baseline: 3440 UTRs/s.

## Skip M-step tiles with no live E-step output and drop run-ahead slots

The E-step now stamps each row tile it touches with the current pass, and the multi-tile M-step exits early when none of its tiles were stamped this pass, avoiding tensor reads for converged or idle jobs. A host-side check marks which jobs can ever run ahead. The E-step launches with a single slot when no job can, or once every run-ahead-capable job has finished, as seen through a device counter read at the existing probe. This adds per-pass tile writes, an extra descriptor hidden in the pend buffer, and more host preparation and upload work per EM call.

Result: no change. 3473 UTRs/s, median of 6 (+1.0%).

```diff
diff --git a/include/scape_hip.h b/include/scape_hip.h
--- a/include/scape_hip.h
+++ b/include/scape_hip.h
@@ -81,6 +81,7 @@
 
 int scape_hip_em_traffic(scape_hip_ctx *ctx, int64_t *mstep_tensor_bytes, int64_t *mstep_v_bytes_requested,
                          int64_t *mstep_v_bytes_unique, int64_t *mstep_launches);
+int scape_hip_em_live_skip(scape_hip_ctx *ctx, int64_t *estep_launches, int64_t *mstep_stamp_exits);
 
 int scape_hip_report_counts(scape_hip_ctx *ctx, int32_t n_rec, const int64_t *read_off, const int32_t *K,
                             const int64_t *label, const int64_t *cb_id, int64_t id_min, int64_t id_span,
diff --git a/scape_amd/_lib.py b/scape_amd/_lib.py
--- a/scape_amd/_lib.py
+++ b/scape_amd/_lib.py
@@ -56,6 +56,7 @@
     "scape_hip_timing_get": (c_i, [P_void, c_i32, P_d, P_i32]),
     "scape_hip_em_counters": (c_i, [P_void, P_i64, P_i64, P_i64]),
     "scape_hip_em_traffic": (c_i, [P_void, P_i64, P_i64, P_i64, P_i64]),
+    "scape_hip_em_live_skip": (c_i, [P_void, P_i64, P_i64]),
     "scape_hip_report_counts": (c_i, [P_void, c_i32, P_i64, P_i32, P_i64, P_i64, c_i64, c_i64, P_i32, c_i32,
                                       P_i64, P_i8, P_i64]),
     "scape_hip_report_render": (c_i, [P_void, c_i32, c_i32, P_i64, P_i8, P_i64, ctypes.c_char_p, P_i64]),
diff --git a/scape_amd/csrc/em_lockstep.inc b/scape_amd/csrc/em_lockstep.inc
--- a/scape_amd/csrc/em_lockstep.inc
+++ b/scape_amd/csrc/em_lockstep.inc
@@ -18,9 +18,13 @@
 #endif
 #define CNT_SLAB 4
 #define CNT_EXEC (4 + 64)
-#define CNT_MSTEP_TENSOR (4 + 2 * 64)
-#define CNT_MSTEP_VREQ (4 + 3 * 64)
-#define CNT_MSTEP_VUNI (4 + 4 * 64)
+#define CNT_RA_DONE (4 + 2 * 64)
+#define CNT_MSTEP_TENSOR (4 + 3 * 64)
+#define CNT_MSTEP_VREQ (4 + 4 * 64)
+#define CNT_MSTEP_VUNI (4 + 5 * 64)
+#define CNT_LIVE_EXIT (4 + 6 * 64)
+#define CNT_STAMPS (4 + 7 * 64)
+#define N_COUNTERS (CNT_STAMPS + 16 + 48)
 static_assert(MT_ROWS == TILE_ROWS, "tile height must match k_tile_extent / the host tables");
 static_assert(MT_MAXJ <= 64, "the per-pass job setup gives one job to each lane of one wavefront");
 
@@ -39,7 +43,22 @@
     double *pt_score;
     int32_t *pt_row;
     const int64_t *ptoff;
+    int32_t *tile_pass;
 };
+
+struct EmLive {
+    int32_t *tile_pass;
+    const int8_t *can_ra;
+    const int32_t *job_tile;
+    void *reserved;
+};
+static_assert(sizeof(EmLive) == 4 * sizeof(unsigned long long), "EmBufs keeps the record in the first four words of the pend buffer");
+__device__ __forceinline__ const EmLive *em_live(const EmState &S) { return reinterpret_cast<const EmLive *>(S.pend) - 1; }
+
+__host__ __device__ inline void em_tile_range(int lo, int hi, int *t0, int *t1) {
+    *t0 = lo / MT_ROWS;
+    *t1 = (hi - 1) / MT_ROWS;
+}
 
 __device__ __forceinline__ double d_wave_allsum(double v) {
 #pragma unroll
@@ -131,7 +150,8 @@
         pt_best[q] = -INFINITY;
         pt_best_r[q] = pre_lo[q];
         if (pre_m[q]) {
-            const int t0 = pre_lo[q] / MT_ROWS, t1 = (pre_hi[q] - 1) / MT_ROWS;
+            int t0, t1;
+            em_tile_range(pre_lo[q], pre_hi[q], &t0, &t1);
             for (int t = t0 + lane; t <= t1; t += 64) {
                 const double sc = S.pt_score[pre_ptoff[q] + t];
                 const int rr = S.pt_row[pre_ptoff[q] + t];
@@ -635,7 +655,7 @@
 #ifdef ESTEP_STAMPS
     if (NW == 1 && lane == 0) {
         const unsigned long long st5 = __builtin_amdgcn_s_memtime();
-        unsigned long long *sp = counters + 4 + 5 * 64;
+        unsigned long long *sp = counters + CNT_STAMPS;
         atomicAdd(&sp[0], st1 - st0);
         atomicAdd(&sp[1], st2 - st1);
         atomicAdd(&sp[2], st3 - st2);
@@ -698,6 +718,39 @@
 __host__ __device__ inline bool em_run_ahead_stops(int status, int nlb, int nround, int k_next, unsigned long long pend) {
     return status != 0 || nlb >= nround || (pend & (7ull << k_next)) != 0ull;
 }
+template <typename KT>
+__host__ __device__ inline bool em_can_run_ahead(const KT *k_arr, int nround, int K, bool fixed) {
+    if (fixed) return false;
+    for (int i = 0; i + 1 < nround; ++i) {
+        const int k = k_arr[i];
+        const unsigned long long pend = (k < K) ? 2ull << k : 0ull;
+        if (!em_run_ahead_stops(0, i + 1, nround, k_arr[i + 1], pend)) return true;
+    }
+    return false;
+}
+#define ESTEP_LIVE_TAIL(COL, PASS)                                                                 \
+    {                                                                                              \
+        const EmLive *Lp = em_live(S);                                                             \
+        if (nx.pub_k >= 0 || nx.status == 2) {                                                     \
+            const EmLive L = *Lp;                                                                  \
+            if (nx.pub_k >= 0 && L.tile_pass) {                                                    \
+                const size_t col = (COL);                                                          \
+                int lo = 0, hi = 0;                                                                \
+                if (lane == 0) {                                                                   \
+                    lo = S.rd_lo[col];                                                             \
+                    hi = S.rd_hi[col];                                                             \
+                }                                                                                  \
+                lo = __builtin_amdgcn_readfirstlane(lo);                                           \
+                hi = __builtin_amdgcn_readfirstlane(hi);                                           \
+                int t0, t1;                                                                        \
+                em_tile_range(lo, hi, &t0, &t1);                                                   \
+                int32_t *tp = L.tile_pass + L.job_tile[job];                                       \
+                for (int t = t0 + lane; t <= t1; t += 64) tp[t] = (PASS) + 1;                      \
+            }                                                                                      \
+            if (lane == 0 && nx.status == 2 && L.can_ra && L.can_ra[job])                          \
+                atomicAdd(&counters[CNT_RA_DONE + (job & 63)], 1ull);                              \
+        }                                                                                          \
+    }
 #define ESTEP_NW 1
 #ifndef ESTEP_WPS
 #define ESTEP_WPS 3
@@ -734,6 +787,7 @@
     d_load_exptab(s_exptab, lane, 64);
     EstepNext nx;
     ESTEP_DISPATCH(CMAX, launch, status);
+    ESTEP_LIVE_TAIL((size_t)job * depth + slot, launch)
     if (depth > 1 && lane == 0) {
         if (nx.pub_k >= 0) pend |= 2ull << nx.pub_k;
         const bool stop = em_run_ahead_stops(nx.status, nx.nlb, P.nround, nx.k_next, pend) || job_fixed[job] != 0;
@@ -803,12 +857,13 @@
     constexpr int slot = 0, depth = 1;
     EstepNext nx;
     ESTEP_DISPATCH(CMAX, round, status);
-    (void)nx;
+    if (wave == 0) ESTEP_LIVE_TAIL((size_t)job, round)
 }
 #undef ESTEP_NW
 #undef ESTEP_EXTRA
 #undef ESTEP_DISPATCH
 #undef ESTEP_CASE
+#undef ESTEP_LIVE_TAIL
 
 
 typedef double v4f64 __attribute__((ext_vector_type(4)));
diff --git a/scape_amd/csrc/mstep_multi.inc b/scape_amd/csrc/mstep_multi.inc
--- a/scape_amd/csrc/mstep_multi.inc
+++ b/scape_amd/csrc/mstep_multi.inc
@@ -170,7 +170,8 @@
                                                         double *__restrict__ pt_score,
                                                         int32_t *__restrict__ pt_row,
                                                         const int32_t *__restrict__ tile_nend,
-                                                        unsigned long long *__restrict__ counters) {
+                                                        unsigned long long *__restrict__ counters,
+                                                        const int32_t *__restrict__ tile_pass, int pass) {
     extern __shared__ __attribute__((aligned(16))) double m4_lds[];
     double *area = m4_lds;
     double *x_ps = m4_lds + M4_AREA_BYTES / 8;
@@ -201,6 +202,16 @@
     if (t_first * MT_ROWS >= nrows) return;
     const int n_tiles = min(M4_TPW, (nrows - t_first * MT_ROWS + MT_ROWS - 1) / MT_ROWS);
     const int tid = threadIdx.x, lane = tid & 63, wave = __builtin_amdgcn_readfirstlane(tid >> 6);
+    if (tile_pass) {
+        bool live = false;
+#pragma unroll
+        for (int i = 0; i < M4_TPW; ++i)
+            if (i < n_tiles) live = live || tile_pass[d.tile_off + t_first + i] == pass + 1;
+        if (!live) {
+            if (tid == 0) atomicAdd(&counters[CNT_LIVE_EXIT + (blockIdx.x & 63)], 1ull);
+            return;
+        }
+    }
     const double *Mu = M + (size_t)d.m_off;
     const int64_t jlo = ujob_off[u], jhi = ujob_off[u + 1];
 
@@ -357,7 +368,7 @@
             }
         }
 #ifdef M4_STAMPS
-        T.stamps = counters + (4 + 5 * 64 + 16);
+        T.stamps = counters + (CNT_STAMPS + 16);
 #endif
         T.tb0 = m3_uniform_ptr(Mu + (size_t)row0 * Np + n_lo);
         T.vb0 = m3_uniform_ptr(V + n_lo);
diff --git a/scape_amd/csrc/scape_hip.hip b/scape_amd/csrc/scape_hip.hip
--- a/scape_amd/csrc/scape_hip.hip
+++ b/scape_amd/csrc/scape_hip.hip
@@ -651,32 +651,34 @@
 struct EmBufs {
     DevBuf ia, ib, sia, sib, ws, slw, lb, ell, nlb, status, pend, rd_k, rd_lo, rd_hi, rd_m, rd_n0, rd_n1, rd_lw, rd_sv, V, Vsuf,
         voff, pt_score, pt_row, ptoff;
+    DevBuf tile_pass, job_tile, can_ra;
     DevBuf ujoff, ujlist, active, elist, dbg;
     int ensure(size_t nj, size_t nc, size_t kmax, size_t n_utr, size_t vtot, size_t pttot) {
         return ia.ensure(nj * kmax * 4) || ib.ensure(nj * kmax * 4) || sia.ensure(nj * kmax * 4) || sib.ensure(nj * kmax * 4) ||
                ws.ensure(nj * (kmax + 1) * 8) || slw.ensure(nj * (kmax + 1) * 8) || lb.ensure(nj * 8) || ell.ensure(nj * 8) ||
-               nlb.ensure(nj * 4) || status.ensure(nj * 4) || pend.ensure(nj * 8) || rd_k.ensure(nc * 4) || rd_lo.ensure(nc * 4) ||
+               nlb.ensure(nj * 4) || status.ensure(nj * 4) || pend.ensure(sizeof(EmLive) + nj * 8) || rd_k.ensure(nc * 4) || rd_lo.ensure(nc * 4) ||
                rd_hi.ensure(nc * 4) || rd_m.ensure(nc * 4) || rd_n0.ensure(nc * 4) || rd_n1.ensure(nc * 4) ||
                rd_lw.ensure(nc * 8) || rd_sv.ensure(nc * 8) || V.ensure(vtot * 8) || Vsuf.ensure((vtot / 16 + nc + 1) * 8) ||
                voff.ensure(nc * 8) || pt_score.ensure(pttot * 8) || pt_row.ensure(pttot * 4) || ptoff.ensure(nc * 8) ||
-               ujoff.ensure((n_utr + 1) * 8) || ujlist.ensure(nc * 4) || active.ensure(n_utr * 4) || elist.ensure(nj * 4);
+               ujoff.ensure((n_utr + 1) * 8) || ujlist.ensure(nc * 4) || active.ensure(n_utr * 4) || elist.ensure(nj * 4) ||
+               job_tile.ensure(nj * 4) || can_ra.ensure(nj);
     }
     EmState state() const {
         return EmState{ia.as<int32_t>(), ib.as<int32_t>(), sia.as<int32_t>(), sib.as<int32_t>(), ws.as<double>(), slw.as<double>(),
-                       lb.as<double>(), ell.as<double>(), nlb.as<int32_t>(), status.as<int32_t>(), pend.as<unsigned long long>(),
+                       lb.as<double>(), ell.as<double>(), nlb.as<int32_t>(), status.as<int32_t>(),
+                       pend.as<unsigned long long>() + sizeof(EmLive) / 8,
                        rd_k.as<int32_t>(),
                        rd_lo.as<int32_t>(), rd_hi.as<int32_t>(), rd_m.as<int32_t>(), rd_n0.as<int32_t>(), rd_n1.as<int32_t>(),
                        rd_lw.as<double>(), rd_sv.as<double>(), V.as<double>(), Vsuf.as<double>(), voff.as<int64_t>(),
-                       pt_score.as<double>(), pt_row.as<int32_t>(), ptoff.as<int64_t>()};
+                       pt_score.as<double>(), pt_row.as<int32_t>(), ptoff.as<int64_t>(), nullptr};
     }
     void release() {
         for (DevBuf *b : {&ia, &ib, &sia, &sib, &ws, &slw, &lb, &ell, &nlb, &status, &pend, &rd_k, &rd_lo, &rd_hi, &rd_m, &rd_n0, &rd_n1, &rd_lw,
-                          &rd_sv, &V, &Vsuf, &voff, &pt_score, &pt_row, &ptoff, &ujoff, &ujlist, &active, &elist, &dbg})
+                          &rd_sv, &V, &Vsuf, &voff, &pt_score, &pt_row, &ptoff, &tile_pass, &job_tile, &can_ra, &ujoff, &ujlist, &active, &elist, &dbg})
             b->release();
     }
 };
 
-#define N_COUNTERS (4 + 5 * 64 + 16 + 48)
 struct scape_hip_ctx {
     int device = 0;
     std::atomic<bool> busy{false};
@@ -705,6 +707,7 @@
     int n_acc[6] = {0, 0, 0, 0, 0, 0};
     unsigned long long h_counters[3] = {0, 0, 0};
     unsigned long long h_traffic[4] = {0, 0, 0, 0};
+    unsigned long long h_live[2] = {0, 0};
     ReportState *rep = nullptr;
 };
 
@@ -861,6 +864,11 @@
     int depth = 1;
     int tiles_max = 1, max_cols_utr = 1;
     bool any_m = false;
+    bool stamps = false;
+    bool count_ra = false;
+    std::vector<int32_t> job_tile;
+    std::vector<int8_t> can_ra;
+    long long n_can_ra = 0;
 };
 
 static EmPlan em_plan(const std::vector<UtrDesc> &h_desc, int B, size_t nj, const int32_t *job_utr, const int32_t *job_fixed,
@@ -918,6 +926,7 @@
     bool size_order, debug, fine, mstep_v2, mstep_v3;
     int split_maxtiles, wide_maxjobs;
     int depth;
+    bool live_skip;
 };
 static EmSwitches em_switches() {
     const char *env_m = getenv("SCAPE_HIP_MSTEP"), *env_r = getenv("SCAPE_HIP_SPLIT_MAXTILES"), *env_w = getenv("SCAPE_HIP_WIDE_MAXJOBS");
@@ -931,6 +940,7 @@
     s.wide_maxjobs = env_w ? atoi(env_w) : 1024;
     const char *env_d = getenv("SCAPE_HIP_EM_DEPTH");
     s.depth = std::min(EM_DEPTH, std::max(1, env_d ? atoi(env_d) : EM_DEPTH));
+    s.live_skip = !getenv("SCAPE_HIP_NO_LIVE_SKIP");
     return s;
 }
 
@@ -977,6 +987,25 @@
     return 0;
 }
 
+static void em_liveness(const std::vector<UtrDesc> &h_desc, size_t tiles_total, int nround, const EmSwitches &sw, const EmKernels &k,
+                        int n_jobs, const int32_t *job_utr, const int32_t *job_K, const int32_t *job_fixed, const int8_t *k_arr,
+                        EmPlan &p) {
+    if (!sw.live_skip || !p.any_m) return;
+    p.stamps = k.multi_mstep && tiles_total < ((size_t)1 << 31);
+    if (p.stamps) {
+        p.job_tile.resize((size_t)n_jobs);
+        for (int j = 0; j < n_jobs; ++j) p.job_tile[j] = (int32_t)h_desc[job_utr[j]].tile_off;
+    }
+    p.count_ra = !k.wide && p.depth > 1;
+    if (p.count_ra) {
+        p.can_ra.resize((size_t)n_jobs);
+        for (int j = 0; j < n_jobs; ++j) {
+            p.can_ra[j] = em_can_run_ahead(k_arr + (size_t)j * nround, nround, job_K[j], job_fixed[j] != 0) ? 1 : 0;
+            p.n_can_ra += p.can_ra[j];
+        }
+    }
+}
+
 static int em_upload(scape_hip_ctx *c, const EmPlan &p, size_t nj, int kmax) {
     EmBufs &e = c->em;
     const size_t nc = nj * p.depth;
@@ -988,6 +1017,19 @@
     HIPCHK(hipMemcpyAsync(e.ptoff.p, p.ptoff.data(), nc * 8, hipMemcpyHostToDevice, c->stream));
     HIPCHK(hipMemcpyAsync(e.ujoff.p, p.ujoff.data(), p.ujoff.size() * 8, hipMemcpyHostToDevice, c->stream));
     HIPCHK(hipMemcpyAsync(e.ujlist.p, p.ujlist.data(), nc * 4, hipMemcpyHostToDevice, c->stream));
+    EmLive live = {nullptr, nullptr, nullptr, nullptr};
+    if (p.stamps) {
+        if (e.tile_pass.ensure(c->tiles_total * 4)) return 1;
+        HIPCHK(hipMemsetAsync(e.tile_pass.p, 0, c->tiles_total * 4, c->stream));
+        HIPCHK(hipMemcpyAsync(e.job_tile.p, p.job_tile.data(), nj * 4, hipMemcpyHostToDevice, c->stream));
+        live.tile_pass = e.tile_pass.as<int32_t>();
+        live.job_tile = e.job_tile.as<int32_t>();
+    }
+    if (p.count_ra) {
+        HIPCHK(hipMemcpyAsync(e.can_ra.p, p.can_ra.data(), nj, hipMemcpyHostToDevice, c->stream));
+        live.can_ra = e.can_ra.as<int8_t>();
+    }
+    HIPCHK(hipMemcpyAsync(e.pend.p, &live, sizeof(live), hipMemcpyHostToDevice, c->stream));
     HIPCHK(hipStreamSynchronize(c->stream));
     return 0;
 }
@@ -995,6 +1037,7 @@
 template <typename Kernel, typename... Round>
 static void launch_estep(scape_hip_ctx *c, Kernel kernel, unsigned threads, const EmState &S, int kmax, const int32_t *job_list,
                          int n_jobs, Round... round) {
+    c->h_live[0] += 1;
     hipLaunchKernelGGL(kernel, dim3((unsigned)(((n_jobs + 7) / 8) * 8)), dim3(threads), 0, c->stream, c->d_desc.as<UtrDesc>(),
                        c->prm, c->d_cnt.as<double>(), c->d_M.as<double>(), kmax, c->j_utr.as<int32_t>(), c->j_K.as<int32_t>(),
                        c->j_fixed.as<int32_t>(), c->j_a.as<int32_t>(), c->j_b.as<int32_t>(), c->j_ws.as<double>(),
@@ -1040,7 +1083,8 @@
 }
 
 static int em_rounds(scape_hip_ctx *c, const EmPlan &p, const EmSwitches &sw, const EmKernels &k, int n_jobs, int kmax) {
-    const EmState S = c->em.state();
+    EmState S = c->em.state();
+    if (p.stamps) S.tile_pass = c->em.tile_pass.as<int32_t>();
     const int nround = c->prm.nround, n_active = (int)p.active.size();
     const int32_t *jl = c->em.elist.as<int32_t>();
     unsigned long long *dbg = nullptr;
@@ -1063,6 +1107,7 @@
     const unsigned psplit = k.job_split ? (unsigned)std::min(64, (p.max_cols_utr + 15) / 16) : 1u;
     unsigned long long executed_prev = 0;
     const int probe_mask = (n_jobs >= 8192 && p.depth == 1) ? 7 : 3;
+    int slots = (p.count_ra && p.n_can_ra == 0) ? 1 : p.depth;
     for (int r = 0; r <= nround; ++r) {
         if (sw.fine && ev_begin(c, 4)) return 1;
         const bool launched =
@@ -1070,7 +1115,7 @@
                          launch_estep(c, k2_estep_cs<decltype(cm)::value>, 256, S, kmax, jl, n_jobs, r);
                      })
                    : with_column_class(EstepClasses{}, kmax + 1, [&](auto cm) {
-                         launch_estep_slots(c, k2_estep<decltype(cm)::value>, S, kmax, jl, n_jobs, r, r < nround ? p.depth : 1, p.depth);
+                         launch_estep_slots(c, k2_estep<decltype(cm)::value>, S, kmax, jl, n_jobs, r, r < nround ? slots : 1, p.depth);
                      });
         if (!launched) return fail("no E-step kernel for kmax " + std::to_string(kmax));
         HIPCHK(hipGetLastError());
@@ -1078,7 +1123,8 @@
         if (r < nround) {
             if (sw.fine && ev_begin(c, 5)) return 1;
             if (k.multi_mstep)
-                launch_mstep(c, k4_mstep, 1u, 64 * M4_NW, M4_LDS_BYTES, S, n_active, (p.tiles_max + M4_TPW - 1) / M4_TPW);
+                launch_mstep(c, k4_mstep, 1u, 64 * M4_NW, M4_LDS_BYTES, S, n_active, (p.tiles_max + M4_TPW - 1) / M4_TPW,
+                             (const int32_t *)S.tile_pass, r);
             else if (k.ring_mstep)
                 launch_mstep(c, k3_mstep, psplit, 256, M3_LDS_BYTES, S, n_active, p.tiles_max, jobs_per_pass, dbg);
             else
@@ -1088,25 +1134,31 @@
             if (sw.fine && ev_end(c, 5)) return 1;
         }
         if (r < nround && (r & probe_mask) == probe_mask) {
-            unsigned long long executed = 0, shard[64];
+            static_assert(CNT_RA_DONE == CNT_EXEC + 64, "the probe reads the two counters in one copy");
+            unsigned long long executed = 0, ra_done = 0, shard[128];
             HIPCHK(hipMemcpyAsync(shard, c->d_counters.as<unsigned long long>() + CNT_EXEC, sizeof(shard),
                                   hipMemcpyDeviceToHost, c->stream));
             HIPCHK(hipStreamSynchronize(c->stream));
             for (int i = 0; i < 64; ++i) executed += shard[i];
+            for (int i = 64; i < 128; ++i) ra_done += shard[i];
             if (executed == executed_prev) break;
             executed_prev = executed;
+            if (p.count_ra && (long long)ra_done == p.n_can_ra) slots = 1;
         }
         if (sw.debug && em_debug_round(c, r, nround)) return 1;
     }
     return 0;
 }
 
-static int em_lockstep(scape_hip_ctx *c, int n_jobs, int kmax, const int32_t *job_utr, const int32_t *job_fixed) {
+static int em_lockstep(scape_hip_ctx *c, int n_jobs, int kmax, const int32_t *job_utr, const int32_t *job_K, const int32_t *job_fixed,
+                       const int8_t *k_arr) {
     const EmSwitches sw = em_switches();
     const int depth = em_depth(c->h_desc, c->prm.B, sw, n_jobs, kmax, job_utr, job_fixed);
-    const EmPlan plan = em_plan(c->h_desc, c->prm.B, (size_t)n_jobs, job_utr, job_fixed, sw.size_order, depth);
+    EmPlan plan = em_plan(c->h_desc, c->prm.B, (size_t)n_jobs, job_utr, job_fixed, sw.size_order, depth);
     EmKernels kernels;
-    if (em_choose(plan, sw, n_jobs, kmax, kernels) || em_upload(c, plan, (size_t)n_jobs, kmax)) return 1;
+    if (em_choose(plan, sw, n_jobs, kmax, kernels)) return 1;
+    em_liveness(c->h_desc, c->tiles_total, c->prm.nround, sw, kernels, n_jobs, job_utr, job_K, job_fixed, k_arr, plan);
+    if (em_upload(c, plan, (size_t)n_jobs, kmax)) return 1;
     return em_rounds(c, plan, sw, kernels, n_jobs, kmax);
 }
 
@@ -1551,8 +1603,9 @@
     HIPCHK(hipMemsetAsync(c->d_counters.p, 0, N_COUNTERS * sizeof(unsigned long long), c->stream));
     HIPCHK(hipMemsetAsync(c->j_lb.p, 0, nj * nround * 8, c->stream));
     c->h_traffic[3] = 0;
+    c->h_live[0] = c->h_live[1] = 0;
     if (ev_begin(c, 2)) return 1;
-    if (em_lockstep(c, n_jobs, kmax, job_utr, job_fixed)) return 1;
+    if (em_lockstep(c, n_jobs, kmax, job_utr, job_K, job_fixed, k_arr)) return 1;
     if (ev_end(c, 2)) return 1;
     HIPCHK(hipMemcpyAsync(alpha_idx_out, c->j_ao.p, nj * kmax * 4, hipMemcpyDeviceToHost, c->stream));
     HIPCHK(hipMemcpyAsync(beta_idx_out, c->j_bo.p, nj * kmax * 4, hipMemcpyDeviceToHost, c->stream));
@@ -1567,7 +1620,7 @@
     c->last_em_jobs = n_jobs;
 #ifdef M4_STAMPS
     {
-        const unsigned long long *st = hc + 4 + 5 * 64 + 16;
+        const unsigned long long *st = hc + CNT_STAMPS + 16;
         for (int ga = 0; ga < 4; ++ga)
             for (int role = 0; role < 2; ++role) {
                 const double n = (double)st[32 + ga * 2 + role];
@@ -1580,7 +1633,7 @@
 #endif
 #ifdef ESTEP_STAMPS
     {
-        const unsigned long long *st = hc + 4 + 5 * 64;
+        const unsigned long long *st = hc + CNT_STAMPS;
         const double n = (double)st[7];
         if (n > 0)
             fprintf(stderr, "[estep stamps] job-rounds %.0f; mean cycles: set-up %.0f, bin loop %.0f, reductions+weights %.0f, suffix sums %.0f, tail %.0f (total %.0f)\n",
@@ -1594,6 +1647,7 @@
         c->h_traffic[0] += hc[CNT_MSTEP_TENSOR + i];
         c->h_traffic[1] += hc[CNT_MSTEP_VREQ + i];
         c->h_traffic[2] += hc[CNT_MSTEP_VUNI + i];
+        c->h_live[1] += hc[CNT_LIVE_EXIT + i];
     }
     return 0;
 }
@@ -1747,6 +1801,13 @@
     return 0;
 }
 
+int scape_hip_em_live_skip(scape_hip_ctx *c, int64_t *estep_launches, int64_t *mstep_stamp_exits) {
+    if (!c) return fail("ctx is NULL");
+    if (estep_launches) *estep_launches = (int64_t)c->h_live[0];
+    if (mstep_stamp_exits) *mstep_stamp_exits = (int64_t)c->h_live[1];
+    return 0;
+}
+
 }
 
 #include "report.inc"
diff --git a/scape_amd/engine.py b/scape_amd/engine.py
--- a/scape_amd/engine.py
+++ b/scape_amd/engine.py
@@ -185,6 +185,11 @@
         check(self.lib.scape_hip_em_traffic(self.ctx.h, ctypes.byref(t), ctypes.byref(vr), ctypes.byref(vu),
                                             ctypes.byref(n)), "em_traffic")
         return dict(tensor_bytes=t.value, v_bytes_requested=vr.value, v_bytes_unique=vu.value, launches=n.value)
+
+    def em_live_skip(self):
+        e, x = ctypes.c_int64(), ctypes.c_int64()
+        check(self.lib.scape_hip_em_live_skip(self.ctx.h, ctypes.byref(e), ctypes.byref(x)), "em_live_skip")
+        return dict(estep_launches=e.value, mstep_stamp_exits=x.value)
 
     def labels(self, sel):
         if not sel:
```
